# seung-lab/crackle

Hardware: AMD Instinct MI355X
Metric: voxels/s encode+decode, 1024x1024x512 uint32; bit-exact .ckl bytes (higher is better)
Workload: dtype u32

## Files before the change

### crackle_amd/csrc/ckl_encode.hip

```cpp
#include "ckl_encoder.hpp"
#include "ckl_runs.hpp"
#include "ckl_trail.hpp"

#include <algorithm>
#include <atomic>
#include <chrono>
#include <functional>
#include <memory>
#include <mutex>

namespace ckl {

using namespace dev;

template <typename LABEL>
__global__ void __launch_bounds__(kBlock) k_stats(const LABEL* __restrict__ labels, uint64_t voxels, unsigned long long* __restrict__ out ) {
	__shared__ unsigned long long s_max[kWaves], s_pairs[kWaves];
	unsigned long long mx = 0, pairs = 0;
	const uint64_t stride = static_cast<uint64_t>(gridDim.x) * kBlock;
	for (uint64_t i = static_cast<uint64_t>(blockIdx.x) * kBlock + threadIdx.x; i < voxels; i += stride) {
		const LABEL v = labels[i];
		if (static_cast<unsigned long long>(v) > mx) mx = v;
		if (i > 0) pairs += (labels[i - 1] == v);
	}
	for (int d = kWave / 2; d >= 1; d >>= 1) {
		const unsigned long long om = __shfl_xor(mx, d, kWave);
		const unsigned long long op = __shfl_xor(pairs, d, kWave);
		mx = om > mx ? om : mx;
		pairs += op;
	}
	const int lane = threadIdx.x & 63, wave = threadIdx.x >> 6;
	if (lane == 0) { s_max[wave] = mx; s_pairs[wave] = pairs; }
	__syncthreads();
	if (threadIdx.x == 0) {
		for (int w = 1; w < kWaves; w++) { mx = s_max[w] > mx ? s_max[w] : mx; pairs += s_pairs[w]; }
		atomicMax(out, mx);
		atomicAdd(out + 1, pairs);
	}
}

constexpr uint32_t kPlaneUnroll = 4;

template <typename LABEL>
__global__ void __launch_bounds__(kBlock) k_label_planes(
	const LABEL* __restrict__ labels, uint32_t sx, uint32_t sy, uint32_t chunks_per_row,
	uint32_t* __restrict__ planeV, uint32_t* __restrict__ planeH, uint32_t row_words, uint64_t plane_words,
	uint32_t* __restrict__ count_v, uint32_t* __restrict__ count_h
) {
	__shared__ uint32_t s_red[2 * kWaves];
	const uint32_t zi = blockIdx.y;
	const int lane = threadIdx.x & 63, wave = threadIdx.x >> 6;
	const uint32_t units = chunks_per_row * sy;
	const uint32_t unit0 = (blockIdx.x * kWaves + wave) * kPlaneUnroll;
	const LABEL* slice = labels + static_cast<uint64_t>(zi) * sy * sx;
	LABEL v[kPlaneUnroll], up[kPlaneUnroll], lf[kPlaneUnroll];
	uint32_t xs[kPlaneUnroll], ys[kPlaneUnroll];
#pragma unroll
	for (uint32_t k = 0; k < kPlaneUnroll; k++) {
		const uint32_t unit = unit0 + k;
		const uint32_t y = unit / chunks_per_row;
		const uint32_t x = (unit - y * chunks_per_row) * 64u + lane;
		xs[k] = x; ys[k] = y;
		const bool valid = unit < units && x < sx;
		const LABEL* row = slice + static_cast<uint64_t>(y) * sx;
		v[k] = valid ? row[x] : LABEL(0);
		up[k] = (valid && y > 0) ? row[static_cast<int64_t>(x) - static_cast<int64_t>(sx)] : v[k];
		lf[k] = (valid && lane == 0 && x > 0) ? row[x - 1] : v[k];
	}
	uint32_t nv = 0, nh = 0;
#pragma unroll
	for (uint32_t k = 0; k < kPlaneUnroll; k++) {
		const uint32_t unit = unit0 + k;
		const bool valid = unit < units && xs[k] < sx;
		LABEL left = __shfl_up(v[k], 1, kWave);
		if (lane == 0) left = lf[k];
		const bool dv = valid && xs[k] > 0 && v[k] != left;
		const bool dh = valid && v[k] != up[k];
		const unsigned long long mv = __ballot(dv), mh = __ballot(dh);
		if (lane == 0 && unit < units) {
			const uint32_t c = xs[k] >> 6;
			const uint64_t wbase = zi * plane_words + static_cast<uint64_t>(ys[k]) * row_words + c * 2u;
			planeV[wbase] = static_cast<uint32_t>(mv);
			planeH[wbase] = static_cast<uint32_t>(mh);
			if (c * 2u + 1u < row_words) {
				planeV[wbase + 1] = static_cast<uint32_t>(mv >> 32);
				planeH[wbase + 1] = static_cast<uint32_t>(mh >> 32);
			}
			nv += __popcll(mv);
			nh += __popcll(mh);
		}
	}
	if (lane == 0) { s_red[wave] = nv; s_red[kWaves + wave] = nh; }
	__syncthreads();
	if (threadIdx.x == 0) {
		uint32_t tv = 0, th = 0;
		for (int w = 0; w < kWaves; w++) { tv += s_red[w]; th += s_red[kWaves + w]; }
		if (tv) atomicAdd(count_v + zi, tv);
		if (th) atomicAdd(count_h + zi, th);
	}
}

constexpr uint32_t kBandRows = 32;

template <typename V, typename T>
__device__ __forceinline__ V nt_load_vec(const T* p) {
	typedef uint32_t u32x4_t __attribute__((ext_vector_type(4)));
	static_assert(sizeof(V) == 16, "one 16-byte vector");
	const u32x4_t raw = __builtin_nontemporal_load(reinterpret_cast<const u32x4_t*>(p));
	V v;
	__builtin_memcpy(&v, &raw, 16);
	return v;
}

template <typename T>
__device__ __forceinline__ T wave_shift_up1_label(T v) {
	if constexpr (sizeof(T) == 8) {
		const uint32_t lo = dev::wave_shift_up1(static_cast<uint32_t>(v), 0u), hi = dev::wave_shift_up1(static_cast<uint32_t>(static_cast<uint64_t>(v) >> 32), 0u);
		return static_cast<T>((static_cast<uint64_t>(hi) << 32) | lo);
	}
	else return static_cast<T>(dev::wave_shift_up1(static_cast<uint32_t>(v), 0u));
}
template <uint32_t G>
__device__ __forceinline__ uint32_t or_over_lane_group(uint32_t v) {
	static_assert(G == 2 || G == 4 || G == 8 || G == 16, "lane groups inside a row of 16");
	if constexpr (G >= 2) v |= dev::dpp_u32<0xB1, 0xF>(0u, v);
	if constexpr (G >= 4) v |= dev::dpp_u32<0x4E, 0xF>(0u, v);
	if constexpr (G >= 8) v |= dev::dpp_u32<0x141, 0xF>(0u, v);
	if constexpr (G >= 16) v |= dev::dpp_u32<0x140, 0xF>(0u, v);
	return v;
}

template <typename LABEL>
__global__ void __launch_bounds__(kBlock) k_label_planes_stream(
	const LABEL* __restrict__ labels, uint32_t sx, uint32_t sy, uint32_t strips, uint32_t bands,
	uint32_t* __restrict__ planeV, uint32_t* __restrict__ planeH, uint32_t row_words, uint64_t plane_words,
	uint32_t* __restrict__ partial, unsigned long long* __restrict__ partial_max, unsigned long long* __restrict__ total_pairs
) {
	if (blockIdx.x == 0 && blockIdx.y == 0 && threadIdx.x == 0) *total_pairs = 0;
	constexpr uint32_t P = 16 / sizeof(LABEL);
	constexpr uint32_t G = 32 / P;
	constexpr uint32_t WPR = 64 / G;
	struct alignas(16) Vec { LABEL v[P]; };
	__shared__ uint32_t s_red[3 * kWaves];
	__shared__ unsigned long long s_max[kWaves];
	__shared__ __attribute__((aligned(16))) uint32_t s_words[kWaves][2][kBandRows * WPR];
	const uint32_t zi = blockIdx.y;
	const uint32_t lane = threadIdx.x & 63u, wave = threadIdx.x >> 6;
	const uint32_t task = blockIdx.x * kWaves + wave;
	uint32_t nv = 0, nh = 0, pairs = 0;
	LABEL mxl = 0;
	if (task < strips * bands) {
		const uint32_t band = __builtin_amdgcn_readfirstlane(task / strips), strip = __builtin_amdgcn_readfirstlane(task - (task / strips) * strips);
		const uint32_t x0 = strip * (64u * P);
		const uint32_t x = x0 + lane * P;
		const uint32_t y0 = band * kBandRows, y1 = min(y0 + kBandRows, sy);
		const bool active = x < sx;
		const uint64_t slice_off = static_cast<uint64_t>(zi) * sy * sx;
		const LABEL* col = labels + slice_off + (active ? x : 0u);
		Vec prev;
#pragma unroll
		for (uint32_t i = 0; i < P; i++) prev.v[i] = 0;
		if (y0 > 0) prev = nt_load_vec<Vec>(col + static_cast<uint64_t>(y0 - 1) * sx);
		uint32_t* sv = s_words[wave][0];
		uint32_t* sh = s_words[wave][1];
		auto edge_of = [&](uint32_t y, bool& have) -> LABEL {
			const uint64_t lin = slice_off + static_cast<uint64_t>(y) * sx + x0;
			have = lin > 0;
			const uint64_t at = have ? lin - 1 : 0;
			if constexpr (sizeof(LABEL) >= 4) return labels[at];
			else {
				const uint64_t byte = at * sizeof(LABEL);
				const uint32_t w = reinterpret_cast<const uint32_t*>(reinterpret_cast<uintptr_t>(labels) & ~static_cast<uintptr_t>(3))[(byte + (reinterpret_cast<uintptr_t>(labels) & 3u)) >> 2];
				return static_cast<LABEL>(w >> (8u * static_cast<uint32_t>((byte + (reinterpret_cast<uintptr_t>(labels) & 3u)) & 3u)));
			}
		};
		constexpr uint32_t kRowsAhead = 4;
		Vec rows[kRowsAhead];
		LABEL edges[kRowsAhead];
		bool have_edges[kRowsAhead];
		auto request = [&](uint32_t r, uint32_t y) {
			const uint32_t yl = y < y1 ? y : y1 - 1u;
			rows[r] = nt_load_vec<Vec>(col + static_cast<uint64_t>(yl) * sx);
			edges[r] = edge_of(yl, have_edges[r]);
		};
#pragma unroll
		for (uint32_t r = 0; r < kRowsAhead; r++) request(r, y0 + r);
#pragma unroll
		for (uint32_t it = 0; it < kBandRows / kRowsAhead; it++) {
			const uint32_t yb = y0 + it * kRowsAhead;
#pragma unroll
			for (uint32_t r = 0; r < kRowsAhead; r++) {
				const uint32_t y = yb + r;
				const Vec cur = rows[r];
				const LABEL edge = edges[r];
				const bool have_edge = have_edges[r];
				request(r, y + kRowsAhead);
				if (y >= y1) continue;
				LABEL left = wave_shift_up1_label(cur.v[P - 1]);
				bool have_left = true;
				if (lane == 0) { left = edge; have_left = have_edge; }
				uint32_t bv = 0, bh = 0;
				if (active) {
#pragma unroll
					for (uint32_t i = 0; i < P; i++) {
						const LABEL l = i ? cur.v[i - 1] : left;
						bv |= (cur.v[i] != l ? 1u : 0u) << i;
						bh |= (cur.v[i] != prev.v[i] ? 1u : 0u) << i;
						mxl = cur.v[i] > mxl ? cur.v[i] : mxl;
					}
					pairs += P - __popc(bv) - ((have_left || (bv & 1u)) ? 0u : 1u);
					if (x == 0) bv &= ~1u;
					if (y == 0) bh = 0u;
				}
				nv += __popc(bv); nh += __popc(bh);
				bv <<= (lane % G) * P; bh <<= (lane % G) * P;
				bv = or_over_lane_group<G>(bv); bh = or_over_lane_group<G>(bh);
				if ((lane % G) == 0) { sv[(y - y0) * WPR + lane / G] = bv; sh[(y - y0) * WPR + lane / G] = bh; }
				prev = cur;
			}
		}
		const uint32_t word0 = x0 >> 5;
		uint32_t* pv = planeV + zi * plane_words;
		uint32_t* ph = planeH + zi * plane_words;
		constexpr uint32_t kVecWords = WPR >= 4 ? 4u : WPR;
		constexpr uint32_t kLanesPerRow = WPR / kVecWords;
		for (uint32_t r0 = 0; r0 < y1 - y0; r0 += 64u / kLanesPerRow) {
			const uint32_t r = r0 + lane / kLanesPerRow, w = (lane % kLanesPerRow) * kVecWords;
			if (r >= y1 - y0) continue;
			const uint64_t at = static_cast<uint64_t>(y0 + r) * row_words + word0 + w;
			if (word0 + w + kVecWords <= row_words && ((at & (kVecWords - 1u)) == 0u) && kVecWords == 4u) {
				*reinterpret_cast<uint4*>(pv + at) = *reinterpret_cast<const uint4*>(sv + r * WPR + w);
				*reinterpret_cast<uint4*>(ph + at) = *reinterpret_cast<const uint4*>(sh + r * WPR + w);
			}
			else {
				for (uint32_t q = 0; q < kVecWords; q++) if (word0 + w + q < row_words) { pv[at + q] = sv[r * WPR + w + q]; ph[at + q] = sh[r * WPR + w + q]; }
			}
		}
	}
	nv = wave_sum(nv); nh = wave_sum(nh); pairs = wave_sum(pairs);
	unsigned long long mx = static_cast<unsigned long long>(mxl);
	for (int d = kWave / 2; d >= 1; d >>= 1) { const unsigned long long o = __shfl_xor(mx, d, kWave); mx = o > mx ? o : mx; }
	if (lane == 0) { s_red[wave] = nv; s_red[kWaves + wave] = nh; s_red[2 * kWaves + wave] = pairs; s_max[wave] = mx; }
	__syncthreads();
	if (threadIdx.x == 0) {
		uint32_t tv = 0, th = 0, tp = 0;
		unsigned long long tm = 0;
		for (int w = 0; w < kWaves; w++) { tv += s_red[w]; th += s_red[kWaves + w]; tp += s_red[2 * kWaves + w]; tm = s_max[w] > tm ? s_max[w] : tm; }
		const uint64_t o = static_cast<uint64_t>(zi) * gridDim.x + blockIdx.x;
		partial[o * 4 + 0] = tv; partial[o * 4 + 1] = th; partial[o * 4 + 2] = tp; partial[o * 4 + 3] = 0;
		partial_max[o] = tm;
	}
}

__global__ void __launch_bounds__(kBlock) k_planes_from_cracks(
	const uint32_t* __restrict__ crackV, const uint32_t* __restrict__ crackH, uint32_t sx, uint32_t sy,
	uint32_t row_words, uint64_t plane_words, uint32_t permissible,
	uint32_t* __restrict__ planeV, uint32_t* __restrict__ planeH, uint32_t* __restrict__ counts, uint32_t nslices
) {
	__shared__ uint32_t s_red[kWaves];
	const uint32_t zi = blockIdx.y;
	const uint64_t i = static_cast<uint64_t>(blockIdx.x) * kBlock + threadIdx.x;
	uint32_t nv = 0, nh = 0;
	if (i < plane_words) {
		const uint32_t y = static_cast<uint32_t>(i / row_words);
		const uint32_t w = static_cast<uint32_t>(i - static_cast<uint64_t>(y) * row_words);
		const uint32_t left = sx - w * 32u;
		const uint32_t in_row = left >= 32u ? 0xFFFFFFFFu : ((1u << left) - 1u);
		const uint32_t mv = in_row & (w == 0 ? 0xFFFFFFFEu : 0xFFFFFFFFu);
		const uint32_t mh = y >= 1 ? in_row : 0u;
		const uint64_t at = zi * plane_words + i;
		const uint32_t inv = permissible ? 0xFFFFFFFFu : 0u;
		const uint32_t v = (crackV[at] ^ inv) & mv, h = (crackH[at] ^ inv) & mh;
		planeV[at] = v; planeH[at] = h;
		nv = __popc(v); nh = __popc(h);
	}
	nv = block_sum(nv, s_red); nh = block_sum(nh, s_red);
	if (threadIdx.x == 0) {
		if (nv) atomicAdd(counts + zi, nv);
		if (nh) atomicAdd(counts + nslices + zi, nh);
	}
}

__global__ void __launch_bounds__(kBlock) k_planes_reduce(
	const uint32_t* __restrict__ partial, const unsigned long long* __restrict__ partial_max, uint32_t nblk,
	unsigned long long* __restrict__ out ,
	unsigned long long* __restrict__ total_pairs
) {
	__shared__ uint32_t s_red[kWaves];
	__shared__ unsigned long long s_max[kWaves];
	const uint32_t zi = blockIdx.x;
	uint32_t tv = 0, th = 0, tp = 0;
	unsigned long long tm = 0;
	for (uint32_t b = threadIdx.x; b < nblk; b += kBlock) {
		const uint64_t o = static_cast<uint64_t>(zi) * nblk + b;
		tv += partial[o * 4 + 0]; th += partial[o * 4 + 1]; tp += partial[o * 4 + 2];
		const unsigned long long m = partial_max[o];
		tm = m > tm ? m : tm;
	}
	tv = block_sum(tv, s_red); th = block_sum(th, s_red); tp = block_sum(tp, s_red);
	for (int d = kWave / 2; d >= 1; d >>= 1) { const unsigned long long o = __shfl_xor(tm, d, kWave); tm = o > tm ? o : tm; }
	if ((threadIdx.x & 63) == 0) s_max[threadIdx.x >> 6] = tm;
	__syncthreads();
	if (threadIdx.x == 0) {
		for (int w = 0; w < kWaves; w++) tm = s_max[w] > tm ? s_max[w] : tm;
		out[4ull * zi + 0] = tv; out[4ull * zi + 1] = th; out[4ull * zi + 2] = tp; out[4ull * zi + 3] = tm;
		atomicAdd(total_pairs, static_cast<unsigned long long>(tp));
	}
}

enum : uint8_t { CODE_UP = 0, CODE_RIGHT = 1, CODE_DOWN = 2, CODE_LEFT = 3, CODE_NONE = 0xFE, CODE_TOMB = 0xFF };

struct FinishArgs {
	int sx, sy, xw, yw;
	uint32_t z0;
	uint32_t markov;
	const uint64_t* cbase;
	const uint64_t* kbase;
	const uint32_t* n_chains;
	const uint32_t* n_raw;
	const uint32_t* n_valid;
	const uint8_t* cp;
	const uint32_t* chain_node;
	const uint32_t* chain_off;
	const uint32_t* chain_clen;
	uint32_t* chain_order;
	uint32_t* chain_dst;
	uint32_t* chain_vstart;
	uint8_t* fcode;
	uint8_t* dcode;
	const uint64_t* pbase;
	uint8_t* payload;
	const uint64_t* bbase;
	uint8_t* boc;
	uint32_t* payload_len;
	uint32_t* boc_len;
};

__device__ __forceinline__ void put_le_dev(uint8_t* p, uint32_t v, int w) {
	for (int i = 0; i < w; i++) p[i] = static_cast<uint8_t>((v >> (8 * i)) & 0xFF);
}

constexpr int kFinishBlock = 1024;
constexpr int kFinishWaves = kFinishBlock / kWave;

constexpr uint32_t kFinishChains = 2048;

__global__ void __launch_bounds__(kFinishBlock) k_finish(FinishArgs a) {
	__shared__ uint32_t s_scan[kFinishWaves];
	__shared__ uint32_t s_node[kFinishChains], s_clen[kFinishChains], s_off[kFinishChains], s_ord[kFinishChains], s_dst[kFinishChains], s_vst[kFinishChains];
	const uint32_t zi = blockIdx.x + a.z0;
	const int tid = threadIdx.x;
	const uint32_t nch = a.n_chains[zi], nraw = a.n_raw[zi], nvalid = a.n_valid[zi];
	const uint8_t* cp = a.cp + a.cbase[zi];
	uint8_t* fcode = a.fcode + a.cbase[zi];
	const bool staged = nch <= kFinishChains;
	const uint32_t* ch_node = a.chain_node + a.kbase[zi];
	const uint32_t* ch_off = a.chain_off + a.kbase[zi];
	const uint32_t* ch_clen = a.chain_clen + a.kbase[zi];
	uint32_t* order = a.chain_order + a.kbase[zi];
	uint32_t* dst = a.chain_dst + a.kbase[zi];
	uint32_t* vstart = a.chain_vstart + a.kbase[zi];
	if (staged) {
		for (uint32_t c = tid; c < nch; c += kFinishBlock) { s_node[c] = ch_node[c]; s_clen[c] = ch_clen[c]; s_off[c] = ch_off[c]; }
		__syncthreads();
		ch_node = s_node; ch_off = s_off; ch_clen = s_clen; order = s_ord; dst = s_dst; vstart = s_vst;
	}
	const uint32_t sxe = a.sx + 1;

	if (tid == 0) {
		uint32_t v = 0;
		for (uint32_t c = 0; c < nch; c++) { vstart[c] = v; v += ch_clen[c]; }
		for (uint32_t c = 0; c < nch; c++) {
			const uint32_t key = ch_node[c];
			uint32_t p = c;
			while (p > 0 && ch_node[order[p - 1]] > key) { order[p] = order[p - 1]; p--; }
			order[p] = c;
		}
		uint32_t d = 0;
		for (uint32_t i = 0; i < nch; i++) { dst[order[i]] = d; d += ch_clen[order[i]]; }

		uint8_t* b = a.boc + a.bbase[zi];
		uint32_t num_y = 0, index_size = a.yw;
		for (uint32_t i = 0; i < nch;) {
			const uint32_t y = ch_node[order[i]] / sxe;
			uint32_t j = i;
			while (j < nch && ch_node[order[j]] / sxe == y) j++;
			index_size += a.yw + (j - i + 1) * a.xw;
			num_y++;
			i = j;
		}
		uint32_t idx = 0;
		put_le_dev(b + idx, index_size, 4); idx += 4;
		put_le_dev(b + idx, num_y, a.yw); idx += a.yw;
		uint32_t last_y = 0;
		for (uint32_t i = 0; i < nch;) {
			const uint32_t y = ch_node[order[i]] / sxe;
			uint32_t j = i;
			while (j < nch && ch_node[order[j]] / sxe == y) j++;
			put_le_dev(b + idx, y - last_y, a.yw); idx += a.yw;
			last_y = y;
			put_le_dev(b + idx, j - i, a.xw); idx += a.xw;
			uint32_t last_x = 0;
			for (uint32_t k = i; k < j; k++) {
				const uint32_t x = ch_node[order[k]] - sxe * y;
				put_le_dev(b + idx, x - last_x, a.xw); idx += a.xw;
				last_x = x;
			}
			i = j;
		}
		a.boc_len[zi] = idx;
	}
	__syncthreads();
	__threadfence_block();

	constexpr uint32_t kPer = 16;
	uint32_t carry = 0;
	for (uint32_t tile = 0; tile < nraw; tile += kFinishBlock * kPer) {
		const uint32_t i0 = tile + tid * kPer;
		uint32_t cnt = 0;
		uint8_t c[kPer];
		static_assert(kPer == 16, "one 16-byte load per thread");
		if (i0 + kPer <= nraw) {
			const uint4 v = *reinterpret_cast<const uint4*>(cp + i0);
			const uint32_t w4[4] = { v.x, v.y, v.z, v.w };
#pragma unroll
			for (uint32_t k = 0; k < kPer; k++) c[k] = static_cast<uint8_t>(w4[k >> 2] >> (8u * (k & 3u)));
		}
		else {
#pragma unroll
			for (uint32_t k = 0; k < kPer; k++) { const uint32_t i = i0 + k; c[k] = i < nraw ? cp[i] : CODE_TOMB; }
		}
#pragma unroll
		for (uint32_t k = 0; k < kPer; k++) cnt += (c[k] != CODE_TOMB);
		uint32_t v[1] = { cnt }, tot[1];
		block_excl_add<1, kFinishWaves>(v, tot, s_scan);
		uint32_t g = carry + v[0];
		if (cnt) {
			uint32_t lo = 0, hi = nch;
			while (lo + 1 < hi) {
				const uint32_t mid = (lo + hi) >> 1;
				if (ch_off[mid] <= i0) lo = mid; else hi = mid;
			}
			uint32_t chain = lo;
			uint32_t next_off = (chain + 1 < nch) ? ch_off[chain + 1] : 0xFFFFFFFFu;
			if (i0 + kPer <= next_off) {
				struct __attribute__((packed)) U128 { uint4 v; };
				struct __attribute__((packed)) U64 { unsigned long long v; };
				struct __attribute__((packed)) U32 { uint32_t v; };
				struct __attribute__((packed)) U16 { uint16_t v; };
				uint8_t* d = fcode + dst[chain] + (g - vstart[chain]);
				unsigned long long w0 = 0, w1 = 0;
				uint32_t m = 0;
#pragma unroll
				for (uint32_t k = 0; k < kPer; k++) {
					if (c[k] != CODE_TOMB) {
						if (m < 8u) w0 |= static_cast<unsigned long long>(c[k]) << (8u * m);
						else w1 |= static_cast<unsigned long long>(c[k]) << (8u * (m - 8u));
						m++;
					}
				}
				if (m == 16u) reinterpret_cast<U128*>(d)->v = make_uint4(static_cast<uint32_t>(w0), static_cast<uint32_t>(w0 >> 32), static_cast<uint32_t>(w1), static_cast<uint32_t>(w1 >> 32));
				else {
					if (m & 8u) { reinterpret_cast<U64*>(d)->v = w0; d += 8; w0 = w1; }
					if (m & 4u) { reinterpret_cast<U32*>(d)->v = static_cast<uint32_t>(w0); d += 4; w0 >>= 32; }
					if (m & 2u) { reinterpret_cast<U16*>(d)->v = static_cast<uint16_t>(w0); d += 2; w0 >>= 16; }
					if (m & 1u) d[0] = static_cast<uint8_t>(w0);
				}
			}
			else {
#pragma unroll
				for (uint32_t k = 0; k < kPer; k++) {
					const uint32_t i = i0 + k;
					while (i >= next_off) { chain++; next_off = (chain + 1 < nch) ? ch_off[chain + 1] : 0xFFFFFFFFu; }
					if (c[k] != CODE_TOMB) {
						fcode[dst[chain] + (g - vstart[chain])] = c[k];
						g++;
					}
				}
			}
		}
		carry += tot[0];
	}
	__syncthreads();
	__threadfence_block();

	if (a.markov) {
		uint8_t* dcode = a.dcode + a.cbase[zi];
		for (uint32_t g = tid; g < nvalid; g += kFinishBlock) {
			const uint32_t prev = g ? fcode[g - 1] : 0u;
			dcode[g] = static_cast<uint8_t>((fcode[g] - prev) & 3u);
		}
		if (tid == 0) a.payload_len[zi] = 0;
	}
	else {
		uint8_t* out = a.payload + a.pbase[zi];
		const uint32_t nbytes = (nvalid + 3) / 4;
		const uint32_t nwords = (nvalid + 15) / 16;
		for (uint32_t w = tid; w < nwords; w += kFinishBlock) {
			const uint32_t g0 = w * 16u;
			uint8_t c[16];
			if (g0 + 16u <= nvalid) {
				const uint4 v = *reinterpret_cast<const uint4*>(fcode + g0);
				const uint32_t w4[4] = { v.x, v.y, v.z, v.w };
#pragma unroll
				for (uint32_t j = 0; j < 16; j++) c[j] = static_cast<uint8_t>(w4[j >> 2] >> (8u * (j & 3u)));
			}
			else {
#pragma unroll
				for (uint32_t j = 0; j < 16; j++) c[j] = g0 + j < nvalid ? fcode[g0 + j] : 0;
			}
			uint32_t prev = g0 ? fcode[g0 - 1] : 0u;
			uint32_t enc = 0;
#pragma unroll
			for (uint32_t j = 0; j < 16; j++) {
				if (g0 + j < nvalid) enc |= ((c[j] - prev) & 3u) << (2 * j);
				prev = c[j];
			}
			if (4u * w + 4u <= nbytes) reinterpret_cast<uint32_t*>(out)[w] = enc;
			else for (uint32_t k = 4u * w; k < nbytes; k++) out[k] = static_cast<uint8_t>(enc >> (8u * (k - 4u * w)));
		}
		if (tid == 0) a.payload_len[zi] = nbytes;
	}
}

__device__ __forceinline__ uint32_t markov_ctx(const uint8_t* d, uint32_t g, int order) {
	uint32_t ctx = 0;
	for (int j = 1; j <= order; j++) {
		const uint32_t v = (g >= static_cast<uint32_t>(j)) ? d[g - j] : 0u;
		ctx |= v << (2 * (order - j));
	}
	return ctx;
}

__global__ void __launch_bounds__(kBlock) k_markov_hist(
	const uint8_t* __restrict__ dcode, const uint64_t* __restrict__ cbase, const uint32_t* __restrict__ n_valid,
	int order, uint32_t* __restrict__ hist, uint32_t lds_entries
) {
	extern __shared__ uint32_t s_hist[];
	const uint32_t zi = blockIdx.x;
	const uint8_t* d = dcode + cbase[zi];
	const uint32_t n = n_valid[zi];
	const uint32_t entries = 4u << (2 * order);
	const bool local = entries <= lds_entries;
	if (local) {
		for (uint32_t i = threadIdx.x; i < entries; i += kBlock) s_hist[i] = 0;
		__syncthreads();
	}
	uint32_t* target = local ? s_hist : hist;
	constexpr uint32_t kPer = 32;
	for (uint32_t g0 = threadIdx.x * kPer; g0 < n; g0 += kBlock * kPer) {
		uint32_t key = 0xFFFFFFFFu, cnt = 0;
		const uint32_t g1 = g0 + kPer < n ? g0 + kPer : n;
		for (uint32_t g = g0; g < g1; g++) {
			const uint32_t k = markov_ctx(d, g, order) * 4u + d[g];
			if (k == key) cnt++;
			else {
				if (cnt) atomicAdd(target + key, cnt);
				key = k; cnt = 1;
			}
		}
		if (cnt) atomicAdd(target + key, cnt);
	}
	if (local) {
		__syncthreads();
		for (uint32_t i = threadIdx.x; i < entries; i += kBlock) { const uint32_t v = s_hist[i]; if (v) atomicAdd(hist + i, v); }
	}
}

__global__ void __launch_bounds__(kBlock) k_markov_pack(
	const uint8_t* __restrict__ dcode, const uint64_t* __restrict__ cbase, const uint32_t* __restrict__ n_valid,
	int order, const uint8_t* __restrict__ model ,
	const uint64_t* __restrict__ pbase, uint8_t* __restrict__ payload, uint32_t* __restrict__ payload_len
) {
	__shared__ uint32_t s_scan[kWaves];
	const uint32_t zi = blockIdx.x;
	const uint8_t* d = dcode + cbase[zi];
	const uint32_t n = n_valid[zi];
	uint32_t* words = reinterpret_cast<uint32_t*>(payload + pbase[zi]);
	constexpr uint32_t kPer = 8;
	uint32_t carry = 0;
	for (uint32_t tile = 0; tile < n; tile += kBlock * kPer) {
		const uint32_t g0 = tile + threadIdx.x * kPer;
		uint32_t bits[kPer], lens[kPer], tot_len = 0;
#pragma unroll
		for (uint32_t k = 0; k < kPer; k++) {
			const uint32_t g = g0 + k;
			bits[k] = 0; lens[k] = 0;
			if (g < n) {
				if (g == 0) { bits[k] = d[0]; lens[k] = 2; }
				else {
					const uint32_t r = model[markov_ctx(d, g, order) * 4u + d[g]];
					bits[k] = (r == 0) ? 0u : (r == 1) ? 1u : (r == 2) ? 3u : 7u;
					lens[k] = (r == 0) ? 1u : (r == 1) ? 2u : 3u;
				}
			}
			tot_len += lens[k];
		}
		uint32_t v[1] = { tot_len }, tot[1];
		block_excl_add<1>(v, tot, s_scan);
		uint32_t off = carry + v[0];
#pragma unroll
		for (uint32_t k = 0; k < kPer; k++) {
			if (lens[k] && bits[k]) {
				const uint32_t w = off >> 5, sh = off & 31;
				atomicOr(words + w, bits[k] << sh);
				if (sh + lens[k] > 32) atomicOr(words + w + 1, bits[k] >> (32 - sh));
			}
			off += lens[k];
		}
		carry += tot[0];
	}
	if (threadIdx.x == 0) payload_len[zi] = (carry + 7) / 8;
}

template <typename LABEL>
__global__ void __launch_bounds__(kBlock) k_mapping_comps(
	const LABEL* __restrict__ labels, RunArrays r, uint64_t sxy,
	const uint64_t* __restrict__ comp_off, uint64_t* __restrict__ mapping
) {
	const uint32_t zi = blockIdx.y;
	const uint32_t c = blockIdx.x * kBlock + threadIdx.x;
	if (c >= r.ncomp[zi]) return;
	mapping[comp_off[zi] + c] = static_cast<uint64_t>(labels[zi * sxy + r.comp_pix[r.rbase[zi] + c]]);
}

__global__ void __launch_bounds__(kBlock) k_paint_components(
	const uint32_t* __restrict__ planeV, uint32_t row_words, uint64_t plane_words, uint32_t sx, uint64_t sxy,
	const uint32_t* __restrict__ word_base, const uint64_t* __restrict__ rbase, const uint32_t* __restrict__ run_cc,
	const uint64_t* __restrict__ comp_off, uint32_t id_base, uint32_t* __restrict__ out
) {
	const uint32_t zi = blockIdx.y;
	const uint32_t px = blockIdx.x * kBlock + threadIdx.x;
	if (px >= sxy) return;
	const uint32_t y = px / sx, x = px - y * sx;
	const uint32_t w = x >> 5, bit = x & 31u;
	const uint64_t wi = zi * plane_words + static_cast<uint64_t>(y) * row_words + w;
	uint32_t b = planeV[wi];
	if (w == 0) b |= 1u;
	const uint32_t run = word_base[wi] - 1u + __popc(b & (0xFFFFFFFFu >> (31u - bit)));
	out[zi * sxy + px] = run_cc[rbase[zi] + run] + static_cast<uint32_t>(comp_off[zi]) + id_base;
}

__global__ void __launch_bounds__(kBlock) k_paint_components4(
	const uint32_t* __restrict__ planeV, uint32_t row_words, uint64_t plane_words, uint32_t sx, uint64_t sxy,
	const uint32_t* __restrict__ word_base, const uint64_t* __restrict__ rbase, const uint32_t* __restrict__ run_cc,
	const uint64_t* __restrict__ comp_off, uint32_t id_base, uint32_t* __restrict__ out
) {
	const uint32_t zi = blockIdx.y;
	const uint32_t px = (blockIdx.x * kBlock + threadIdx.x) * 4u;
	if (px >= sxy) return;
	const uint32_t y = px / sx, x = px - y * sx;
	const uint32_t w = x >> 5, bit = x & 31u;
	const uint64_t wi = zi * plane_words + static_cast<uint64_t>(y) * row_words + w;
	uint32_t b = planeV[wi];
	if (w == 0) b |= 1u;
	const uint32_t* cc = run_cc + rbase[zi];
	const uint32_t add = static_cast<uint32_t>(comp_off[zi]) + id_base;
	uint32_t run = word_base[wi] - 1u + __popc(b & (0xFFFFFFFFu >> (31u - bit)));
	uint4 o;
	o.x = cc[run] + add;
	run += (b >> (bit + 1u)) & 1u; o.y = cc[run] + add;
	run += (b >> (bit + 2u)) & 1u; o.z = cc[run] + add;
	run += (b >> (bit + 3u)) & 1u; o.w = cc[run] + add;
	*reinterpret_cast<uint4*>(out + zi * sxy + px) = o;
}

inline void launch_paint_components(hipStream_t s, const uint32_t* planeV, uint32_t row_words, uint64_t plane_words, int64_t sx, int64_t sy, int64_t sz,
	const uint32_t* word_base, const uint64_t* rbase, const uint32_t* run_cc, const uint64_t* comp_off, uint32_t id_base, uint32_t* out) {
	const uint64_t sxy = static_cast<uint64_t>(sx) * sy;
	const bool four = sx % 4 == 0 && (reinterpret_cast<uintptr_t>(out) & 15u) == 0;
	const uint64_t threads = four ? sxy / 4 : sxy;
	const dim3 grid(static_cast<uint32_t>((threads + kBlock - 1) / kBlock), static_cast<uint32_t>(sz));
	if (four) hipLaunchKernelGGL(k_paint_components4, grid, dim3(kBlock), 0, s, planeV, row_words, plane_words, static_cast<uint32_t>(sx), sxy, word_base, rbase, run_cc, comp_off, id_base, out);
	else hipLaunchKernelGGL(k_paint_components, grid, dim3(kBlock), 0, s, planeV, row_words, plane_words, static_cast<uint32_t>(sx), sxy, word_base, rbase, run_cc, comp_off, id_base, out);
}

__global__ void __launch_bounds__(kBlock) k_bitonic_step(uint64_t* __restrict__ a, uint32_t j, uint32_t k, uint32_t n) {
	const uint32_t i = blockIdx.x * kBlock + threadIdx.x;
	if (i >= n) return;
	const uint32_t l = i ^ j;
	if (l > i) {
		const uint64_t x = a[i], y = a[l];
		const bool up = (i & k) == 0;
		if ((x > y) == up) { a[i] = y; a[l] = x; }
	}
}
__global__ void __launch_bounds__(kBlock) k_bitonic_step2(uint64_t* __restrict__ a, uint32_t j, uint32_t k, uint32_t n) {
	const uint32_t t = blockIdx.x * kBlock + threadIdx.x;
	if (t >= n / 4u) return;
	const uint32_t h = j >> 1;
	const uint32_t lb = static_cast<uint32_t>(__ffs(h)) - 1u;
	const uint32_t i = (t & (h - 1u)) | ((t >> lb) << (lb + 2u));
	uint64_t v0 = a[i], v1 = a[i | h], v2 = a[i | j], v3 = a[i | j | h];
	const bool up = (i & k) == 0;
	auto cx = [&](uint64_t& x, uint64_t& y) { if ((x > y) == up) { const uint64_t z = x; x = y; y = z; } };
	cx(v0, v2); cx(v1, v3);
	cx(v0, v1); cx(v2, v3);
	a[i] = v0; a[i | h] = v1; a[i | j] = v2; a[i | j | h] = v3;
}

__global__ void __launch_bounds__(kBlock) k_bitonic_first(uint64_t* __restrict__ a, uint32_t n) {
	__shared__ uint64_t s[2048];
	const uint32_t base = blockIdx.x * 2048u;
	for (uint32_t t = threadIdx.x; t < 2048u; t += kBlock) s[t] = base + t < n ? a[base + t] : ~0ull;
	__syncthreads();
	for (uint32_t k = 2; k <= 2048u; k <<= 1) {
		for (uint32_t j = k >> 1; j > 0; j >>= 1) {
			for (uint32_t t = threadIdx.x; t < 2048u; t += kBlock) {
				const uint32_t l = t ^ j;
				if (l > t) {
					const uint64_t x = s[t], y = s[l];
					const bool up = ((base + t) & k) == 0;
					if ((x > y) == up) { s[t] = y; s[l] = x; }
				}
			}
			__syncthreads();
		}
	}
	for (uint32_t t = threadIdx.x; t < 2048u; t += kBlock) if (base + t < n) a[base + t] = s[t];
}
__global__ void __launch_bounds__(kBlock) k_bitonic_local(uint64_t* __restrict__ a, uint32_t j_start, uint32_t k, uint32_t n) {
	__shared__ uint64_t s[2048];
	const uint32_t base = blockIdx.x * 2048u;
	for (uint32_t t = threadIdx.x; t < 2048u; t += kBlock) s[t] = base + t < n ? a[base + t] : ~0ull;
	__syncthreads();
	for (uint32_t j = j_start; j > 0; j >>= 1) {
		for (uint32_t t = threadIdx.x; t < 2048u; t += kBlock) {
			const uint32_t l = t ^ j;
			if (l > t) {
				const uint64_t x = s[t], y = s[l];
				const bool up = ((base + t) & k) == 0;
				if ((x > y) == up) { s[t] = y; s[l] = x; }
			}
		}
		__syncthreads();
	}
	for (uint32_t t = threadIdx.x; t < 2048u; t += kBlock) if (base + t < n) a[base + t] = s[t];
}
__global__ void __launch_bounds__(kBlock) k_pad_copy_u64(const uint64_t* __restrict__ src, uint64_t n, uint64_t* __restrict__ dst, uint64_t n_pad) {
	const uint64_t i = static_cast<uint64_t>(blockIdx.x) * kBlock + threadIdx.x;
	if (i < n_pad) dst[i] = i < n ? src[i] : ~0ull;
}
constexpr uint32_t kUniqPer = 8, kUniqItems = kBlock * kUniqPer;
__device__ __forceinline__ uint32_t unique_heads(const uint64_t* __restrict__ sorted, uint32_t n, uint32_t i0, uint64_t (&v)[kUniqPer]) {
	uint32_t flag = 0;
#pragma unroll
	for (uint32_t q = 0; q < kUniqPer; q++) {
		const uint32_t i = i0 + q;
		v[q] = i < n ? sorted[i] : 0;
		const uint64_t prev = q ? v[q - 1] : ((i > 0 && i < n) ? sorted[i - 1] : 0);
		flag |= ((i < n && (i == 0 || v[q] != prev)) ? 1u : 0u) << q;
	}
	return flag;
}
__global__ void __launch_bounds__(kBlock) k_unique_count(const uint64_t* __restrict__ sorted, uint32_t n, uint32_t* __restrict__ blk_count) {
	__shared__ uint32_t s_red[kWaves];
	uint64_t v[kUniqPer];
	const uint32_t flag = unique_heads(sorted, n, blockIdx.x * kUniqItems + threadIdx.x * kUniqPer, v);
	const uint32_t tot = block_sum(static_cast<uint32_t>(__popc(flag)), s_red);
	if (threadIdx.x == 0) blk_count[blockIdx.x] = tot;
}
__global__ void __launch_bounds__(kBlock) k_unique_scan(uint32_t* __restrict__ blk_count, uint32_t nblk, uint32_t* __restrict__ n_uniq) {
	__shared__ uint32_t s_scan[kWaves];
	uint32_t carry = 0;
	for (uint32_t b0 = 0; b0 < nblk; b0 += kBlock) {
		const uint32_t b = b0 + threadIdx.x;
		uint32_t c[1] = { b < nblk ? blk_count[b] : 0u }, tot[1];
		block_excl_add<1>(c, tot, s_scan);
		if (b < nblk) blk_count[b] = carry + c[0];
		carry += tot[0];
	}
	if (threadIdx.x == 0) *n_uniq = carry;
}
__global__ void __launch_bounds__(kBlock) k_unique_scatter(const uint64_t* __restrict__ sorted, uint32_t n, const uint32_t* __restrict__ blk_base, uint64_t* __restrict__ uniq) {
	__shared__ uint32_t s_scan[kWaves];
	uint64_t v[kUniqPer];
	const uint32_t flag = unique_heads(sorted, n, blockIdx.x * kUniqItems + threadIdx.x * kUniqPer, v);
	uint32_t c[1] = { static_cast<uint32_t>(__popc(flag)) }, tot[1];
	block_excl_add<1>(c, tot, s_scan);
	uint32_t o = blk_base[blockIdx.x] + c[0];
#pragma unroll
	for (uint32_t q = 0; q < kUniqPer; q++) if ((flag >> q) & 1u) uniq[o++] = v[q];
}

constexpr uint64_t kLabelHashEmpty = ~0ull;
__device__ __forceinline__ uint32_t label_hash(uint64_t v) {
	v ^= v >> 33; v *= 0xff51afd7ed558ccdull; v ^= v >> 33;
	return static_cast<uint32_t>(v);
}
__global__ void __launch_bounds__(kBlock) k_label_hash_insert(const uint64_t* __restrict__ mapping, uint32_t n, unsigned long long* __restrict__ table, uint32_t mask, uint32_t* __restrict__ has_max) {
	const uint32_t i = blockIdx.x * kBlock + threadIdx.x;
	if (i >= n) return;
	const unsigned long long v = mapping[i];
	if (v == kLabelHashEmpty) { *has_max = 1u; return; }
	uint32_t h = label_hash(v) & mask;
	for (uint32_t probe = 0; probe <= mask; probe++) {
		const unsigned long long seen = table[h];
		if (seen == v) return;
		if (seen == kLabelHashEmpty) {
			const unsigned long long old = atomicCAS(table + h, kLabelHashEmpty, v);
			if (old == kLabelHashEmpty || old == v) return;
		}
		h = (h + 1u) & mask;
	}
}
__device__ __forceinline__ uint32_t hash_occupied(const unsigned long long* __restrict__ table, uint32_t slots, uint32_t i0, uint64_t (&v)[kUniqPer]) {
	uint32_t flag = 0;
#pragma unroll
	for (uint32_t q = 0; q < kUniqPer; q++) {
		v[q] = i0 + q < slots ? table[i0 + q] : kLabelHashEmpty;
		flag |= (v[q] != kLabelHashEmpty ? 1u : 0u) << q;
	}
	return flag;
}
__global__ void __launch_bounds__(kBlock) k_label_hash_count(const unsigned long long* __restrict__ table, uint32_t slots, uint32_t* __restrict__ blk_count) {
	__shared__ uint32_t s_red[kWaves];
	uint64_t v[kUniqPer];
	const uint32_t flag = hash_occupied(table, slots, blockIdx.x * kUniqItems + threadIdx.x * kUniqPer, v);
	const uint32_t tot = block_sum(static_cast<uint32_t>(__popc(flag)), s_red);
	if (threadIdx.x == 0) blk_count[blockIdx.x] = tot;
}
__global__ void __launch_bounds__(kBlock) k_label_hash_scatter(
	const unsigned long long* __restrict__ table, uint32_t slots, const uint32_t* __restrict__ blk_base, const uint32_t* __restrict__ n_found,
	const uint32_t* __restrict__ has_max, uint64_t* __restrict__ out
) {
	__shared__ uint32_t s_scan[kWaves];
	uint64_t v[kUniqPer];
	const uint32_t flag = hash_occupied(table, slots, blockIdx.x * kUniqItems + threadIdx.x * kUniqPer, v);
	uint32_t c[1] = { static_cast<uint32_t>(__popc(flag)) }, tot[1];
	block_excl_add<1>(c, tot, s_scan);
	uint32_t o = blk_base[blockIdx.x] + c[0];
#pragma unroll
	for (uint32_t q = 0; q < kUniqPer; q++) if ((flag >> q) & 1u) out[o++] = v[q];
	if (blockIdx.x == 0 && threadIdx.x == 0 && *has_max) out[*n_found] = kLabelHashEmpty;
}

__global__ void __launch_bounds__(kBlock) k_flat_section(
	const uint64_t* __restrict__ uniq, const uint32_t* __restrict__ n_uniq, int stored_width,
	const uint32_t* __restrict__ ncomp, uint32_t nslices, int component_width,
	const uint64_t* __restrict__ mapping, uint32_t n, uint8_t* __restrict__ out
) {
	const uint32_t nu = *n_uniq;
	const int key_width = nu <= 0xFFu ? 1 : (nu <= 0xFFFFu ? 2 : 4);
	const uint32_t i = blockIdx.x * kBlock + threadIdx.x;
	if (i == 0) for (int b = 0; b < 8; b++) out[b] = static_cast<uint8_t>((static_cast<uint64_t>(nu) >> (8 * b)) & 0xFF);
	uint8_t* o_uniq = out + 8;
	uint8_t* o_cc = o_uniq + static_cast<uint64_t>(nu) * stored_width;
	uint8_t* o_keys = o_cc + static_cast<uint64_t>(nslices) * component_width;
	if (i < nu) {
		const uint64_t v = uniq[i];
		for (int b = 0; b < stored_width; b++) o_uniq[static_cast<uint64_t>(i) * stored_width + b] = static_cast<uint8_t>((v >> (8 * b)) & 0xFF);
	}
	if (i < nslices) {
		const uint32_t v = ncomp[i];
		for (int b = 0; b < component_width; b++) o_cc[static_cast<uint64_t>(i) * component_width + b] = b < 4 ? static_cast<uint8_t>((v >> (8 * b)) & 0xFF) : 0;
	}
	if (i < n) {
		const uint64_t v = mapping[i];
		uint32_t lo = 0, hi = nu;
		while (lo + 1 < hi) {
			const uint32_t mid = (lo + hi) >> 1;
			if (uniq[mid] <= v) lo = mid; else hi = mid;
		}
		for (int b = 0; b < key_width; b++) o_keys[static_cast<uint64_t>(i) * key_width + b] = static_cast<uint8_t>((lo >> (8 * b)) & 0xFF);
	}
}

__global__ void __launch_bounds__(kBlock) k_code_offsets(
	const uint32_t* __restrict__ boc_len, const uint32_t* __restrict__ payload_len, const uint32_t* __restrict__ slice_err,
	uint32_t nslices, uint64_t* __restrict__ out_off, uint32_t* __restrict__ report
) {
	__shared__ unsigned long long s_part[kBlock];
	__shared__ uint32_t s_err;
	if (threadIdx.x == 0) s_err = 0;
	const uint32_t per = (nslices + kBlock - 1) / kBlock;
	const uint32_t z0 = threadIdx.x * per, z1 = min(z0 + per, nslices);
	unsigned long long sum = 0;
	uint32_t err = 0;
	for (uint32_t z = z0; z < z1; z++) { sum += static_cast<unsigned long long>(boc_len[z]) + payload_len[z]; err |= slice_err[z]; }
	s_part[threadIdx.x] = sum;
	__syncthreads();
	if (err) atomicOr(&s_err, err);
	if (threadIdx.x == 0) {
		unsigned long long run = 0;
		for (uint32_t i = 0; i < kBlock; i++) { const unsigned long long v = s_part[i]; s_part[i] = run; run += v; }
		report[nslices] = static_cast<uint32_t>(run); report[nslices + 1] = static_cast<uint32_t>(run >> 32);
	}
	__syncthreads();
	unsigned long long off = s_part[threadIdx.x];
	for (uint32_t z = z0; z < z1; z++) {
		const uint32_t len = boc_len[z] + payload_len[z];
		out_off[z] = off;
		report[z] = len;
		off += len;
	}
	if (threadIdx.x == 0) report[nslices + 2] = s_err;
}

__global__ void __launch_bounds__(kBlock) k_gather_codes(
	const uint8_t* __restrict__ boc, const uint64_t* __restrict__ bbase, const uint32_t* __restrict__ boc_len,
	const uint8_t* __restrict__ payload, const uint64_t* __restrict__ pbase, const uint32_t* __restrict__ payload_len,
	const uint64_t* __restrict__ out_off, uint8_t* __restrict__ out
) {
	const uint32_t zi = blockIdx.x;
	uint8_t* o = out + out_off[zi];
	const uint32_t nb = boc_len[zi], np = payload_len[zi];
	const uint8_t* b = boc + bbase[zi];
	const uint8_t* p = payload + pbase[zi];
	for (uint32_t i = threadIdx.x; i < nb; i += kBlock) o[i] = b[i];
	for (uint32_t i = threadIdx.x; i < np; i += kBlock) o[nb + i] = p[i];
}

struct CrcShifts { uint32_t x[8]; };
__global__ void __launch_bounds__(kBlock) k_crc32c_pieces(const uint8_t* __restrict__ data, uint64_t n, uint64_t pad, uint32_t P, CrcShifts sh, uint32_t* __restrict__ parts) {
	__shared__ uint32_t s_tab[256];
	__shared__ uint32_t s_st[kBlock];
	{
		uint32_t c = threadIdx.x;
		for (int k = 0; k < 8; k++) c = (c & 1u) ? (c >> 1) ^ dev::kCrcPoly : (c >> 1);
		s_tab[threadIdx.x] = c;
	}
	__syncthreads();
	const uint64_t f0 = (static_cast<uint64_t>(blockIdx.x) * kBlock + threadIdx.x) * P;
	uint32_t c = 0;
	for (uint32_t g = 0; g < P; g += 16) {
		const int64_t m0 = static_cast<int64_t>(f0 + g) - static_cast<int64_t>(pad);
		uint32_t w[4] = { 0, 0, 0, 0 };
		if (m0 >= 0 && static_cast<uint64_t>(m0) + 16u <= n) __builtin_memcpy(w, data + m0, 16);
		else if (m0 + 16 > 0) for (int b = 0; b < 16; b++) { const int64_t i = m0 + b; if (i >= 0 && static_cast<uint64_t>(i) < n) w[b >> 2] |= static_cast<uint32_t>(data[i]) << (8 * (b & 3)); }
#pragma unroll
		for (int b = 0; b < 16; b++) c = s_tab[(c ^ (w[b >> 2] >> (8 * (b & 3)))) & 0xFFu] ^ (c >> 8);
	}
	s_st[threadIdx.x] = c;
	__syncthreads();
	for (int k = 0; k < 8; k++) {
		const uint32_t stride = 1u << k;
		if ((threadIdx.x & (2u * stride - 1u)) == 0u) s_st[threadIdx.x] = gf_mul(s_st[threadIdx.x], sh.x[k]) ^ s_st[threadIdx.x + stride];
		__syncthreads();
	}
	if (threadIdx.x == 0) parts[blockIdx.x] = s_st[0];
}
__global__ void __launch_bounds__(kBlock) k_crc32c_fold(const uint32_t* __restrict__ parts, uint32_t G, CrcShifts sh, uint32_t init_term, uint32_t* __restrict__ out) {
	__shared__ uint32_t s_st[kBlock];
	s_st[threadIdx.x] = threadIdx.x < G ? parts[threadIdx.x] : 0u;
	__syncthreads();
	for (int k = 0; (1u << k) < G; k++) {
		const uint32_t stride = 1u << k;
		if ((threadIdx.x & (2u * stride - 1u)) == 0u && threadIdx.x + stride < G) s_st[threadIdx.x] = gf_mul(s_st[threadIdx.x], sh.x[k]) ^ s_st[threadIdx.x + stride];
		__syncthreads();
	}
	if (threadIdx.x == 0) out[0] = ~(s_st[0] ^ init_term);
}

__global__ void __launch_bounds__(kBlock) k_copy_bytes(const uint8_t* __restrict__ src, uint8_t* __restrict__ dst, uint64_t n) {
	const uint64_t head = min(n, static_cast<uint64_t>((4u - (reinterpret_cast<uintptr_t>(dst) & 3u)) & 3u));
	const uint64_t words = (n - head) / 4u;
	const uint64_t tid = static_cast<uint64_t>(blockIdx.x) * kBlock + threadIdx.x;
	const uint64_t stride = static_cast<uint64_t>(gridDim.x) * kBlock;
	if (tid < head) dst[tid] = src[tid];
	const uint64_t tail0 = head + words * 4u;
	if (tid < n - tail0) dst[tail0 + tid] = src[tail0 + tid];
	const uint8_t* s0 = src + head;
	const uint32_t sh = static_cast<uint32_t>(reinterpret_cast<uintptr_t>(s0) & 3u) * 8u;
	const uint32_t* sw = reinterpret_cast<const uint32_t*>(reinterpret_cast<uintptr_t>(s0) & ~static_cast<uintptr_t>(3));
	uint32_t* dw = reinterpret_cast<uint32_t*>(dst + head);
	if (sh == 0u) {
		for (uint64_t i = tid; i < words; i += stride) dw[i] = sw[i];
	}
	else {
		for (uint64_t i = tid; i < words; i += stride) dw[i] = __funnelshift_r(sw[i], sw[i + 1], sh);
	}
}

__global__ void __launch_bounds__(kBlock) k_trail_step_kinds(const uint32_t* __restrict__ events, const uint64_t* __restrict__ ibase, const uint32_t* __restrict__ n_events, uint32_t* __restrict__ counts) {
	__shared__ uint32_t s_c[5];
	const uint32_t zi = blockIdx.x;
	if (threadIdx.x < 5) s_c[threadIdx.x] = 0u;
	__syncthreads();
	const uint32_t n = n_events[zi] & ~(dev::kEvFormatAddr12 | dev::kEvWalkWide);
	const uint32_t* ev = events + ibase[zi];
	uint32_t c[4] = { 0, 0, 0, 0 };
	for (uint32_t i = threadIdx.x; i < n; i += kBlock) c[ev[i] >> 30]++;
	for (int k = 0; k < 4; k++) if (c[k]) atomicAdd(&s_c[k], c[k]);
	if (threadIdx.x == 0) {
		uint32_t run = 0, longest = 0;
		for (uint32_t i = 0; i < n; i++) { if ((ev[i] >> 30) == 1u) run = 0; else { run++; longest = run > longest ? run : longest; } }
		s_c[4] = longest;
	}
	__syncthreads();
	if (threadIdx.x < 5) counts[zi * 5u + threadIdx.x] = s_c[threadIdx.x];
}

}

using namespace ckl;

static void crc32c_device(const uint8_t* data, uint64_t n, uint32_t* parts, uint32_t* out, hipStream_t s) {
	uint32_t P = 128, G = 1;
	while (G < static_cast<uint32_t>(kBlock) && static_cast<uint64_t>(G) * kBlock * P < n) G <<= 1;
	if (static_cast<uint64_t>(G) * kBlock * P < n) P = static_cast<uint32_t>(((n + static_cast<uint64_t>(G) * kBlock - 1) / (static_cast<uint64_t>(G) * kBlock) + 15) / 16 * 16);
	const uint64_t frame = static_cast<uint64_t>(G) * kBlock * P;
	static std::mutex shifts_mutex;
	static uint32_t shifts_for = 0;
	static CrcShifts shifts_in, shifts_over;
	CrcShifts in_wg, over_wg;
	{
		std::lock_guard<std::mutex> lock(shifts_mutex);
		if (shifts_for != P) {
			for (int k = 0; k < 8; k++) {
				shifts_in.x[k] = gf_xpow(8ull * P << k);
				shifts_over.x[k] = gf_xpow(8ull * P * kBlock << k);
			}
			shifts_for = P;
		}
		in_wg = shifts_in; over_wg = shifts_over;
	}
	hipLaunchKernelGGL(k_crc32c_pieces, dim3(G), dim3(kBlock), 0, s, data, n, frame - n, P, in_wg, parts);
	hipLaunchKernelGGL(k_crc32c_fold, dim3(1), dim3(kBlock), 0, s, parts, G, over_wg, gf_mul(0xFFFFFFFFu, gf_xpow(8ull * n)), out);
}

static void copy_bytes_device(const uint8_t* src, uint8_t* dst, uint64_t n, hipStream_t s) {
	if (!n) return;
	const uint32_t blocks = static_cast<uint32_t>(std::min<uint64_t>((n / 4u + kBlock - 1) / kBlock + 1u, 8192u));
	hipLaunchKernelGGL(k_copy_bytes, dim3(blocks), dim3(kBlock), 0, s, src, dst, n);
}

namespace {

struct UploadPacker {
	struct Item { void* buf; size_t off, count; void (*bind)(void*, uint8_t*, size_t); };
	std::vector<Item> items;
	std::vector<uint8_t> image;
	template <typename T>
	void add(DevBuf<T>& dst, const std::vector<T>& src) {
		const size_t off = (image.size() + 255) & ~static_cast<size_t>(255);
		image.resize(off + std::max<size_t>(src.size(), 1) * sizeof(T));
		if (!src.empty()) memcpy(image.data() + off, src.data(), src.size() * sizeof(T));
		items.push_back({ &dst, off, src.size(), [](void* b, uint8_t* base, size_t n) { static_cast<DevBuf<T>*>(b)->borrow(reinterpret_cast<T*>(base), n); } });
	}
	void commit(DevBuf<uint8_t>& block, hipStream_t s, void** staging = nullptr) {
		if (image.empty()) return;
		for (const Item& it : items) it.bind(it.buf, nullptr, 0);
		block.ensure(image.size());
		if (staging) {
			if (*staging) host_out_free(*staging);
			*staging = host_out_alloc(std::max<size_t>(image.size(), 64u << 10));
			memcpy(*staging, image.data(), image.size());
			upload_small(block.p, *staging, image.size(), s, *staging);
		}
		else CKL_HIP(hipMemcpyAsync(block.p, image.data(), image.size(), hipMemcpyHostToDevice, s));
		for (const Item& it : items) it.bind(it.buf, block.p + it.off, it.count);
	}
};

template <typename LABEL>
VolumeStats volume_stats(ckl_encoder& e, const LABEL* labels, uint64_t voxels) {
	VolumeStats st;
	if (voxels == 0) return st;
	hipStream_t s = e.stream;
	e.d_stats.ensure(2);
	CKL_HIP(hipMemsetAsync(e.d_stats.p, 0, 2 * sizeof(unsigned long long), s));
	const uint32_t blocks = static_cast<uint32_t>(std::min<uint64_t>((voxels + kBlock - 1) / kBlock, 256ull * 8));
	hipLaunchKernelGGL(k_stats<LABEL>, dim3(blocks), dim3(kBlock), 0, s, labels, voxels, e.d_stats.p);
	auto r = download(e.d_stats.p, 2, s);
	st.max_label = r[0]; st.pairs = r[1];
	LABEL f, l;
	CKL_HIP(hipMemcpy(&f, labels, sizeof(LABEL), hipMemcpyDeviceToHost));
	CKL_HIP(hipMemcpy(&l, labels + (voxels - 1), sizeof(LABEL), hipMemcpyDeviceToHost));
	st.first = f; st.last = l;
	return st;
}

inline uint32_t* plane_v(const ckl_encoder& e) { return e.d_planes.p; }
inline uint32_t* plane_h(const ckl_encoder& e, uint32_t ns) { return e.d_planes.p + e.plane_words * ns; }

inline bool planes_cached(const ckl_encoder& e, const void* labels, int64_t sx, int64_t sy, int64_t sz) {
	return e.planes_for == labels && e.planes_dims[0] == sx && e.planes_dims[1] == sy && e.planes_dims[2] == sz;
}

inline uint64_t crack_edges(const ckl_encoder& e, int64_t sx, int64_t sy, size_t zi, bool permissible) {
	const uint64_t interior = static_cast<uint64_t>(sx > 0 ? sx - 1 : 0) * sy + static_cast<uint64_t>(sx) * (sy > 0 ? sy - 1 : 0);
	const uint64_t differ = static_cast<uint64_t>(e.count_v[zi]) + e.count_h[zi];
	return permissible ? interior - differ : differ;
}

void planes_collect(ckl_encoder& e, uint32_t ns, VolumeStats* st, const std::vector<unsigned long long>* fetched = nullptr) {
	std::vector<unsigned long long> mine;
	if (!fetched) { mine = download(e.d_plane_out.p, 4ull * ns, e.stream); fetched = &mine; }
	const std::vector<unsigned long long>& o = *fetched;
	e.count_v.resize(ns); e.count_h.resize(ns);
	VolumeStats v;
	for (uint32_t zi = 0; zi < ns; zi++) {
		e.count_v[zi] = static_cast<uint32_t>(o[4ull * zi]);
		e.count_h[zi] = static_cast<uint32_t>(o[4ull * zi + 1]);
		v.pairs += o[4ull * zi + 2];
		v.max_label = std::max<uint64_t>(v.max_label, o[4ull * zi + 3]);
	}
	e.planes_deferred = false;
	if (st) *st = v;
}

void trail_prezero(ckl_encoder& e, int64_t sx, int64_t sy, int64_t sz) {
	hipStream_t s = e.stream2;
	const uint32_t ns = static_cast<uint32_t>(sz);
	const uint64_t nverts = static_cast<uint64_t>(sx + 1) * (sy + 1);
	const uint32_t start_words = static_cast<uint32_t>((nverts + 31) / 32);
	e.d_slice_err.ensure(ns);
	e.t_counters.ensure(7 * static_cast<size_t>(ns));
	e.t_start_bits.ensure(static_cast<size_t>(start_words) * ns);
	CKL_HIP(hipMemsetAsync(e.d_slice_err.p, 0, ns * sizeof(uint32_t), s));
	CKL_HIP(hipMemsetAsync(e.t_counters.p, 0, 7 * static_cast<size_t>(ns) * sizeof(uint32_t), s));
	CKL_HIP(hipMemsetAsync(e.t_start_bits.p, 0, static_cast<size_t>(start_words) * ns * sizeof(uint32_t), s));
	CKL_HIP(hipEventRecord(e.ev_prezero, s));
	e.trail_zeroed = true;
}

template <typename LABEL>
void planes_pass(ckl_encoder& e, const LABEL* labels, int64_t sx, int64_t sy, int64_t sz, VolumeStats* st, bool defer = false) {
	hipStream_t s = e.stream;
	const uint32_t ns = static_cast<uint32_t>(sz);
	e.trail_zeroed = false;
	e.planes_deferred = false;
	e.row_words = static_cast<uint32_t>((sx + 31) / 32);
	e.plane_words = static_cast<uint64_t>(e.row_words) * sy;
	e.d_planes.ensure(2 * e.plane_words * ns);
	constexpr uint32_t P = 16 / sizeof(LABEL);
	const bool fast = !getenv("CKL_PLANES_GENERIC") && sx >= static_cast<int64_t>(P) && sx % P == 0 && (reinterpret_cast<uintptr_t>(labels) & 15u) == 0;
	if (fast) {
		const uint32_t strips = static_cast<uint32_t>((sx + 64 * P - 1) / (64 * P));
		const uint32_t bands = static_cast<uint32_t>((sy + kBandRows - 1) / kBandRows);
		const uint32_t nblk = (strips * bands + kWaves - 1) / kWaves;
		e.d_plane_partial.ensure(4ull * nblk * ns);
		e.d_plane_partial_max.ensure(static_cast<size_t>(nblk) * ns);
		e.d_plane_out.ensure(4ull * ns + 1);
		trail_prezero(e, sx, sy, sz);
		hipLaunchKernelGGL(k_label_planes_stream<LABEL>, dim3(nblk, ns), dim3(kBlock), 0, s,
			labels, static_cast<uint32_t>(sx), static_cast<uint32_t>(sy), strips, bands,
			plane_v(e), plane_h(e, ns), e.row_words, e.plane_words,
			e.d_plane_partial.p, e.d_plane_partial_max.p, e.d_plane_out.p + 4ull * ns);
		hipLaunchKernelGGL(k_planes_reduce, dim3(ns), dim3(kBlock), 0, s, e.d_plane_partial.p, e.d_plane_partial_max.p, nblk, e.d_plane_out.p, e.d_plane_out.p + 4ull * ns);
		e.planes_deferred = defer;
		if (!e.planes_deferred) planes_collect(e, ns, st);
		return;
	}
	if (st) *st = volume_stats<LABEL>(e, labels, static_cast<uint64_t>(sx) * sy * sz);
	e.d_count_vh.ensure(2 * static_cast<size_t>(ns));
	CKL_HIP(hipMemsetAsync(e.d_count_vh.p, 0, 2 * static_cast<size_t>(ns) * sizeof(uint32_t), s));
	const uint32_t chunks = static_cast<uint32_t>((sx + 63) / 64);
	const uint64_t units = static_cast<uint64_t>(chunks) * sy;
	hipLaunchKernelGGL(k_label_planes<LABEL>, dim3(static_cast<uint32_t>((units + kWaves * kPlaneUnroll - 1) / (kWaves * kPlaneUnroll)), ns), dim3(kBlock), 0, s,
		labels, static_cast<uint32_t>(sx), static_cast<uint32_t>(sy), chunks,
		plane_v(e), plane_h(e, ns), e.row_words, e.plane_words,
		e.d_count_vh.p, e.d_count_vh.p + ns);
	std::vector<uint32_t> c = download(e.d_count_vh.p, 2 * static_cast<size_t>(ns), s);
	e.count_v.assign(c.begin(), c.begin() + ns);
	e.count_h.assign(c.begin() + ns, c.end());
}

void planes_pass_any(ckl_encoder& e, const void* labels, int64_t sx, int64_t sy, int64_t sz, VolumeStats* st) {
	with_label_type(e.dtype_bytes, [&](auto t) { planes_pass(e, static_cast<const typename decltype(t)::type*>(labels), sx, sy, sz, st); });
}

enum class GraphFormat : uint32_t { IMPERMISSIBLE = 0, PERMISSIBLE = 1, ON_DEVICE = 2 };
inline GraphFormat graph_format(bool permissible) { return permissible ? GraphFormat::PERMISSIBLE : GraphFormat::IMPERMISSIBLE; }
void graph_pass(ckl_encoder& e, int64_t sx, int64_t sy, int64_t sz, GraphFormat format, VolumeStats* st = nullptr) {
	hipStream_t s = e.stream;
	const uint32_t ns = static_cast<uint32_t>(sz);
	e.tiles_x = static_cast<uint32_t>((sx + 1 + kTrailTileDim - 1) / kTrailTileDim);
	e.tiles_y = static_cast<uint32_t>((sy + 1 + 7) / 8);
	const uint32_t mtx = static_cast<uint32_t>((sx + 1 + 7) / 8), mty = static_cast<uint32_t>((sy + 1 + 7) / 8);
	e.mtx2 = (mtx + 1) / 2;
	e.adjm_stride = static_cast<uint64_t>(e.mtx2) * ((mty + 1) / 2) * 4 * 2;
	e.d_adjm.ensure(e.adjm_stride * ns);
	e.graph_blocks = (e.tiles_x * e.tiles_y + kBlock - 1) / kBlock;
	e.t_blk_special.ensure(static_cast<size_t>(e.graph_blocks) * ns);
	e.t_blk_corner.ensure(static_cast<size_t>(e.graph_blocks) * ns);
	e.d_count_vh.ensure(4 * static_cast<size_t>(ns));
	const bool on_device = format == GraphFormat::ON_DEVICE;
	if (on_device && !e.planes_deferred) throw Error(CKL_ERR_RUNTIME, "crackle_amd: internal: crack format left to the device without deferred counts");
	const unsigned long long half_voxels = static_cast<unsigned long long>(static_cast<int64_t>(static_cast<uint64_t>(sx) * sy * sz) / 2);
	hipLaunchKernelGGL(k_trail_graph, dim3(e.graph_blocks, ns), dim3(kBlock), 0, s,
		plane_v(e), plane_h(e, ns), e.row_words, e.plane_words,
		static_cast<uint32_t>(sx), static_cast<uint32_t>(sy), static_cast<uint32_t>(format),
		on_device ? e.d_plane_out.p + 4ull * ns : nullptr, half_voxels,
		reinterpret_cast<uint32_t*>(e.d_adjm.p), e.adjm_stride * 4,
		e.mtx2, e.tiles_x, e.tiles_y, e.t_blk_special.p, e.t_blk_corner.p);
	hipLaunchKernelGGL(k_trail_count_scan, dim3(ns), dim3(kBlock), 0, s, e.t_blk_special.p, e.t_blk_corner.p, e.graph_blocks,
		e.d_count_vh.p + 2 * static_cast<size_t>(ns), e.d_count_vh.p + 3 * static_cast<size_t>(ns));
	std::vector<unsigned long long> po;
	if (e.planes_deferred) {
		po.resize(4ull * ns);
		CKL_HIP(hipMemcpyAsync(po.data(), e.d_plane_out.p, po.size() * sizeof(unsigned long long), hipMemcpyDeviceToHost, s));
	}
	std::vector<uint32_t> c = download(e.d_count_vh.p + 2 * static_cast<size_t>(ns), 2 * static_cast<size_t>(ns), s);
	e.count_special.assign(c.begin(), c.begin() + ns);
	e.count_corner.assign(c.begin() + ns, c.end());
	VolumeStats v;
	if (!po.empty()) planes_collect(e, ns, &v, &po);
	if (st && !po.empty()) *st = v;
	e.graph_permissible = on_device ? static_cast<int64_t>(v.pairs) < static_cast<int64_t>(static_cast<uint64_t>(sx) * sy * sz) / 2 : format == GraphFormat::PERMISSIBLE;
}

enum class CrackGoal { HISTOGRAM, CODES };
struct CrackRequest {
	CrackGoal goal = CrackGoal::CODES;
	bool permissible = false;
	int markov_order = 0;
	const std::vector<uint8_t>* model = nullptr;
	bool reuse_trail = false;
	std::function<void()> overlap;
};
struct CrackResult {
	std::vector<uint32_t> code_len;
	uint64_t total = 0;
	bool any_chain = false;
	std::vector<uint32_t> hist;
	std::vector<uint8_t> model;
};

inline size_t trail_walk_lds(uint32_t max_special) { return (static_cast<size_t>(max_special) + 256) * 16 + 1024; }

FinishArgs finish_args(const ckl_encoder& e, int64_t sx, int64_t sy, int markov_order) {
	FinishArgs fa;
	fa.sx = static_cast<int>(sx); fa.sy = static_cast<int>(sy);
	fa.xw = byte_width(static_cast<uint64_t>(sx) + 1); fa.yw = byte_width(static_cast<uint64_t>(sy) + 1);
	fa.markov = markov_order ? 1u : 0u;
	fa.cbase = e.d_cbase.p; fa.kbase = e.d_kbase.p;
	fa.n_chains = e.d_n_chains.p; fa.n_raw = e.d_n_raw.p; fa.n_valid = e.d_n_valid.p;
	fa.cp = e.d_cp.p; fa.chain_node = e.d_chain_node.p; fa.chain_off = e.d_chain_off.p; fa.chain_clen = e.d_chain_clen.p;
	fa.chain_order = e.d_chain_order.p; fa.chain_dst = e.d_chain_dst.p; fa.chain_vstart = e.d_chain_vstart.p;
	fa.fcode = e.d_fcode.p; fa.dcode = e.d_dcode.p;
	fa.pbase = e.d_pbase.p; fa.payload = e.d_payload.p; fa.bbase = e.d_bbase.p; fa.boc = e.d_boc.p;
	fa.payload_len = e.d_payload_len.p; fa.boc_len = e.d_boc_len.p;
	fa.z0 = 0;
	return fa;
}

TrailArgs trail_args(const ckl_encoder& e, int64_t sx, int64_t sy, uint32_t ns) {
	const uint64_t nverts = static_cast<uint64_t>(sx + 1) * (sy + 1);
	TrailArgs ta;
	ta.adjm = e.d_adjm.p; ta.adjm_stride = e.adjm_stride; ta.mtx2 = e.mtx2; ta.tiles_x = e.tiles_x; ta.tiles_y = e.tiles_y;
	ta.planeV = plane_v(e); ta.planeH = plane_h(e, ns); ta.row_words = e.row_words; ta.plane_words = e.plane_words;
	ta.sx = static_cast<uint32_t>(sx); ta.sy = static_cast<uint32_t>(sy); ta.inv = e.graph_permissible ? 0xFFFFFFFFu : 0u;
	ta.sxe = static_cast<uint32_t>(sx + 1); ta.sye = static_cast<uint32_t>(sy + 1); ta.nverts = static_cast<uint32_t>(nverts);
	ta.max_steps = e.t_max_steps.p;
	ta.nbase = e.t_nbase.p; ta.ncap = e.t_ncap.p;
	ta.n_nodes = e.t_counters.p; ta.n_corners = e.t_counters.p + 2 * ns;
	ta.n_starts = e.t_counters.p + 3 * ns; ta.n_items = e.t_counters.p + 4 * ns;
	ta.node_vertex = e.t_node_vertex.p; ta.node_adj = e.t_node_adj.p; ta.vert2node = e.t_vert2node.p;
	ta.cobase = e.t_cobase.p; ta.cocap = e.t_cocap.p; ta.corner_vertex = e.t_corner_vertex.p;
	ta.dart_end = e.t_dart_end.p; ta.dart_len = e.t_dart_len.p; ta.dart_minv = e.t_dart_minv.p; ta.dart_minpos = e.t_dart_minpos.p;
	ta.dart_codes = e.t_dart_codes.p; ta.dart_inline = e.t_dart_inline.p;
	ta.parent = e.t_parent.p; ta.compmin = e.t_compmin.p;
	ta.start_bits = e.t_start_bits.p; ta.start_words = static_cast<uint32_t>((nverts + 31) / 32); ta.starts = e.t_starts.p;
	ta.ibase = e.t_ibase.p; ta.icap = e.t_icap.p; ta.items = e.t_items.p; ta.item_off = e.t_item_off.p;
	ta.sbase = e.d_sbase.p; ta.scap = e.d_scap.p; ta.stack_node = e.d_stack_node.p; ta.stack_item = e.d_stack_code.p;
	ta.kbase = e.d_kbase.p; ta.kcap = e.d_kcap.p;
	ta.chain_node = e.d_chain_node.p; ta.chain_item0 = e.t_chain_item0.p; ta.chain_off = e.d_chain_off.p; ta.chain_clen = e.d_chain_clen.p;
	ta.n_chains = e.d_n_chains.p; ta.n_raw = e.d_n_raw.p; ta.n_valid = e.d_n_valid.p;
	ta.cbase = e.d_cbase.p; ta.ccap = e.d_ccap.p; ta.cp = e.d_cp.p; ta.slice_err = e.d_slice_err.p;
	ta.events = e.t_events.p; ta.n_events = e.t_counters.p + 5 * ns; ta.seg_len_sum = e.t_counters.p + 6 * ns; ta.chain_ev0 = e.t_chain_ev0.p; ta.ev_lnd = e.t_ev_lnd.p; ta.ev_item = e.t_ev_item.p;
	ta.dbg = nullptr;
	{ const char* env = getenv("CKL_TRAIL_WALK"); ta.walk_plain = (env && !strcmp(env, "plain")) ? 1u : 0u; ta.walk_no_regs = (env && !strcmp(env, "lds")) ? 1u : 0u; }
	{ const char* env = getenv("CKL_TRAIL_WALK_STACK"); ta.walk_stack_cap = env ? static_cast<uint32_t>(std::max(1, atoi(env))) : 0xFFFFFFFFu; }
	ta.graph_blocks = e.graph_blocks; ta.blk_special = e.t_blk_special.p; ta.blk_corner = e.t_blk_corner.p;
	ta.z0 = 0;
	return ta;
}

void trail_diag(ckl_encoder& e, uint32_t ns, const unsigned long long* ta_dbg, uint32_t max_special, size_t trail_lds_used) {
	hipStream_t s = e.stream;
	std::vector<uint32_t> c = download(e.t_counters.p, 5 * static_cast<size_t>(ns), s);
	double m[5] = { 0 };
	for (int k = 0; k < 5; k++) for (uint32_t zi = 0; zi < ns; zi++) m[k] += static_cast<double>(c[static_cast<size_t>(k) * ns + zi]) / ns;
	double sp = 0, co = 0;
	for (uint32_t zi = 0; zi < ns; zi++) { sp += static_cast<double>(e.count_special[zi]) / ns; co += static_cast<double>(e.count_corner[zi]) / ns; }
	if (ta_dbg) {
		std::vector<unsigned long long> g = download(ta_dbg, 16, s);
		if (g[11]) fprintf(stderr, "[ckl trail diag, k_trail_walk] mean cycles per slice: table fill=%.0f fill + walk=%.0f\n", static_cast<double>(g[6]) / g[11], static_cast<double>(g[7]) / g[11]);
		if (g[11]) fprintf(stderr, "[ckl trail diag, k_trail_walk] slices=%llu iterations/slice=%.0f cycles/iteration=%.0f clock=%.2f GHz (cycles / 100 MHz ticks)\n",
			g[11], static_cast<double>(g[8]) / g[11], g[8] ? static_cast<double>(g[9]) / g[8] : 0.0, g[10] ? static_cast<double>(g[9]) / (g[10] * 10.0) : 0.0);
		fprintf(stderr, "[ckl trail diag, k_trail_components, mean cycles per slice] union=%.0f component minima=%.0f starts/splits=%.0f bitmap scan=%.0f\n",
			static_cast<double>(g[12]) / ns, static_cast<double>(g[13]) / ns, static_cast<double>(g[14]) / ns, static_cast<double>(g[15]) / ns);
		fprintf(stderr, "[ckl trail diag, k_trail_segments] waves=%llu iterations/wave mean=%.1f max=%llu cycles/wave mean=%.0f max=%llu cycles/iteration=%.0f active lanes/iteration=%.1f\n",
			g[4], g[4] ? static_cast<double>(g[0]) / g[4] : 0.0, g[1], g[4] ? static_cast<double>(g[2]) / g[4] : 0.0, g[3],
			g[0] ? static_cast<double>(g[2]) / g[0] : 0.0, g[0] ? static_cast<double>(g[5]) / g[0] : 0.0);
	}
	fprintf(stderr, "[ckl trail diag] max degree-1/3/4 vertices of a slice=%u, k_trail_walk LDS=%zu bytes\n", max_special, trail_lds_used);
	fprintf(stderr, "[ckl trail diag, mean per slice] degree-1/3/4 vertices=%.0f corners=%.0f nodes=%.0f starts=%.0f items=%.0f\n", sp, co, m[0], m[3], m[4]);
}

void check_walk_errors(ckl_encoder& e, uint32_t ns) {
	const std::vector<uint32_t> errs = download(e.d_slice_err.p, ns, e.stream);
	for (uint32_t zi = 0; zi < ns; zi++) if (errs[zi]) throw Error(CKL_ERR_RUNTIME, "crackle_amd: crack walk scratch overflow on z=" + std::to_string(zi));
}

CrackResult crack_pass(ckl_encoder& e, int64_t sx, int64_t sy, int64_t sz, const CrackRequest& rq) {
	hipStream_t s = e.stream;
	const uint32_t ns = static_cast<uint32_t>(sz);
	const uint64_t nverts = static_cast<uint64_t>(sx + 1) * (sy + 1);
	const int markov_order = rq.markov_order;
	const bool reuse_trail = rq.reuse_trail;
	if (rq.goal == CrackGoal::HISTOGRAM && (!markov_order || rq.model)) throw Error(CKL_ERR_RUNTIME, "crackle_amd: internal: a markov histogram needs an order and no model");
	CrackResult result;
	e.d_slice_err.ensure(ns);
	const bool prezeroed = e.trail_zeroed && !reuse_trail;
	e.trail_zeroed = false;
	if (prezeroed) CKL_HIP(hipStreamWaitEvent(s, e.ev_prezero, 0));
	if (!reuse_trail && !prezeroed) CKL_HIP(hipMemsetAsync(e.d_slice_err.p, 0, ns * sizeof(uint32_t), s));

	std::vector<uint64_t> cbase(ns), sbase(ns), kbase(ns);
	std::vector<uint32_t> ccap(ns), scap(ns), kcap(ns), max_steps(ns);
	std::vector<uint64_t> nbase(ns), cobase(ns), ibase(ns);
	std::vector<uint32_t> ncap(ns), cocap(ns), icap(ns);
	uint64_t ctot = 0, stot = 0, ktot = 0, ntot = 0, cotot = 0, itot = 0;
	uint32_t max_ncap = 0, max_cocap = 0, max_icap = 0, max_special = 0;
	bool any = false;
	for (uint32_t zi = 0; zi < ns; zi++) {
		const uint64_t E = crack_edges(e, sx, sy, zi, rq.permissible);
		any = any || E > 0;
		const uint64_t cc = ((7 * E + 16 + 15) / 16) * 16;
		if (cc > 0xFFFFFFF0ull) throw Error(CKL_ERR_RUNTIME, "crackle_amd: slice has too many crack edges");
		cbase[zi] = ctot; ccap[zi] = static_cast<uint32_t>(cc); ctot += cc;
		max_steps[zi] = static_cast<uint32_t>(E + 1);
		const uint64_t nc = ((static_cast<uint64_t>(e.count_special[zi]) + e.count_corner[zi] + 16) / 16) * 16;
		if (nc >= (1ull << 28)) throw Error(CKL_ERR_RUNTIME, "crackle_amd: slice has too many crack vertices");
		nbase[zi] = ntot; ncap[zi] = static_cast<uint32_t>(nc); ntot += nc;
		cobase[zi] = cotot; cocap[zi] = e.count_corner[zi]; cotot += e.count_corner[zi];
		const uint64_t ic = 7 * nc + 16;
		ibase[zi] = itot; icap[zi] = static_cast<uint32_t>(ic); itot += ic;
		sbase[zi] = stot; scap[zi] = static_cast<uint32_t>(2 * nc + 4); stot += 2 * nc + 4;
		kbase[zi] = ktot; kcap[zi] = static_cast<uint32_t>(nc); ktot += nc;
		max_ncap = std::max<uint32_t>(max_ncap, ncap[zi]);
		max_cocap = std::max<uint32_t>(max_cocap, cocap[zi]);
		max_icap = std::max<uint32_t>(max_icap, icap[zi]);
		max_special = std::max<uint32_t>(max_special, e.count_special[zi]);
	}
	result.any_chain = any;
	if (g_ht && g_ht->on) {
		uint32_t over = 0;
		for (uint32_t zi = 0; zi < ns; zi++) over += e.count_special[zi] > 3584u;
		fprintf(stderr, "[ckl trail nodes] max special %u, slices above 3584: %u of %u\n", max_special, over, ns);
	}
	HT_MARK("c:caps");

	UploadPacker tables;
	tables.add(e.d_cbase, cbase); tables.add(e.d_ccap, ccap);
	tables.add(e.d_sbase, sbase); tables.add(e.d_scap, scap);
	tables.add(e.d_kbase, kbase); tables.add(e.d_kcap, kcap);
	e.d_cp.ensure(ctot); e.d_fcode.ensure(ctot);
	if (markov_order) e.d_dcode.ensure(ctot);
	e.d_stack_node.ensure(stot); e.d_stack_code.ensure(stot);
	e.d_chain_node.ensure(ktot); e.d_chain_off.ensure(ktot); e.d_chain_clen.ensure(ktot);
	e.d_chain_order.ensure(ktot); e.d_chain_dst.ensure(ktot); e.d_chain_vstart.ensure(ktot);
	e.d_n_chains.ensure(ns); e.d_n_raw.ensure(ns); e.d_n_valid.ensure(ns);
	e.d_payload_len.ensure(ns); e.d_boc_len.ensure(ns);
	const int xw = byte_width(static_cast<uint64_t>(sx) + 1), yw = byte_width(static_cast<uint64_t>(sy) + 1);
	std::vector<uint64_t> pbase(ns), bbase(ns);
	uint64_t ptot = 0, btot = 0;
	for (uint32_t zi = 0; zi < ns; zi++) {
		const uint64_t ncodes = ccap[zi];
		const uint64_t pbytes = markov_order ? (3ull * ncodes + 2 + 7) / 8 : (ncodes + 3) / 4;
		pbase[zi] = ptot; ptot += ((pbytes + 8 + 3) / 4) * 4;
		const uint64_t bbytes = 4 + yw + static_cast<uint64_t>(kcap[zi]) * (yw + 2 * xw);
		bbase[zi] = btot; btot += bbytes;
	}
	tables.add(e.d_pbase, pbase); tables.add(e.d_bbase, bbase);
	tables.add(e.t_nbase, nbase); tables.add(e.t_ncap, ncap);
	tables.add(e.t_cobase, cobase); tables.add(e.t_cocap, cocap);
	tables.add(e.t_ibase, ibase); tables.add(e.t_icap, icap);
	tables.add(e.t_max_steps, max_steps);
	tables.commit(e.d_crack_tables, s, e.uploads_by_kernel ? &e.tables_staging : nullptr);
	HT_MARK("c:tables");
	e.d_payload.ensure(ptot + 8); e.d_boc.ensure(btot + 8);
	e.codes_capacity = ptot + btot;
	if (markov_order) CKL_HIP(hipMemsetAsync(e.d_payload.p, 0, ptot + 8, s));

	DevBuf<unsigned long long> d_tdbg;
	size_t trail_lds_used = 0;
	if (!reuse_trail) {
		e.t_counters.ensure(7 * static_cast<size_t>(ns));
		if (!prezeroed) CKL_HIP(hipMemsetAsync(e.t_counters.p, 0, 7 * static_cast<size_t>(ns) * sizeof(uint32_t), s));
		e.t_node_vertex.ensure(ntot); e.t_node_adj.ensure(ntot + 16); e.t_vert2node.ensure(nverts * ns);
		e.t_corner_vertex.ensure(cotot);
		e.t_dart_end.ensure(4 * ntot); e.t_dart_len.ensure(4 * ntot); e.t_dart_minv.ensure(4 * ntot); e.t_dart_minpos.ensure(4 * ntot);
		e.t_dart_codes.ensure(4 * ntot); e.t_dart_inline.ensure(4 * ntot);
		e.t_parent.ensure(ntot); e.t_compmin.ensure(ntot); e.t_starts.ensure(ntot);
		const uint32_t start_words = static_cast<uint32_t>((nverts + 31) / 32);
		e.t_start_bits.ensure(static_cast<size_t>(start_words) * ns);
		if (!prezeroed) CKL_HIP(hipMemsetAsync(e.t_start_bits.p, 0, static_cast<size_t>(start_words) * ns * sizeof(uint32_t), s));
		e.t_items.ensure(itot); e.t_item_off.ensure(itot); e.t_chain_item0.ensure(ktot);
		e.t_events.ensure(itot); e.t_chain_ev0.ensure(ktot); e.t_ev_lnd.ensure(itot); e.t_ev_item.ensure(itot);
		e.last_trail_slices = ns;

		TrailArgs ta = trail_args(e, sx, sy, ns);
		const FinishArgs fa = finish_args(e, sx, sy, markov_order);
		if (kTuning && getenv("CKL_TRAIL_DIAG")) { d_tdbg.ensure(16); CKL_HIP(hipMemsetAsync(d_tdbg.p, 0, 128, s)); ta.dbg = d_tdbg.p; }
		int max_lds = 0;
		CKL_HIP(hipDeviceGetAttribute(&max_lds, hipDeviceAttributeMaxSharedMemoryPerBlock, e.device));
		const size_t budget = static_cast<size_t>(max_lds > 1024 ? max_lds - 1024 : 0);
		const uint32_t dart_blocks = (4 * max_ncap + kWalkChunk * kWaves - 1) / (kWalkChunk * kWaves);
		size_t clds = (static_cast<size_t>(max_special) + 1024) * 12;
		if (const char* env = getenv("CKL_TRAIL_LDS")) clds = static_cast<size_t>(std::max(0, atoi(env)));
		clds = (std::min(budget, std::max<size_t>(clds, 1024)) / 16) * 16;
		CKL_HIP(hipFuncSetAttribute(reinterpret_cast<const void*>(&k_trail_components), hipFuncAttributeMaxDynamicSharedMemorySize, static_cast<int>(clds)));
		size_t lds = trail_walk_lds(max_special);
		if (const char* env = getenv("CKL_TRAIL_LDS")) lds = static_cast<size_t>(std::max(0, atoi(env)));
		lds = std::min(budget, std::max<size_t>(lds, 4096));
		lds = (lds / 16) * 16;
		CKL_HIP(hipFuncSetAttribute(reinterpret_cast<const void*>(&k_trail_walk), hipFuncAttributeMaxDynamicSharedMemorySize, static_cast<int>(lds)));
		trail_lds_used = lds;
		HT_MARK("c:setup");

		if (any) {
			hipLaunchKernelGGL(k_trail_nodes, dim3(e.graph_blocks, ns), dim3(kBlock), 0, s, ta);
			hipLaunchKernelGGL(k_trail_segments, dim3(dart_blocks, ns), dim3(kBlock), 0, s, ta);
			if (max_cocap) hipLaunchKernelGGL(k_trail_loops, dim3((max_cocap + kBlock - 1) / kBlock, ns), dim3(kBlock), 0, s, ta);
			hipLaunchKernelGGL(k_trail_components, dim3(ns), dim3(kCompBlock), clds, s, ta, static_cast<uint32_t>(clds));
		}
		CKL_HIP(hipEventRecord(e.evd0, s));
		hipLaunchKernelGGL(k_trail_walk, dim3(ns), dim3(kWave), lds, s, ta, static_cast<uint32_t>(lds));
		CKL_HIP(hipEventRecord(e.evd1, s));
		hipLaunchKernelGGL(k_trail_items, dim3(ns), dim3(kItemsBlock), 0, s, ta);
		hipLaunchKernelGGL(k_trail_offsets, dim3(ns), dim3(kBlock), 0, s, ta);
		hipLaunchKernelGGL(k_trail_expand, dim3((max_icap + kExpandChunk * kWaves - 1) / (kExpandChunk * kWaves), ns), dim3(kBlock), 0, s, ta);
		hipLaunchKernelGGL(k_finish, dim3(ns), dim3(kFinishBlock), 0, s, fa);
	}
	HT_MARK("c:enqueue");
	if (kTuning && getenv("CKL_TRAIL_DIAG")) trail_diag(e, ns, d_tdbg.p, max_special, trail_lds_used);

	auto enqueue_tail = [&]() {
		e.d_out_off.ensure(ns);
		e.d_code_report.ensure(static_cast<size_t>(ns) + 3);
		e.d_codes_out.ensure(e.codes_capacity + 8);
		hipLaunchKernelGGL(k_code_offsets, dim3(1), dim3(kBlock), 0, s, e.d_boc_len.p, e.d_payload_len.p, e.d_slice_err.p, ns, e.d_out_off.p, e.d_code_report.p);
		hipLaunchKernelGGL(k_gather_codes, dim3(ns), dim3(kBlock), 0, s, e.d_boc.p, e.d_bbase.p, e.d_boc_len.p,
			e.d_payload.p, e.d_pbase.p, e.d_payload_len.p, e.d_out_off.p, e.d_codes_out.p);
	};
	if (!markov_order) enqueue_tail();
	if (rq.overlap) rq.overlap();
	HT_MARK("c:overlap");

	if (markov_order) {
		if (rq.model) result.model = *rq.model;
		else {
			const size_t rows = static_cast<size_t>(1) << (2 * markov_order);
			e.d_hist.ensure(rows * 4);
			CKL_HIP(hipMemsetAsync(e.d_hist.p, 0, rows * 4 * sizeof(uint32_t), s));
			const uint32_t hist_lds = (rows * 4 <= 16384) ? static_cast<uint32_t>(rows * 4) : 0u;
			if (hist_lds * 4 > 48 * 1024) CKL_HIP(hipFuncSetAttribute(reinterpret_cast<const void*>(&k_markov_hist), hipFuncAttributeMaxDynamicSharedMemorySize, static_cast<int>(hist_lds * 4)));
			hipLaunchKernelGGL(k_markov_hist, dim3(ns), dim3(kBlock), hist_lds * sizeof(uint32_t), s, e.d_dcode.p, e.d_cbase.p, e.d_n_valid.p, markov_order, e.d_hist.p, hist_lds);
			result.hist = download(e.d_hist.p, rows * 4, s);
			if (rq.goal == CrackGoal::HISTOGRAM) { check_walk_errors(e, ns); return result; }
			result.model = markov_stats_to_model(result.hist.data(), rows);
		}
		upload(e.d_model, result.model, s);
		hipLaunchKernelGGL(k_markov_pack, dim3(ns), dim3(kBlock), 0, s, e.d_dcode.p, e.d_cbase.p, e.d_n_valid.p, markov_order,
			e.d_model.p, e.d_pbase.p, e.d_payload.p, e.d_payload_len.p);
		enqueue_tail();
	}
	HT_MARK("c:finish_enq");
	const std::vector<uint32_t> report = download(e.d_code_report.p, static_cast<size_t>(ns) + 3, s);
	HT_MARK("c:finish_wait");
	if (report[ns + 2]) check_walk_errors(e, ns);
	result.code_len.assign(report.begin(), report.begin() + ns);
	result.total = static_cast<uint64_t>(report[ns]) | (static_cast<uint64_t>(report[ns + 1]) << 32);
	return result;
}

struct FlatResult {
	std::vector<uint32_t> ncomp;
	std::vector<uint32_t> crcs;
	uint64_t total = 0;
};

void ensure_geom_table(ckl_encoder& e, uint64_t sxy) {
	if (e.g_table_pixels == sxy && e.d_G.p) return;
	hipStream_t s = e.stream2;
	const uint32_t npx = static_cast<uint32_t>(sxy);
	const uint32_t B = 1024, nblk = npx / B + 1;
	std::vector<uint32_t> g_base(B), blk_g(nblk), blk_x(nblk);
	const uint32_t X = gf_xpow(32);
	g_base[0] = 0;
	for (uint32_t i = 1; i < B; i++) g_base[i] = gf_mul(X, g_base[i - 1] ^ 0x80000000u);
	const uint32_t gB = gf_mul(X, g_base[B - 1] ^ 0x80000000u);
	const uint32_t XB = gf_xpow(32ull * B);
	blk_g[0] = 0; blk_x[0] = 0x80000000u;
	for (uint32_t k = 1; k < nblk; k++) {
		blk_g[k] = blk_g[k - 1] ^ gf_mul(blk_x[k - 1], gB);
		blk_x[k] = gf_mul(blk_x[k - 1], XB);
	}
	DevBuf<uint32_t> t_base, t_g, t_x;
	upload(t_base, g_base, s); upload(t_g, blk_g, s); upload(t_x, blk_x, s);
	e.d_G.ensure(static_cast<size_t>(npx) + 1);
	hipLaunchKernelGGL(k_build_geom_table, dim3(npx / kBlock + 1), dim3(kBlock), 0, s, t_base.p, t_g.p, t_x.p, npx, e.d_G.p);
	CKL_HIP(hipStreamSynchronize(s));
	e.g_table_pixels = sxy;
}

RunArrays flat_arrays(const ckl_encoder& e) {
	RunArrays ra;
	ra.word_base = e.d_word_base.p; ra.rbase = e.d_rbase.p; ra.rcap = e.d_rcap.p;
	ra.parent = e.d_parent.p; ra.run_start = e.d_run_start.p; ra.run_cc = e.d_run_cc.p;
	ra.nruns = e.d_nruns.p; ra.ncomp = e.d_ncomp.p; ra.slice_err = e.d_slice_err2.p;
	ra.comp_pix = e.d_comp_pix.p;
	return ra;
}

void flat_enqueue(ckl_encoder& e, int64_t sx, int64_t sy, int64_t sz) {
	hipStream_t s = e.stream2;
	const uint32_t ns = static_cast<uint32_t>(sz);
	const uint64_t sxy = static_cast<uint64_t>(sx) * sy;
	ensure_geom_table(e, sxy);

	std::vector<uint64_t>& rbase = e.h_rbase;
	std::vector<uint32_t>& rcap = e.h_rcap;
	rbase.assign(ns, 0); rcap.assign(ns, 0);
	uint64_t rtot = 0;
	uint32_t max_rcap = 0;
	for (uint32_t zi = 0; zi < ns; zi++) {
		const uint64_t runs = static_cast<uint64_t>(sy) + e.count_v[zi];
		rbase[zi] = rtot; rcap[zi] = static_cast<uint32_t>(runs); rtot += runs;
		max_rcap = std::max<uint32_t>(max_rcap, static_cast<uint32_t>(runs));
	}
	upload(e.d_rbase, rbase, s); upload(e.d_rcap, rcap, s);
	e.d_word_base.ensure(e.plane_words * ns);
	e.d_parent.ensure(rtot); e.d_run_start.ensure(rtot); e.d_run_cc.ensure(rtot); e.d_comp_pix.ensure(rtot);
	e.d_nruns.ensure(ns);
	e.d_flat_report.ensure(4 * static_cast<size_t>(ns));
	e.d_ncomp.borrow(e.d_flat_report.p, ns); e.d_crc_acc.borrow(e.d_flat_report.p + ns, ns);
	e.d_idbits.borrow(e.d_flat_report.p + 2 * static_cast<size_t>(ns), ns); e.d_slice_err2.borrow(e.d_flat_report.p + 3 * static_cast<size_t>(ns), ns);
	CKL_HIP(hipMemsetAsync(e.d_slice_err2.p, 0, ns * sizeof(uint32_t), s));

	RunGeom g;
	g.planeV = plane_v(e); g.planeH = plane_h(e, ns);
	g.row_words = e.row_words; g.plane_words = e.plane_words;
	g.flip = 1u;
	g.sx = static_cast<uint32_t>(sx); g.sy = static_cast<uint32_t>(sy);
	const RunArrays ra = flat_arrays(e);
	hipLaunchKernelGGL(k_run_index, dim3(ns), dim3(kIndexBlock), 0, s, g, ra);
	launch_run_union(s, ns, g, ra);
	ResolveScratch rs;
	rs.nblk = (max_rcap + kBlock - 1) / kBlock;
	e.d_run_local.ensure(rtot);
	e.d_blk_roots.ensure(static_cast<size_t>(rs.nblk) * ns);
	rs.run_local = e.d_run_local.p; rs.blk_roots = e.d_blk_roots.p;
	launch_run_resolve(s, ns, ra, rs, e.d_G.p, static_cast<uint32_t>(sxy), 0u, e.d_crc_acc.p, e.d_idbits.p);
	HT_MARK("f:enqueue");
}

template <typename LABEL>
void flat_collect(ckl_encoder& e, const LABEL* labels, int64_t sx, int64_t sy, int64_t sz, FlatResult& out) {
	hipStream_t s = e.stream2;
	const uint32_t ns = static_cast<uint32_t>(sz);
	const uint64_t sxy = static_cast<uint64_t>(sx) * sy;
	const std::vector<uint32_t> rep = download(e.d_flat_report.p, 4 * static_cast<size_t>(ns), s);
	const uint32_t *acc = rep.data() + ns, *idbits = rep.data() + 2 * static_cast<size_t>(ns), *errs = rep.data() + 3 * static_cast<size_t>(ns);
	out.ncomp.assign(rep.begin(), rep.begin() + ns);
	HT_MARK("f:wait");
	for (uint32_t zi = 0; zi < ns; zi++) if (errs[zi]) throw Error(CKL_ERR_RUNTIME, "crackle_amd: run table overflow on z=" + std::to_string(zi));
	const uint32_t init_term = gf_mul(0xFFFFFFFFu, gf_xpow(32ull * sxy));
	out.crcs.resize(ns);
	uint32_t fix_bits = 0xFFFFFFFFu, fix = 0;
	for (uint32_t zi = 0; zi < ns; zi++) {
		if (idbits[zi] != fix_bits) { fix_bits = idbits[zi]; fix = gf_xpow(32 - fix_bits); }
		out.crcs[zi] = ~(gf_mul(acc[zi], fix) ^ init_term);
	}

	std::vector<uint64_t> comp_off(ns);
	uint64_t total = 0;
	for (uint32_t zi = 0; zi < ns; zi++) { comp_off[zi] = total; total += out.ncomp[zi]; }
	upload(e.d_comp_off, comp_off, s);
	e.d_mapping.ensure(total + 1);
	const RunArrays ra = flat_arrays(e);
	uint32_t max_ncomp = 1;
	for (uint32_t zi = 0; zi < ns; zi++) max_ncomp = std::max(max_ncomp, out.ncomp[zi]);
	hipLaunchKernelGGL(k_mapping_comps<LABEL>, dim3((max_ncomp + kBlock - 1) / kBlock, ns), dim3(kBlock), 0, s,
		labels, ra, sxy, e.d_comp_off.p, e.d_mapping.p);
	CKL_HIP(hipStreamSynchronize(s));
	out.total = total;
}

uint64_t flat_section(ckl_encoder& e, uint64_t N, int stored_width, int component_width, uint32_t ns, const ckl_encode_overrides* ov = nullptr) {
	hipStream_t s = e.stream2;
	if (N > 0x7FFFFFFFull) throw Error(CKL_ERR_RUNTIME, "crackle_amd: too many components");
	e.d_n_uniq.ensure(2);
	e.d_uniq.ensure(N + 1);
	const uint64_t* sort_src = e.d_mapping.p;
	uint64_t n_sort = N;
	if (N > 8192 && N <= (1ull << 26) && !getenv("CKL_LABEL_SORT_ALL")) {
		uint32_t slots = 16384;
		while (slots < 2 * N) slots <<= 1;
		e.d_label_hash.ensure(slots);
		CKL_HIP(hipMemsetAsync(e.d_label_hash.p, 0xFF, static_cast<size_t>(slots) * sizeof(uint64_t), s));
		CKL_HIP(hipMemsetAsync(e.d_n_uniq.p, 0, 2 * sizeof(uint32_t), s));
		unsigned long long* table = reinterpret_cast<unsigned long long*>(e.d_label_hash.p);
		hipLaunchKernelGGL(k_label_hash_insert, dim3(static_cast<uint32_t>((N + kBlock - 1) / kBlock)), dim3(kBlock), 0, s, e.d_mapping.p, static_cast<uint32_t>(N), table, slots - 1u, e.d_n_uniq.p + 1);
		const uint32_t hb = (slots + kUniqItems - 1) / kUniqItems;
		e.d_uniq_blk.ensure(hb + 1);
		hipLaunchKernelGGL(k_label_hash_count, dim3(hb), dim3(kBlock), 0, s, table, slots, e.d_uniq_blk.p);
		hipLaunchKernelGGL(k_unique_scan, dim3(1), dim3(kBlock), 0, s, e.d_uniq_blk.p, hb, e.d_n_uniq.p);
		hipLaunchKernelGGL(k_label_hash_scatter, dim3(hb), dim3(kBlock), 0, s, table, slots, e.d_uniq_blk.p, e.d_n_uniq.p, e.d_n_uniq.p + 1, e.d_uniq.p);
		const std::vector<uint32_t> found = download(e.d_n_uniq.p, 2, s);
		n_sort = static_cast<uint64_t>(found[0]) + (found[1] ? 1u : 0u);
		if (n_sort == 0 || n_sort > N) throw Error(CKL_ERR_RUNTIME, "crackle_amd: label table pass failed");
		e.d_label_list.ensure(n_sort);
		CKL_HIP(hipMemcpyAsync(e.d_label_list.p, e.d_uniq.p, n_sort * sizeof(uint64_t), hipMemcpyDeviceToDevice, s));
		sort_src = e.d_label_list.p;
	}
	const bool merge_unsorted = ov && ov->merge_unique && sort_src == e.d_label_list.p;
	uint32_t n_pad = 2048;
	while (n_pad < n_sort) n_pad <<= 1;
	if (!merge_unsorted) {
	e.d_sorted.ensure(n_pad);
	const uint32_t blocks = (n_pad + kBlock - 1) / kBlock;
	hipLaunchKernelGGL(k_pad_copy_u64, dim3(blocks), dim3(kBlock), 0, s, sort_src, n_sort, e.d_sorted.p, static_cast<uint64_t>(n_pad));
	hipLaunchKernelGGL(k_bitonic_first, dim3(n_pad / 2048), dim3(kBlock), 0, s, e.d_sorted.p, n_pad);
	for (uint32_t k = 4096; k <= n_pad; k <<= 1) {
		uint32_t j = k >> 1;
		for (; j >= 4096 && !getenv("CKL_BITONIC_SINGLE_STEPS"); j >>= 2) hipLaunchKernelGGL(k_bitonic_step2, dim3((n_pad / 4 + kBlock - 1) / kBlock), dim3(kBlock), 0, s, e.d_sorted.p, j, k, n_pad);
		for (; j >= 2048; j >>= 1) hipLaunchKernelGGL(k_bitonic_step, dim3(blocks), dim3(kBlock), 0, s, e.d_sorted.p, j, k, n_pad);
		hipLaunchKernelGGL(k_bitonic_local, dim3(n_pad / 2048), dim3(kBlock), 0, s, e.d_sorted.p, j, k, n_pad);
	}
	{
		const uint32_t ub = static_cast<uint32_t>((n_sort + kUniqItems - 1) / kUniqItems);
		e.d_uniq_blk.ensure(ub + 1);
		hipLaunchKernelGGL(k_unique_count, dim3(ub), dim3(kBlock), 0, s, e.d_sorted.p, static_cast<uint32_t>(n_sort), e.d_uniq_blk.p);
		hipLaunchKernelGGL(k_unique_scan, dim3(1), dim3(kBlock), 0, s, e.d_uniq_blk.p, ub, e.d_n_uniq.p);
		hipLaunchKernelGGL(k_unique_scatter, dim3(ub), dim3(kBlock), 0, s, e.d_sorted.p, static_cast<uint32_t>(n_sort), e.d_uniq_blk.p, e.d_uniq.p);
	}
	}
	uint64_t uniq_bound = N;
	if (ov && ov->merge_unique) {
		HT_MARK("l:enqueue");
		const uint32_t n_local = merge_unsorted ? static_cast<uint32_t>(n_sort) : download(e.d_n_uniq.p, 1, s)[0];
		std::vector<uint64_t> local = download(merge_unsorted ? e.d_label_list.p : e.d_uniq.p, n_local, s);
		HT_MARK("l:local");
		const uint64_t* merged = nullptr;
		uint64_t n_merged = 0;
		if (ov->merge_unique(ov->merge_ctx, local.data(), n_local, &merged, &n_merged) != 0 || (!merged && n_merged))
			throw Error(CKL_ERR_RUNTIME, "crackle_amd: the merge_unique callback failed");
		HT_MARK("l:merge");
		if (n_merged < n_local || n_merged > 0xFFFFFFFFull) throw Error(CKL_ERR_ARG, "crackle_amd: merge_unique returned a list that cannot contain the slab's labels");
		e.d_uniq.ensure(n_merged + 1);
		if (n_merged) CKL_HIP(hipMemcpyAsync(e.d_uniq.p, merged, n_merged * sizeof(uint64_t), hipMemcpyHostToDevice, s));
		const uint32_t nm = static_cast<uint32_t>(n_merged);
		CKL_HIP(hipMemcpyAsync(e.d_n_uniq.p, &nm, sizeof(uint32_t), hipMemcpyHostToDevice, s));
		CKL_HIP(hipStreamSynchronize(s));
		e.d_labels_bin.ensure(8 + n_merged * static_cast<uint64_t>(stored_width) + static_cast<uint64_t>(ns) * component_width + N * 4 + 16);
		uniq_bound = std::max<uint64_t>(uniq_bound, n_merged);
	}
	e.d_labels_bin.ensure(8 + N * static_cast<uint64_t>(stored_width) + static_cast<uint64_t>(ns) * component_width + N * 4 + 16);
	const uint64_t work = std::max<uint64_t>(std::max<uint64_t>(uniq_bound, ns), 1);
	hipLaunchKernelGGL(k_flat_section, dim3(static_cast<uint32_t>((work + kBlock - 1) / kBlock)), dim3(kBlock), 0, s,
		e.d_uniq.p, e.d_n_uniq.p, stored_width, e.d_ncomp.p, ns, component_width, e.d_mapping.p, static_cast<uint32_t>(N), e.d_labels_bin.p);
	HT_MARK("l:enqueue");
	const uint32_t nu = download(e.d_n_uniq.p, 1, s)[0];
	HT_MARK("l:wait");
	return 8 + static_cast<uint64_t>(nu) * stored_width + static_cast<uint64_t>(ns) * component_width + N * static_cast<uint64_t>(byte_width(nu));
}

Header stream_header(int data_width, int64_t sx, int64_t sy, int64_t sz, const VolumeStats& st, bool allow_pins, bool fortran_order, uint64_t markov_model_order, const ckl_encode_overrides* ov) {
	Header head;
	head.crack_format = IMPERMISSIBLE;
	head.label_format = PINS_VARIABLE_WIDTH;
	if (static_cast<int64_t>(st.pairs) < static_cast<int64_t>(static_cast<uint64_t>(sx) * sy * sz) / 2) {
		head.crack_format = PERMISSIBLE;
		head.label_format = FLAT;
	}
	if (ov && ov->force_crack_format >= 0) {
		head.crack_format = ov->force_crack_format;
		head.label_format = ov->force_crack_format == PERMISSIBLE ? FLAT : PINS_VARIABLE_WIDTH;
	}
	if (sz == 1 || !allow_pins) head.label_format = FLAT;
	if (ov && ov->force_label_format >= 0) head.label_format = ov->force_label_format;
	head.is_signed = false;
	head.data_width = data_width;
	head.stored_data_width = ov && ov->force_stored_width ? ov->force_stored_width : byte_width(st.max_label);
	head.sx = static_cast<uint32_t>(sx); head.sy = static_cast<uint32_t>(sy); head.sz = static_cast<uint32_t>(sz);
	head.log2_grid_size = 31;
	head.fortran_order = fortran_order;
	head.markov_model_order = static_cast<int>(markov_model_order & 0xFF);
	head.is_sorted = true;
	return head;
}
inline std::vector<uint8_t> header_bytes(const Header& head) {
	std::vector<uint8_t> hb;
	head.write(hb);
	return hb;
}

template <typename LABEL>
void encode_typed(
	ckl_encoder& e, const LABEL* labels, int64_t sx, int64_t sy, int64_t sz,
	bool allow_pins, bool fortran_order, uint64_t markov_model_order,
	bool optimize_pins, bool auto_bgcolor, int64_t manual_bgcolor,
	const ckl_encode_overrides* ov, uint8_t** out, uint64_t* out_len
) {
	const uint64_t voxels = static_cast<uint64_t>(sx) * sy * sz;
	hipStream_t s = e.stream;
	CKL_HIP(hipEventRecord(e.ev0, s));

	HostTimer ht;
	g_ht = &ht;
	VolumeStats st;
	e.trail_zeroed = false;
	const bool have_planes = ov && voxels > 0 && planes_cached(e, labels, sx, sy, sz);
	e.planes_for = nullptr;
	const bool labels_first = getenv("CKL_NO_OVERLAP") || static_cast<uint64_t>(sx) * sy > (1536ull * 1536ull)
		|| (getenv("CKL_LABELS_AT_WALK") && atoi(getenv("CKL_LABELS_AT_WALK")) == 0);
	if (voxels > 0 && !have_planes) planes_pass<LABEL>(e, labels, sx, sy, sz, &st, !labels_first);
	else if (have_planes) st = e.planes_stats;
	ht.mark("planes");
	bool graph_done = false;
	if (e.planes_deferred) {
		e.trail_for = nullptr;
		graph_pass(e, sx, sy, sz, ov && ov->force_crack_format >= 0 ? graph_format(ov->force_crack_format == PERMISSIBLE) : GraphFormat::ON_DEVICE, &st);
		graph_done = true;
		ht.mark("graph");
	}
	Header head = stream_header(static_cast<int>(sizeof(LABEL)), sx, sy, sz, st, allow_pins, fortran_order, markov_model_order, ov);
	const int stored_width = head.stored_data_width;
	e.uploads_by_kernel = head.label_format == FLAT;
	if (voxels == 0) { hand_out(header_bytes(head), OutAlloc::MALLOC, out, out_len); return; }
	if (optimize_pins) throw Error(CKL_ERR_ARG, "crackle_amd: allow_pins=2 (find_optimal_pins) is out of scope");
	if (head.label_format != FLAT && head.label_format != PINS_VARIABLE_WIDTH) throw Error(CKL_ERR_ARG, "crackle_amd: unsupported label format");
	if (head.markov_model_order > 13) throw Error(CKL_ERR_ARG, "crackle_amd: markov_model_order > 13 is not supported on device");

	bool labels_at_walk = false;
	if (labels_first && !graph_done) flat_enqueue(e, sx, sy, sz);
	const bool trail_cached = !graph_done && have_planes && ov && ov->has_model && head.markov_model_order > 0 && e.trail_for == static_cast<const void*>(labels)
		&& e.trail_perm == (head.crack_format == PERMISSIBLE) && e.trail_order == head.markov_model_order;
	e.trail_for = nullptr;
	if (graph_done && e.graph_permissible != (head.crack_format == PERMISSIBLE)) throw Error(CKL_ERR_RUNTIME, "crackle_amd: internal: device and host disagree on the crack format");
	if (!trail_cached && !graph_done) graph_pass(e, sx, sy, sz, graph_format(head.crack_format == PERMISSIBLE));
	ht.mark("graph");
	if (!labels_first) {
		uint32_t max_special = 0;
		for (uint32_t v : e.count_special) max_special = std::max(max_special, v);
		int max_lds = 0;
		CKL_HIP(hipDeviceGetAttribute(&max_lds, hipDeviceAttributeMaxSharedMemoryPerBlock, e.device));
		labels_at_walk = max_special < 5000 && 2 * trail_walk_lds(max_special) + 40960 <= static_cast<size_t>(max_lds);
		if (!labels_at_walk) flat_enqueue(e, sx, sy, sz);
	}

	const bool permissible = head.crack_format == PERMISSIBLE;
	{
		bool any = false;
		for (int64_t z = 0; z < sz && !any; z++) any = crack_edges(e, sx, sy, z, permissible) > 0;
		if (!any && !(ov && ov->has_model)) head.markov_model_order = 0;
	}
	std::vector<uint8_t> forced_model;
	CrackRequest crq;
	crq.permissible = permissible;
	crq.markov_order = head.markov_model_order;
	crq.reuse_trail = trail_cached;
	if (ov && ov->has_model && head.markov_model_order > 0) {
		const size_t rows = static_cast<size_t>(1) << (2 * head.markov_model_order);
		forced_model.assign(ov->model, ov->model + rows * 4);
		crq.model = &forced_model;
	}

	FlatResult fr;
	std::vector<uint8_t> pins_binary;
	uint64_t label_bytes = 0;
	const uint64_t off_index = Header::kBytes;
	const uint64_t off_labels = off_index + 4ull * (sz + 1);
	uint64_t est_code_bytes = 0;
	{
		const int xw = byte_width(static_cast<uint64_t>(sx) + 1), yw = byte_width(static_cast<uint64_t>(sy) + 1);
		for (int64_t z = 0; z < sz; z++) {
			const uint64_t codes = crack_edges(e, sx, sy, z, permissible) + 4ull * (static_cast<uint64_t>(e.count_special[z]) + e.count_corner[z]) + 16;
			est_code_bytes += (head.markov_model_order ? (3 * codes + 7) / 8 : (codes + 3) / 4) + 8;
			est_code_bytes += 4 + yw + 64ull * (yw + 2 * xw);
		}
	}
	if (getenv("CKL_SMALL_ESTIMATE")) est_code_bytes = 0;
	const uint64_t model_bytes_est = head.markov_model_order ? (1ull << (2 * head.markov_model_order)) : 0;
	struct HostOut { void* p = nullptr; ~HostOut() { if (p) host_out_free(p); } } early;
	uint64_t early_cap = 0;
	uint32_t labels_crc = 0;
	const int component_width = byte_width(static_cast<uint64_t>(sx) * sy);
	hipStream_t s2 = e.stream2;
	bool labels_stay = false;
	auto label_side = [&]() {
		if (labels_at_walk) {
			CKL_HIP(hipStreamWaitEvent(s2, e.evd0, 0));
			flat_enqueue(e, sx, sy, sz);
		}
		flat_collect<LABEL>(e, labels, sx, sy, sz, fr);
		HT_MARK("flat");
		const uint64_t N = fr.total;
		if (head.label_format == PINS_VARIABLE_WIDTH) {
			if (N > 0xFFFFFFFFull) throw Error(CKL_ERR_RUNTIME, "crackle_amd: too many components");
			e.d_cc_volume.ensure(voxels);
			launch_paint_components(s2, plane_v(e), e.row_words, e.plane_words, sx, sy, sz, e.d_word_base.p, e.d_rbase.p, e.d_run_cc.p, e.d_comp_off.p, 0u, e.d_cc_volume.p);
			pins_binary = pins_section_plain<LABEL>(e, labels, e.d_cc_volume.p, e.d_mapping.p, sx, sy, sz, N, fr.ncomp, head.pin_index_width(), stored_width, auto_bgcolor, manual_bgcolor);
			label_bytes = pins_binary.size();
		}
		else {
			label_bytes = flat_section(e, N, stored_width, component_width, static_cast<uint32_t>(sz), ov);
			HT_MARK("label_table");
			labels_stay = e.async_host_copy && e.keep_device_stream && !e.defer_codes && label_bytes > 0;
			early_cap = off_labels + label_bytes + model_bytes_est + est_code_bytes + 4ull * (sz + 1) + 64;
			early.p = host_out_alloc(early_cap);
			HT_MARK("l:buffer");
			uint8_t* eo = static_cast<uint8_t*>(early.p);
			if (labels_stay) {
				e.d_labels_crc.ensure(1 + kBlock);
				if (!e.ev_labels_crc) CKL_HIP(hipEventCreateWithFlags(&e.ev_labels_crc, hipEventDisableTiming));
				crc32c_device(e.d_labels_bin.p, label_bytes, e.d_labels_crc.p + 1, e.d_labels_crc.p, s2);
				CKL_HIP(hipEventRecord(e.ev_labels_crc, s2));
			}
			else {
				if (label_bytes) CKL_HIP(hipMemcpyAsync(eo + off_labels, e.d_labels_bin.p, label_bytes, hipMemcpyDeviceToHost, s2));
				CKL_HIP(hipStreamSynchronize(s2));
				labels_crc = crc32c(eo + off_labels, label_bytes);
			}
			HT_MARK("labels_d2h");
		}
	};

	const bool no_overlap = getenv("CKL_NO_OVERLAP") != nullptr;
	if (!no_overlap) crq.overlap = label_side;
	const CrackResult cr = crack_pass(e, sx, sy, sz, crq);
	if (no_overlap) label_side();
	ht.mark("cracks");
	std::vector<uint8_t> stored_model;
	if (head.markov_model_order > 0) stored_model = markov_model_to_stored(cr.model);

	head.num_label_bytes = label_bytes;
	const uint64_t off_model = off_labels + label_bytes;
	const uint64_t off_codes = off_model + stored_model.size();
	const uint64_t off_tail = off_codes + cr.total;
	const uint64_t total = off_tail + 4ull * (sz + 1);
	uint8_t* o;
	if (early.p && total <= early_cap) { o = static_cast<uint8_t*>(early.p); early.p = nullptr; }
	else {
		o = static_cast<uint8_t*>(host_out_alloc(total));
		if (early.p && label_bytes) memcpy(o + off_labels, static_cast<uint8_t*>(early.p) + off_labels, label_bytes);
	}
	try {
		e.last_codes_total = cr.total;
		if (head.label_format == PINS_VARIABLE_WIDTH) {
			if (label_bytes) memcpy(o + off_labels, pins_binary.data(), label_bytes);
			labels_crc = crc32c(o + off_labels, label_bytes);
		}
		std::vector<uint8_t> hb;
		head.write(hb);
		memcpy(o, hb.data(), hb.size());
		auto put4 = [&](uint64_t at, uint32_t v) { for (int b = 0; b < 4; b++) o[at + b] = static_cast<uint8_t>((v >> (8 * b)) & 0xFF); };
		for (int64_t z = 0; z < sz; z++) put4(off_index + 4ull * z, cr.code_len[z]);
		put4(off_index + 4ull * sz, crc32c(o + off_index, 4ull * sz));
		if (!stored_model.empty()) memcpy(o + off_model, stored_model.data(), stored_model.size());
		for (int64_t z = 0; z < sz; z++) put4(off_tail + 4 + 4ull * z, fr.crcs[z]);
		put4(off_tail, labels_crc);
		e.device_stream_bytes = 0;
		if (e.keep_device_stream) {
			e.d_stream_out.ensure(total + 16);
			uint8_t* ds = e.d_stream_out.p;
			const void* up = head.label_format == FLAT ? o : nullptr;
			upload_small(ds, o, off_labels, s, up);
			if (label_bytes) {
				if (head.label_format == FLAT) copy_bytes_device(e.d_labels_bin.p, ds + off_labels, label_bytes, s);
				else CKL_HIP(hipMemcpyAsync(ds + off_labels, o + off_labels, label_bytes, hipMemcpyHostToDevice, s));
			}
			if (!stored_model.empty()) upload_small(ds + off_model, o + off_model, stored_model.size(), s, up);
			if (cr.total) copy_bytes_device(e.d_codes_out.p, ds + off_codes, cr.total, s);
			upload_small(ds + off_tail, o + off_tail, 4ull * (sz + 1), s, up);
			if (labels_stay) {
				CKL_HIP(hipStreamWaitEvent(s, e.ev_labels_crc, 0));
				CKL_HIP(hipMemcpyAsync(ds + off_tail, e.d_labels_crc.p, 4, hipMemcpyDeviceToDevice, s));
			}
			e.device_stream_bytes = total;
		}
		if (cr.total && !e.defer_codes) {
			if (e.async_host_copy && e.keep_device_stream) {
				if (!e.stream_copy) CKL_HIP(hipStreamCreateWithFlags(&e.stream_copy, hipStreamNonBlocking));
				if (!e.ev_codes) CKL_HIP(hipEventCreateWithFlags(&e.ev_codes, hipEventDisableTiming));
				CKL_HIP(hipEventRecord(e.ev_codes, s));
				CKL_HIP(hipStreamWaitEvent(e.stream_copy, e.ev_codes, 0));
				CKL_HIP(hipMemcpyAsync(o + off_codes, e.d_codes_out.p, cr.total, hipMemcpyDeviceToHost, e.stream_copy));
				if (labels_stay) {
					CKL_HIP(hipMemcpyAsync(o + off_labels, e.d_labels_bin.p, label_bytes, hipMemcpyDeviceToHost, e.stream_copy));
					CKL_HIP(hipMemcpyAsync(o + off_tail, e.d_labels_crc.p, 4, hipMemcpyDeviceToHost, e.stream_copy));
				}
				e.host_copy_pending = true;
			}
			else CKL_HIP(hipMemcpyAsync(o + off_codes, e.d_codes_out.p, cr.total, hipMemcpyDeviceToHost, s));
		}
		ht.mark("assembly");
		CKL_HIP(hipEventRecord(e.ev1, s));
		CKL_HIP(hipStreamSynchronize(s));
		ht.mark("codes_d2h");
		CKL_HIP(hipGetLastError());
		CKL_HIP(hipEventElapsedTime(&e.pipeline_ms, e.ev0, e.ev1));
		CKL_HIP(hipEventElapsedTime(&e.dominant_ms, e.evd0, e.evd1));
	}
	catch (...) {
		drain_host_copy(e, true);
		host_out_free(o);
		throw;
	}
	*out = o;
	*out_len = total;
}

void reencode_markov(const uint8_t* buf, uint64_t n, int markov_order, int device, uint8_t** out, uint64_t* out_len) {
	if (n < Header::kBytesV0) throw Error(CKL_ERR_FORMAT, "crackle: Input too small to be a valid stream. Bytes: " + std::to_string(n));
	Header head = Header::parse(buf, n);
	if (markov_order < 0 || markov_order > 13) throw Error(CKL_ERR_ARG, "crackle_amd: markov_model_order must be in [0, 13] on device");
	if (head.markov_model_order == markov_order) { hand_out(buf, n, OutAlloc::HOST_OUT, out, out_len); return; }
	const bool v0 = head.format_version == 0;
	const uint64_t sz = head.sz;
	const uint64_t tail_bytes = v0 ? 0 : 4 * (sz + 1);
	const uint64_t off_index = head.header_bytes();
	const uint64_t off_labels = off_index + head.grid_index_bytes();
	if (!head.layout_fits(n)) throw Error(CKL_ERR_RUNTIME, "crackle: get_crack_code_offsets: Unable to read past end of buffer.");
	const uint64_t old_codes = off_labels + head.num_label_bytes + head.markov_model_bytes();
	uint64_t old_tail = old_codes;
	for (uint64_t z = 0; z < sz; z++) old_tail += rd_le(buf + off_index + 4 * z, 4);
	if (old_tail > n || tail_bytes > n - old_tail) throw Error(CKL_ERR_RUNTIME, "crackle: get_crack_codes: Unable to read past end of buffer.");

	const bool prof = getenv("CKL_PROFILE") != nullptr;
	auto t_prev = std::chrono::steady_clock::now();
	auto lap = [&](const char* what) {
		if (!prof) return;
		const auto now = std::chrono::steady_clock::now();
		fprintf(stderr, "[ckl reencode host ms] %s=%.2f\n", what, std::chrono::duration<double, std::milli>(now - t_prev).count());
		t_prev = now;
	};
	struct DecoderGuard { ckl_decoder* d = nullptr; ~DecoderGuard() { if (d) ckl_decoder_destroy(d); } } dec;
	struct EncoderGuard { ckl_encoder* e = nullptr; ~EncoderGuard() { if (e) ckl_encoder_destroy(e); } } enc;
	if (ckl_decoder_create(buf, n, 0, -1, device, &dec.d) != CKL_OK) throw Error(CKL_ERR_RUNTIME, ckl_last_error());
	lap("decoder_create");
	CrackResult cr;
	std::vector<uint8_t> stored_model;
	head.markov_model_order = markov_order;
	if (head.voxels() > 0) {
		const uint32_t *cv = nullptr, *ch = nullptr;
		uint32_t row_words = 0;
		uint64_t plane_words = 0;
		if (ckl_decoder_crack_planes(dec.d, &cv, &ch, &row_words, &plane_words) != CKL_OK) throw Error(CKL_ERR_RUNTIME, ckl_last_error());
		lap("crack_planes");
		if (ckl_encoder_create(head.sx, head.sy, head.sz, 1, device, &enc.e) != CKL_OK) throw Error(CKL_ERR_RUNTIME, ckl_last_error());
		lap("encoder_create");
		ckl_encoder& e = *enc.e;
		hipStream_t s = e.stream;
		const uint32_t ns = head.sz;
		const bool permissible = head.crack_format == PERMISSIBLE;
		e.row_words = row_words;
		e.plane_words = plane_words;
		e.d_planes.ensure(2 * plane_words * ns);
		e.d_count_vh.ensure(4 * static_cast<size_t>(ns));
		CKL_HIP(hipMemsetAsync(e.d_count_vh.p, 0, 2 * static_cast<size_t>(ns) * sizeof(uint32_t), s));
		hipLaunchKernelGGL(k_planes_from_cracks, dim3(static_cast<uint32_t>((plane_words + kBlock - 1) / kBlock), ns), dim3(kBlock), 0, s,
			cv, ch, head.sx, head.sy, row_words, plane_words, permissible ? 1u : 0u,
			plane_v(e), plane_h(e, ns), e.d_count_vh.p, ns);
		std::vector<uint32_t> c = download(e.d_count_vh.p, 2 * static_cast<size_t>(ns), s);
		e.count_v.assign(c.begin(), c.begin() + ns);
		e.count_h.assign(c.begin() + ns, c.end());
		lap("planes");
		graph_pass(e, head.sx, head.sy, head.sz, graph_format(permissible));
		lap("graph");
		CrackRequest crq;
		crq.permissible = permissible;
		crq.markov_order = markov_order;
		cr = crack_pass(e, head.sx, head.sy, head.sz, crq);
		lap("cracks");
		if (markov_order > 0) stored_model = markov_model_to_stored(cr.model);
	}
	else cr.code_len.assign(sz, 0);

	const uint64_t off_model = off_labels + head.num_label_bytes;
	const uint64_t off_codes = off_model + stored_model.size();
	const uint64_t off_tail = off_codes + cr.total;
	const uint64_t total = off_tail + tail_bytes;
	uint8_t* o = static_cast<uint8_t*>(host_out_alloc(total));
	try {
		if (cr.total) CKL_HIP(hipMemcpyAsync(o + off_codes, enc.e->d_codes_out.p, cr.total, hipMemcpyDeviceToHost, enc.e->stream));
		std::vector<uint8_t> hb;
		head.write(hb);
		memcpy(o, hb.data(), hb.size());
		auto put4 = [&](uint64_t at, uint32_t v) { for (int b = 0; b < 4; b++) o[at + b] = static_cast<uint8_t>((v >> (8 * b)) & 0xFF); };
		for (uint64_t z = 0; z < sz; z++) put4(off_index + 4 * z, cr.code_len[z]);
		if (!v0) put4(off_index + 4 * sz, crc32c(o + off_index, 4 * sz));
		memcpy(o + off_labels, buf + off_labels, head.num_label_bytes);
		if (!stored_model.empty()) memcpy(o + off_model, stored_model.data(), stored_model.size());
		if (tail_bytes) memcpy(o + off_tail, buf + old_tail, tail_bytes);
		if (cr.total) CKL_HIP(hipStreamSynchronize(enc.e->stream));
		lap("assembly");
	}
	catch (...) { host_out_free(o); throw; }
	*out = o;
	*out_len = total;
}

void check_dims(int64_t sx, int64_t sy, int64_t sz, int dtype_bytes, int is_signed) {
	if (is_signed) throw Error(CKL_ERR_ARG, "Signed integer data types are not currently supported.");
	if (dtype_bytes != 1 && dtype_bytes != 2 && dtype_bytes != 4 && dtype_bytes != 8) throw Error(CKL_ERR_ARG, "crackle_amd: dtype width must be 1, 2, 4 or 8 bytes");
	if (sx < 0 || sy < 0 || sz < 0) throw Error(CKL_ERR_ARG, "crackle_amd: negative dimension");
	if (sx > 0x7FFFFFF0ll || sy > 0x7FFFFFF0ll || sz > 0x7FFFFFF0ll) throw Error(CKL_ERR_ARG, "crackle_amd: dimension too large");
	if (static_cast<uint64_t>(sx + 1) * static_cast<uint64_t>(sy + 1) >= (1ull << 30)) throw Error(CKL_ERR_ARG, "crackle_amd: slices of 2^30 or more crack vertices are not supported");
}

}

extern "C" {

int ckl_encoder_create(int64_t sx, int64_t sy, int64_t sz, int dtype_bytes, int device, ckl_encoder** out) {
	return guard([&] {
		if (!out) throw Error(CKL_ERR_ARG, "crackle_amd: null argument");
		check_dims(sx, sy, sz, dtype_bytes, 0);
		select_device(device);
		std::unique_ptr<ckl_encoder> e(new ckl_encoder());
		e->device = device;
		e->dtype_bytes = dtype_bytes;
		CKL_HIP(hipStreamCreateWithFlags(&e->stream, hipStreamNonBlocking));
		{
			int lo = 0, hi = 0;
			CKL_HIP(hipDeviceGetStreamPriorityRange(&lo, &hi));
			CKL_HIP(hipStreamCreateWithPriority(&e->stream2, hipStreamNonBlocking, hi));
		}
		CKL_HIP(hipEventCreate(&e->ev0));
		CKL_HIP(hipEventCreate(&e->ev1));
		CKL_HIP(hipEventCreate(&e->evd0));
		CKL_HIP(hipEventCreate(&e->evd1));
		CKL_HIP(hipEventCreateWithFlags(&e->ev_in, hipEventDisableTiming));
		CKL_HIP(hipEventCreateWithFlags(&e->ev_prezero, hipEventDisableTiming));
		*out = e.release();
	});
}

int ckl_encoder_run(
	ckl_encoder* e, const void* labels_device, int64_t sx, int64_t sy, int64_t sz,
	int allow_pins, int fortran_order, uint64_t markov_model_order,
	int optimize_pins, int auto_bgcolor, int64_t manual_bgcolor,
	const ckl_encode_overrides* overrides, uint8_t** out, uint64_t* out_len
) {
	return guard([&] {
		if (!e || !out || !out_len) throw Error(CKL_ERR_ARG, "crackle_amd: null argument");
		check_dims(sx, sy, sz, e->dtype_bytes, 0);
		if (markov_model_order > 15) throw Error(CKL_ERR_ARG, "crackle_amd: markov_model_order must be in [0, 15]");
		enter(e);
		drain_host_copy(*e);
		const auto t_run0 = std::chrono::steady_clock::now();
		with_label_type(e->dtype_bytes, [&](auto t) {
			encode_typed(*e, static_cast<const typename decltype(t)::type*>(labels_device), sx, sy, sz, allow_pins != 0, fortran_order != 0,
				markov_model_order, optimize_pins != 0, auto_bgcolor != 0, manual_bgcolor, overrides, out, out_len);
		});
		if (getenv("CKL_PROFILE")) {
			fprintf(stderr, "[ckl encoder_run ms] encode=%.2f\n", std::chrono::duration<double, std::milli>(std::chrono::steady_clock::now() - t_run0).count());
		}
	});
}

int ckl_reencode_markov(const uint8_t* buf, uint64_t n, int markov_model_order, int device, uint8_t** out, uint64_t* out_len) {
	return guard([&] {
		if (!buf || !out || !out_len) throw Error(CKL_ERR_ARG, "crackle_amd: null argument");
		select_device(device);
		reencode_markov(buf, n, markov_model_order, device, out, out_len);
	});
}

int ckl_encoder_defer_codes(ckl_encoder* e, int defer) {
	if (!e) { set_last_error("crackle_amd: null encoder"); return CKL_ERR_ARG; }
	e->defer_codes = defer != 0;
	return CKL_OK;
}

int ckl_encoder_async_host_copy(ckl_encoder* e, int on) {
	if (!e) { set_last_error("crackle_amd: null encoder"); return CKL_ERR_ARG; }
	e->async_host_copy = on != 0;
	return CKL_OK;
}

int ckl_encoder_host_wait(ckl_encoder* e) {
	return guard([&] {
		if (!e) throw Error(CKL_ERR_ARG, "crackle_amd: null encoder");
		if (e->host_copy_pending) select_device(e->device);
		drain_host_copy(*e);
	});
}

int ckl_encoder_keep_device_stream(ckl_encoder* e, int keep) {
	if (!e) { set_last_error("crackle_amd: null encoder"); return CKL_ERR_ARG; }
	e->keep_device_stream = keep != 0;
	return CKL_OK;
}

int ckl_encoder_device_stream(const ckl_encoder* e, const uint8_t** stream_device, uint64_t* n_bytes) {
	if (!e || !stream_device || !n_bytes) { set_last_error("crackle_amd: null argument"); return CKL_ERR_ARG; }
	if (!e->device_stream_bytes) { set_last_error("crackle_amd: no device-resident stream (ckl_encoder_keep_device_stream before the run)"); return CKL_ERR_ARG; }
	*stream_device = e->d_stream_out.p;
	*n_bytes = e->device_stream_bytes;
	return CKL_OK;
}

int ckl_encoder_codes_to_host(ckl_encoder* e, uint8_t* dst_host, uint64_t capacity, uint64_t* n_bytes) {
	return guard([&] {
		if (!e || !n_bytes) throw Error(CKL_ERR_ARG, "crackle_amd: null argument");
		*n_bytes = e->last_codes_total;
		if (e->last_codes_total == 0) return;
		if (!dst_host || capacity < e->last_codes_total) throw Error(CKL_ERR_ARG, "crackle_amd: code buffer too small: need " + std::to_string(e->last_codes_total) + " bytes");
		select_device(e->device);
		if (e->async_host_copy) {
			if (!e->stream_copy) CKL_HIP(hipStreamCreateWithFlags(&e->stream_copy, hipStreamNonBlocking));
			CKL_HIP(hipMemcpyAsync(dst_host, e->d_codes_out.p, e->last_codes_total, hipMemcpyDeviceToHost, e->stream_copy));
			e->host_copy_pending = true;
			return;
		}
		CKL_HIP(hipMemcpyAsync(dst_host, e->d_codes_out.p, e->last_codes_total, hipMemcpyDeviceToHost, e->stream));
		CKL_HIP(hipStreamSynchronize(e->stream));
	});
}

int ckl_encoder_stats(
	ckl_encoder* e, const void* labels_device, int64_t sx, int64_t sy, int64_t sz,
	uint64_t* max_label, uint64_t* pixel_pairs, uint64_t* first_voxel, uint64_t* last_voxel
) {
	return guard([&] {
		enter(e);
		check_dims(sx, sy, sz, e->dtype_bytes, 0);
		const uint64_t voxels = static_cast<uint64_t>(sx) * sy * sz;
		VolumeStats st;
		e->planes_for = nullptr;
		if (voxels > 0) {
			uint64_t f = 0, l = 0;
			const uint8_t* base = static_cast<const uint8_t*>(labels_device);
			struct Drain { hipStream_t s; ~Drain() { (void)hipStreamSynchronize(s); } } drain{ e->stream };
			CKL_HIP(hipMemcpyAsync(&f, base, e->dtype_bytes, hipMemcpyDeviceToHost, e->stream));
			CKL_HIP(hipMemcpyAsync(&l, base + (voxels - 1) * e->dtype_bytes, e->dtype_bytes, hipMemcpyDeviceToHost, e->stream));
			planes_pass_any(*e, labels_device, sx, sy, sz, &st);
			CKL_HIP(hipStreamSynchronize(e->stream));
			st.first = f; st.last = l;
			e->planes_for = labels_device;
			e->planes_stats = st;
			e->planes_dims[0] = sx; e->planes_dims[1] = sy; e->planes_dims[2] = sz;
		}
		if (max_label) *max_label = st.max_label;
		if (pixel_pairs) *pixel_pairs = st.pairs;
		if (first_voxel) *first_voxel = st.first;
		if (last_voxel) *last_voxel = st.last;
	});
}

int ckl_encoder_markov_stats(
	ckl_encoder* e, const void* labels_device, int64_t sx, int64_t sy, int64_t sz,
	int crack_format, uint64_t markov_model_order, uint32_t* hist
) {
	return guard([&] {
		if (!e || !hist) throw Error(CKL_ERR_ARG, "crackle_amd: null argument");
		check_dims(sx, sy, sz, e->dtype_bytes, 0);
		if (markov_model_order == 0 || markov_model_order > 13) throw Error(CKL_ERR_ARG, "crackle_amd: markov_model_order must be in [1, 13]");
		enter(e);
		const size_t rows = static_cast<size_t>(1) << (2 * markov_model_order);
		std::vector<uint32_t> h(rows * 4, 0);
		if (static_cast<uint64_t>(sx) * sy * sz > 0) {
			CrackRequest crq;
			crq.goal = CrackGoal::HISTOGRAM;
			crq.permissible = crack_format == PERMISSIBLE;
			crq.markov_order = static_cast<int>(markov_model_order);
			const bool cached = planes_cached(*e, labels_device, sx, sy, sz);
			if (!cached) planes_pass_any(*e, labels_device, sx, sy, sz, nullptr);
			e->trail_for = nullptr;
			graph_pass(*e, sx, sy, sz, graph_format(crq.permissible));
			h = crack_pass(*e, sx, sy, sz, crq).hist;
			if (cached) { e->trail_for = labels_device; e->trail_perm = crq.permissible; e->trail_order = crq.markov_order; }
		}
		memcpy(hist, h.data(), h.size() * sizeof(uint32_t));
	});
}

static uint32_t* encoder_components(ckl_encoder* e, const void* labels_device, int64_t sx, int64_t sy, int64_t sz, uint32_t id_base, uint32_t* cc_device, uint32_t* ncomp_host) {
	check_dims(sx, sy, sz, e->dtype_bytes, 0);
	enter(e);
	const uint64_t voxels = static_cast<uint64_t>(sx) * sy * sz;
	if (voxels == 0) return cc_device;
	FlatResult fr;
	if (!planes_cached(*e, labels_device, sx, sy, sz)) planes_pass_any(*e, labels_device, sx, sy, sz, nullptr);
	flat_enqueue(*e, sx, sy, sz);
	with_label_type(e->dtype_bytes, [&](auto t) { flat_collect(*e, static_cast<const typename decltype(t)::type*>(labels_device), sx, sy, sz, fr); });
	if (fr.total + id_base > 0xFFFFFFFFull) throw Error(CKL_ERR_RUNTIME, "crackle_amd: too many components");
	hipStream_t s2 = e->stream2;
	if (!cc_device) { e->d_cc_volume.ensure(voxels); cc_device = e->d_cc_volume.p; }
	launch_paint_components(s2, plane_v(*e), e->row_words, e->plane_words, sx, sy, sz, e->d_word_base.p, e->d_rbase.p, e->d_run_cc.p, e->d_comp_off.p, id_base, cc_device);
	for (int64_t z = 0; z < sz; z++) ncomp_host[z] = fr.ncomp[z];
	return cc_device;
}

int ckl_encoder_components(
	ckl_encoder* e, const void* labels_device, int64_t sx, int64_t sy, int64_t sz,
	uint32_t id_base, uint32_t* cc_host, uint32_t* ncomp_host
) {
	return guard([&] {
		if (!e || !cc_host || !ncomp_host) throw Error(CKL_ERR_ARG, "crackle_amd: null argument");
		const uint32_t* cc = encoder_components(e, labels_device, sx, sy, sz, id_base, nullptr, ncomp_host);
		const uint64_t voxels = static_cast<uint64_t>(sx) * sy * sz;
		if (voxels) CKL_HIP(hipMemcpyAsync(cc_host, cc, voxels * sizeof(uint32_t), hipMemcpyDeviceToHost, e->stream2));
		CKL_HIP(hipStreamSynchronize(e->stream2));
	});
}

int ckl_encoder_components_device(
	ckl_encoder* e, const void* labels_device, int64_t sx, int64_t sy, int64_t sz,
	uint32_t id_base, uint32_t* cc_device, uint32_t* ncomp_host
) {
	return guard([&] {
		if (!e || !cc_device || !ncomp_host) throw Error(CKL_ERR_ARG, "crackle_amd: null argument");
		encoder_components(e, labels_device, sx, sy, sz, id_base, cc_device, ncomp_host);
		CKL_HIP(hipStreamSynchronize(e->stream2));
	});
}

int ckl_encoder_last_timing(const ckl_encoder* e, float* pipeline_ms, float* dominant_kernel_ms) {
	if (!e) { set_last_error("crackle_amd: null encoder"); return CKL_ERR_ARG; }
	if (pipeline_ms) *pipeline_ms = e->pipeline_ms;
	if (dominant_kernel_ms) *dominant_kernel_ms = e->dominant_ms;
	return CKL_OK;
}

int ckl_encoder_walk_paths(ckl_encoder* e, uint32_t* fast_slices, uint32_t* compiled_slices) {
	return guard([&] {
		if (!e) throw Error(CKL_ERR_ARG, "crackle_amd: null encoder");
		uint32_t fast = 0, plain = 0;
		const size_t ns = e->last_trail_slices;
		if (ns && e->t_counters.p) {
			select_device(e->device);
			std::vector<uint32_t> nev(ns);
			CKL_HIP(hipMemcpy(nev.data(), e->t_counters.p + 5 * ns, ns * sizeof(uint32_t), hipMemcpyDeviceToHost));
			for (uint32_t v : nev) { if (v & (kEvFormatAddr12 | kEvWalkWide)) fast++; else if (v) plain++; }
		}
		if (fast_slices) *fast_slices = fast;
		if (compiled_slices) *compiled_slices = plain;
	});
}

int ckl_encoder_walk_step_kinds(ckl_encoder* e, uint32_t* counts, uint32_t max_slices, uint32_t* n_slices) {
	return guard([&] {
		if (!e || !counts || !n_slices) throw Error(CKL_ERR_ARG, "crackle_amd: null argument");
		const size_t ns = e->last_trail_slices;
		*n_slices = static_cast<uint32_t>(ns);
		if (!ns || !e->t_counters.p || !e->t_events.p) { *n_slices = 0; return; }
		if (ns > max_slices) throw Error(CKL_ERR_ARG, "crackle_amd: counts holds fewer slices than the last run had");
		select_device(e->device);
		DevBuf<uint32_t> d_counts;
		d_counts.ensure(ns * 5);
		hipLaunchKernelGGL(k_trail_step_kinds, dim3(static_cast<uint32_t>(ns)), dim3(kBlock), 0, e->stream, e->t_events.p, e->t_ibase.p, e->t_counters.p + 5 * ns, d_counts.p);
		CKL_HIP(hipMemcpyAsync(counts, d_counts.p, ns * 5 * sizeof(uint32_t), hipMemcpyDeviceToHost, e->stream));
		CKL_HIP(hipStreamSynchronize(e->stream));
	});
}

void ckl_encoder_destroy(ckl_encoder* e) { delete e; }

int ckl_compress(
	const void* labels, int labels_mem, int dtype_bytes, int is_signed,
	int64_t sx, int64_t sy, int64_t sz,
	int allow_pins, int fortran_order, uint64_t markov_model_order,
	int optimize_pins, int auto_bgcolor, int64_t manual_bgcolor,
	int device, uint8_t** out, uint64_t* out_len
) {
	ckl_encoder* e = nullptr;
	try {
		check_dims(sx, sy, sz, dtype_bytes, is_signed);
		if (!out || !out_len) throw Error(CKL_ERR_ARG, "crackle_amd: null argument");
		if (static_cast<uint64_t>(sx) * sy * sz == 0) {
			hand_out(header_bytes(stream_header(dtype_bytes, sx, sy, sz, VolumeStats(), allow_pins != 0, fortran_order != 0, markov_model_order, nullptr)), OutAlloc::MALLOC, out, out_len);
			return CKL_OK;
		}
	}
	catch (const Error& err) { set_last_error(err.what()); return err.status; }
	const int rc = ckl_encoder_create(sx, sy, sz, dtype_bytes, device, &e);
	if (rc != CKL_OK) return rc;
	const EncoderPtr owner(e);
	return guard([&]() -> int {
		const uint64_t bytes = static_cast<uint64_t>(sx) * sy * sz * dtype_bytes;
		const void* dev_labels = labels;
		DevBuf<uint8_t> tmp;
		if (labels_mem == CKL_MEM_HOST && bytes) {
			if (!labels) throw Error(CKL_ERR_ARG, "crackle_amd: null labels");
			tmp.ensure(bytes);
			CKL_HIP(hipMemcpy(tmp.p, labels, bytes, hipMemcpyHostToDevice));
			dev_labels = tmp.p;
		}
		return ckl_encoder_run(e, dev_labels, sx, sy, sz, allow_pins, fortran_order, markov_model_order,
			optimize_pins, auto_bgcolor, manual_bgcolor, nullptr, out, out_len);
	});
}

}
```

### crackle_amd/csrc/ckl_encoder.hpp

```cpp
#pragma once

#include "ckl_common.hpp"

#include <chrono>
#include <utility>

struct VolumeStats { uint64_t max_label = 0, pairs = 0, first = 0, last = 0; };

struct ckl_encoder {
	template <typename T> using DevBuf = ckl::DevBuf<T>;

	int device = 0;
	hipStream_t stream = nullptr;
	hipStream_t stream2 = nullptr;
	hipEvent_t ev0 = nullptr, ev1 = nullptr, ev_in = nullptr;
	hipEvent_t evd0 = nullptr, evd1 = nullptr;
	hipEvent_t ev_prezero = nullptr;
	float pipeline_ms = 0.f, dominant_ms = 0.f;
	int dtype_bytes = 0;

	DevBuf<unsigned long long> d_stats;
	DevBuf<uint4> d_adjm;
	DevBuf<uint32_t> d_slice_err;
	DevBuf<uint64_t> d_cbase, d_sbase, d_kbase, d_pbase, d_bbase, d_out_off, d_comp_off;
	DevBuf<uint32_t> d_ccap, d_scap, d_kcap;
	DevBuf<uint8_t> d_crack_tables;
	DevBuf<uint8_t> d_cp, d_fcode, d_dcode, d_payload, d_boc, d_codes_out, d_model;
	DevBuf<uint32_t> d_code_report;
	uint64_t codes_capacity = 0;
	bool defer_codes = false;
	bool keep_device_stream = false;
	bool async_host_copy = false;
	bool host_copy_pending = false;
	hipStream_t stream_copy = nullptr;
	hipStream_t stream_tab = nullptr;
	hipEvent_t ev_codes = nullptr;
	void* tables_staging = nullptr;
	bool uploads_by_kernel = false;
	hipEvent_t ev_labels_crc = nullptr;
	DevBuf<uint32_t> d_labels_crc;
	DevBuf<uint8_t> d_stream_out;
	uint64_t device_stream_bytes = 0;
	uint64_t last_codes_total = 0;
	DevBuf<uint32_t> d_stack_node, d_stack_code;
	DevBuf<uint32_t> d_chain_node, d_chain_off, d_chain_clen, d_chain_order, d_chain_dst, d_chain_vstart;
	DevBuf<uint32_t> d_n_chains, d_n_raw, d_n_valid, d_payload_len, d_boc_len;
	DevBuf<uint32_t> d_hist;
	DevBuf<uint32_t> d_planes, d_count_vh;
	uint32_t row_words = 0;
	uint64_t plane_words = 0;
	std::vector<uint32_t> count_v, count_h;
	DevBuf<uint64_t> d_rbase;
	DevBuf<uint32_t> d_rcap, d_word_base, d_parent, d_run_start, d_run_cc, d_comp_pix, d_nruns, d_ncomp, d_idbits, d_blk_roots;
	DevBuf<uint16_t> d_run_local;
	DevBuf<uint32_t> d_G, d_crc_acc;
	DevBuf<uint32_t> d_flat_report;
	uint64_t g_table_pixels = 0;
	DevBuf<uint64_t> d_mapping, d_sorted, d_uniq, d_label_hash, d_label_list;
	DevBuf<uint32_t> d_cc_volume;
	DevBuf<uint32_t> d_pin_kept, d_pin_u32;
	DevBuf<uint8_t> d_pin_tables;
	DevBuf<uint64_t> d_pin_u64;
	DevBuf<uint32_t> d_slice_err2, d_n_uniq, d_uniq_blk;
	DevBuf<uint8_t> d_labels_bin;
	const void* planes_for = nullptr;
	const void* trail_for = nullptr;
	bool trail_perm = false;
	int trail_order = 0;
	VolumeStats planes_stats;
	int64_t planes_dims[3] = { 0, 0, 0 };
	std::vector<uint64_t> h_rbase;
	std::vector<uint32_t> h_rcap;
	std::vector<uint32_t> count_special, count_corner;
	DevBuf<uint32_t> d_plane_partial, t_blk_special, t_blk_corner;
	DevBuf<unsigned long long> d_plane_partial_max, d_plane_out;
	uint32_t graph_blocks = 0;
	uint32_t tiles_x = 0, tiles_y = 0, mtx2 = 0;
	uint64_t adjm_stride = 0;
	bool graph_permissible = false;
	bool planes_deferred = false;
	bool trail_zeroed = false;
	DevBuf<uint64_t> t_nbase, t_cobase, t_ibase;
	DevBuf<uint32_t> t_ncap, t_cocap, t_icap, t_max_steps;
	size_t last_trail_slices = 0;
	DevBuf<uint32_t> t_counters;
	DevBuf<uint32_t> t_node_vertex, t_vert2node, t_corner_vertex;
	DevBuf<uint8_t> t_node_adj;
	DevBuf<uint32_t> t_dart_end, t_dart_len, t_dart_minv, t_dart_minpos, t_parent, t_start_bits, t_starts;
	DevBuf<uint4> t_dart_codes;
	DevBuf<uint8_t> t_dart_inline;
	DevBuf<unsigned long long> t_compmin;
	DevBuf<uint32_t> t_items, t_item_off, t_chain_item0, t_events, t_chain_ev0, t_ev_lnd, t_ev_item;

	~ckl_encoder() {
		if (ev0) (void)hipEventDestroy(ev0);
		if (ev1) (void)hipEventDestroy(ev1);
		if (evd0) (void)hipEventDestroy(evd0);
		if (evd1) (void)hipEventDestroy(evd1);
		if (ev_in) (void)hipEventDestroy(ev_in);
		if (ev_prezero) (void)hipEventDestroy(ev_prezero);
		if (stream) (void)hipStreamDestroy(stream);
		if (stream2) (void)hipStreamDestroy(stream2);
		if (stream_copy) { (void)hipStreamSynchronize(stream_copy); (void)hipStreamDestroy(stream_copy); }
		if (stream_tab) { (void)hipStreamSynchronize(stream_tab); (void)hipStreamDestroy(stream_tab); }
		if (ev_codes) (void)hipEventDestroy(ev_codes);
		if (tables_staging) ckl::host_out_free(tables_staging);
		if (ev_labels_crc) (void)hipEventDestroy(ev_labels_crc);
	}
};

namespace ckl {

template <typename T>
inline std::vector<T> download(const T* p, size_t n, hipStream_t s) {
	std::vector<T> h(n);
	if (n) CKL_HIP(hipMemcpyAsync(h.data(), p, n * sizeof(T), hipMemcpyDeviceToHost, s));
	CKL_HIP(hipStreamSynchronize(s));
	return h;
}

struct HostTimer {
	bool on;
	std::chrono::steady_clock::time_point t0;
	std::vector<std::pair<const char*, double>> marks;
	HostTimer() : on(getenv("CKL_PROFILE") != nullptr), t0(std::chrono::steady_clock::now()) {}
	void mark(const char* name) {
		if (!on) return;
		auto t1 = std::chrono::steady_clock::now();
		marks.emplace_back(name, std::chrono::duration<double, std::milli>(t1 - t0).count());
		t0 = t1;
	}
	~HostTimer();
};
inline thread_local HostTimer* g_ht = nullptr;
#define HT_MARK(name) do { if (g_ht) g_ht->mark(name); } while (0)
inline HostTimer::~HostTimer() {
		g_ht = nullptr;
		if (!on) return;
		fprintf(stderr, "[ckl encode host ms]");
		for (auto& m : marks) fprintf(stderr, " %s=%.2f", m.first, m.second);
		fprintf(stderr, "\n");
}

inline void enter(ckl_encoder* e) {
	if (!e) throw Error(CKL_ERR_ARG, "crackle_amd: null encoder");
	select_device(e->device);
	wait_for_default_stream(e->stream, e->ev_in);
	wait_for_default_stream(e->stream2, e->ev_in);
}

inline void drain_host_copy(ckl_encoder& e, bool quiet = false) {
	if (!e.host_copy_pending) return;
	if (quiet) (void)hipStreamSynchronize(e.stream_copy);
	else CKL_HIP(hipStreamSynchronize(e.stream_copy));
	e.host_copy_pending = false;
}

enum class OutAlloc { MALLOC, HOST_OUT };
inline void hand_out(const uint8_t* bytes, size_t n, OutAlloc how, uint8_t** out, uint64_t* out_len) {
	uint8_t* p = static_cast<uint8_t*>(how == OutAlloc::MALLOC ? malloc(n ? n : 1) : host_out_alloc(n ? n : 1));
	if (!p) throw Error(CKL_ERR_RUNTIME, "crackle_amd: out of host memory");
	if (n) memcpy(p, bytes, n);
	*out = p;
	*out_len = n;
}
inline void hand_out(const std::vector<uint8_t>& bin, OutAlloc how, uint8_t** out, uint64_t* out_len) { hand_out(bin.data(), bin.size(), how, out, out_len); }

template <typename LABEL>
std::vector<uint8_t> pins_section_plain(
	ckl_encoder& e, const LABEL* labels, const uint32_t* cc, const uint64_t* comp_label, int64_t sx, int64_t sy, int64_t sz, uint64_t N,
	const std::vector<uint32_t>& nc, int index_width, int stored_width, bool auto_bgcolor, int64_t manual_bgcolor);

}
```

### crackle_amd/csrc/ckl_strips.hpp

```cpp
#pragma once

#include "ckl_runs.hpp"
#include <type_traits>

namespace ckl {
namespace dev {

constexpr uint32_t kStripWords = 1024;
constexpr uint32_t kStripCap = 2560;
constexpr uint32_t kStripRunsPerThread = kStripCap / kBlock;
constexpr uint32_t kStripBitmapWords = kStripCap / 32;
constexpr uint32_t kStripEdgeCap = kStripWords + kStripCap / 2;
constexpr uint32_t kStripOverflow = 0xFFFFFFFFu;
constexpr int kResolveBlock = 1024;
constexpr uint32_t kResolveCap = 0xFFFFu;
constexpr uint32_t kMaxStrips = 1024;

struct StripArrays {
	uint16_t* run_lid;
	uint32_t* sc_w;
	uint32_t* sc_cc;
	void* sc_label;
	uint32_t* strip_nruns;
	uint32_t* strip_nsc;
	uint16_t* row_run;
	uint16_t* seam_first;
	uint16_t* seam_last;
	uint32_t* slice_err;
	uint32_t* overflow;
	uint32_t nstrips, strip_rows;
	uint32_t cap;
	uint32_t zbase;
};

__device__ __forceinline__ void strip_of_block(uint32_t& zi_local, uint32_t& k) {
	const uint32_t total = gridDim.x * gridDim.y, i = blockIdx.y * gridDim.x + blockIdx.x;
	const uint32_t body = total & ~7u;
	const uint32_t c = i < body ? (i & 7u) * (body >> 3) + (i >> 3) : i;
	zi_local = c / gridDim.x;
	k = c - zi_local * gridDim.x;
}

__device__ __forceinline__ uint32_t strip_lid(const uint16_t* slot_lids, uint32_t nsc, uint32_t j) {
	return nsc <= 256u ? reinterpret_cast<const uint8_t*>(slot_lids)[j] : slot_lids[j];
}

struct RecordLists {
	uint4* rec;
	uint32_t* count;
	uint32_t cap;
	uint32_t nstrips, strip_rows;
	uint32_t strip_shift;
	uint32_t strip_magic;
	__device__ __forceinline__ uint32_t strip_of(uint32_t y) const { return strip_shift != 0xFFFFFFFFu ? y >> strip_shift : __umulhi(y, strip_magic); }
};

__device__ __forceinline__ void raster_record(
	const uint4 rec, uint32_t y0, uint32_t rows, uint32_t sx, uint32_t sy, uint32_t rw, uint32_t* sV, uint32_t* sH, uint32_t& bad
) {
	uint32_t p = rec.x;
	const uint32_t jump = rec.z & 0xAAAAAAAAu;
#pragma unroll
	for (uint32_t k = 0; k < 16; k++) {
		if ((jump >> (2u * k + 1u)) & 1u) p += rec.w;
		if (((rec.z >> (2u * k)) & 1u) == 0u) continue;
		const uint32_t kind = (rec.y >> (2u * k)) & 3u;
		const uint32_t horiz = kind & 1u;
		const uint32_t unit = horiz ? 1u : 0x10000u;
		const uint32_t neg = ((kind ^ (kind >> 1)) & 1u) ^ 1u;
		const uint32_t q = neg ? p - unit : p + unit;
		const uint32_t c = p < q ? p : q;
		const uint32_t col = c & 0xFFFFu, row = c >> 16;
		const uint32_t qx = q & 0xFFFFu, qy = q >> 16;
		if (qx > sx || qy > sy) bad |= 1u;
		else {
			const bool ok = horiz ? (row - 1u < sy - 1u && col < sx) : (col - 1u < sx - 1u && row < sy);
			const uint32_t rel = row - y0;
			if (ok && rel < rows) atomicOr((horiz ? sH : sV) + rel * rw + (col >> 5), 1u << (col & 31u));
		}
		p = q;
	}
}

__device__ __forceinline__ void raster_half_record(
	const uint4 rec, uint32_t h, uint32_t y0, uint32_t y1, uint32_t rlo_h, uint32_t sx, uint32_t sy, uint32_t rw, uint32_t* lds_v, uint32_t* lds_h, uint32_t& bad
) {
	constexpr uint32_t kLo = 0x55555555u;
	uint32_t p = rec.x;
	uint32_t kinds = rec.y, flags = rec.z;
	if (h) {
		const uint32_t ms = flags & kLo & 0xFFFFu, pv = kinds;
		const uint32_t mR = ms & ~(pv >> 1) & pv, mL = ms & (pv >> 1) & pv, mD = ms & (pv >> 1) & ~pv, mU = ms & ~(pv >> 1) & ~pv;
		p += __popc(mR) - __popc(mL) + ((__popc(mD) - __popc(mU)) << 16);
		if (flags & 0xAAAAu) p += rec.w;
		kinds >>= 16; flags >>= 16;
	}
#pragma unroll
	for (uint32_t k = 0; k < 8; k++) {
		const uint32_t j = (flags >> (2u * k + 1u)) & 1u;
		p += rec.w & (0u - j);
		const uint32_t e = (flags >> (2u * k)) & 1u;
		const uint32_t kind = (kinds >> (2u * k)) & 3u;
		const uint32_t horiz = kind & 1u;
		const uint32_t neg = ((kind ^ (kind >> 1)) & 1u) ^ 1u;
		const uint32_t unit = horiz ? 1u : 0x10000u;
		const uint32_t d = ((unit ^ (0u - neg)) + neg) & (0u - e);
		const uint32_t q = p + d;
		const uint32_t c = p < q ? p : q;
		const uint32_t col = c & 0xFFFFu, row = c >> 16;
		bad |= ((q & 0xFFFFu) > sx || (q >> 16) > sy) ? 1u : 0u;
		const uint32_t rlo = horiz ? rlo_h : y0, clo = horiz ? 0u : 1u;
		const bool ok = e != 0u && (row - rlo) <= (y1 - 1u - rlo) && row >= rlo && (col - clo) <= (sx - 1u - clo) && col >= clo;
		uint32_t* base = horiz ? lds_h : lds_v;
		const uint32_t at = ok ? (row - y0) * rw + (col >> 5) : 0u;
		atomicOr(base + at, ok ? (1u << (col & 31u)) : 0u);
		p = q;
	}
}

constexpr uint32_t kStripCclWords = (kStripCap + kStripEdgeCap + kStripWords / 2 + 2 * kStripBitmapWords + kWaves + 2 + 7) & ~7u;
template <bool DIAG, bool RECORDS>
__device__ __forceinline__ void strip_ccl_body(
	const RunGeom& g, const StripArrays& sa, const RecordLists& rl, const uint32_t* __restrict__ G, uint32_t n_pixels, unsigned long long* __restrict__ diag,
	uint32_t zi, uint32_t k, uint32_t* lds
) {
	uint32_t* s_parent = lds;
	uint32_t* s_mem = s_parent + kStripCap;
	uint16_t* s_wb = reinterpret_cast<uint16_t*>(s_mem + kStripEdgeCap);
	uint32_t* s_b = s_mem;
	uint16_t* s_pool = reinterpret_cast<uint16_t*>(s_mem + kStripWords);
	uint32_t* s_bm = s_mem + kStripEdgeCap + kStripWords / 2;
	uint32_t* s_bmbase = s_bm + kStripBitmapWords;
	uint32_t* s_scan = s_bmbase + kStripBitmapWords;
	uint32_t* s_misc = s_scan + kWaves;
	static_assert((kStripCap * 4) % 16 == 0 && (kStripEdgeCap * 4) % 16 == 0, "tables stay 16-byte aligned");
	unsigned long long d_t = DIAG ? __builtin_amdgcn_s_memtime() : 0ull;
	auto stamp = [&](int slot) {
		if (DIAG && threadIdx.x == 0) {
			const unsigned long long now = __builtin_amdgcn_s_memtime();
			atomicAdd(diag + slot, now - d_t);
			d_t = now;
		}
	};
	const uint32_t rw = g.row_words;
	const uint32_t t = threadIdx.x;
	const uint32_t si = zi * sa.nstrips + k;
	const uint32_t y0 = k * sa.strip_rows;
	const uint32_t y1 = min(y0 + sa.strip_rows, g.sy);
	const uint32_t nw = (y1 - y0) * rw;
	const uint64_t slot = static_cast<uint64_t>(si) * sa.cap;
	uint32_t b[4], up[4], upl[4], cnt = 0;
	if (RECORDS) {
		static_assert(kStripCap >= kStripWords, "plane H piece is built in the union-find table");
		uint32_t* sV = s_mem;
		uint32_t* sH = s_parent;
		const uint32_t n_rec = min(rl.count[si], rl.cap);
		const uint4* list = rl.rec + static_cast<uint64_t>(si) * rl.cap;
		uint4 first = list[(t >> 1) < rl.cap ? (t >> 1) : 0u];
#pragma unroll
		for (uint32_t j = 0; j < 4; j++) { sV[t * 4u + j] = 0u; sH[t * 4u + j] = 0u; }
		__syncthreads();
		uint32_t bad = 0;
		{
			const uint32_t half = t & 1u, rlo_h = y0 ? y0 : 1u;
			if ((t >> 1) < n_rec) raster_half_record(first, half, y0, y1, rlo_h, g.sx, g.sy, rw, sV, sH, bad);
			for (uint32_t r = (t >> 1) + kBlock / 2u; r < n_rec; r += kBlock / 2u) raster_half_record(list[r], half, y0, y1, rlo_h, g.sx, g.sy, rw, sV, sH, bad);
		}
		if (bad) atomicOr(sa.slice_err + zi, ERR_RANGE);
		__syncthreads();
		stamp(5);
		const uint4 v4 = *reinterpret_cast<const uint4*>(sV + t * 4u);
		const uint4 h4 = *reinterpret_cast<const uint4*>(sH + t * 4u);
		b[0] = v4.x; b[1] = v4.y; b[2] = v4.z; b[3] = v4.w;
		up[0] = h4.x; up[1] = h4.y; up[2] = h4.z; up[3] = h4.w;
		upl[0] = sH[t ? t * 4u - 1u : 0u];
		if (t * 4u < nw) {
			uint32_t* pv = const_cast<uint32_t*>(g.planeV) + zi * g.plane_words + static_cast<uint64_t>(y0) * rw;
			uint32_t* ph = const_cast<uint32_t*>(g.planeH) + zi * g.plane_words + static_cast<uint64_t>(y0) * rw;
			if (t * 4u + 4u <= nw) {
				*reinterpret_cast<uint4*>(pv + t * 4u) = v4;
				*reinterpret_cast<uint4*>(ph + t * 4u) = h4;
			}
			else {
				for (uint32_t j = 0; t * 4u + j < nw; j++) { pv[t * 4u + j] = b[j]; ph[t * 4u + j] = up[j]; }
			}
		}
		__syncthreads();
	}
	else {
		const uint32_t* pv = g.planeV + zi * g.plane_words + static_cast<uint64_t>(y0) * rw;
		const uint32_t* ph = g.planeH + zi * g.plane_words + static_cast<uint64_t>(y0) * rw;
#pragma unroll
		for (uint32_t j = 0; j < 4; j++) {
			const uint32_t wl = t * 4u + j;
			const uint32_t at = wl < nw ? wl : 0u;
			b[j] = pv[at];
			up[j] = ph[at];
		}
		upl[0] = ph[(t * 4u < nw && t) ? t * 4u - 1u : 0u];
	}
	uint32_t w[4];
	{
		const uint32_t yy = (t * 4u) / rw;
		uint32_t ww = t * 4u - yy * rw;
#pragma unroll
		for (uint32_t j = 0; j < 4; j++) { w[j] = ww; if (++ww == rw) ww = 0; }
	}
	upl[0] = (w[0] && t * 4u >= rw && t * 4u < nw) ? g.ups_of(upl[0], w[0] - 1u) : 0u;
#pragma unroll
	for (uint32_t j = 0; j < 4; j++) {
		const uint32_t wl = t * 4u + j;
		b[j] = wl < nw ? g.breaks_of(b[j], w[j]) : 0u;
		up[j] = (wl >= rw && wl < nw) ? g.ups_of(up[j], w[j]) : 0u;
		cnt += __popc(b[j]);
	}
#pragma unroll
	for (uint32_t j = 1; j < 4; j++) upl[j] = w[j] ? up[j - 1] : 0u;
	uint32_t v[1] = { cnt }, tot[1];
	block_excl_add<1>(v, tot, s_scan);
	const uint32_t nloc = tot[0];
	if (nloc > sa.cap) {
		if (t == 0) { sa.strip_nruns[si] = kStripOverflow; sa.strip_nsc[si] = 0u; atomicOr(sa.overflow, 1u); }
		return;
	}
	stamp(0);
	{
		uint32_t local = v[0];
		uint32_t px = ((t * 4u) / rw) * g.sx;
#pragma unroll
		for (uint32_t j = 0; j < 4; j++) {
			const uint32_t wl = t * 4u + j;
			if (j && w[j] == 0) px += g.sx;
			if (wl < nw) {
				s_b[wl] = b[j];
				s_wb[wl] = static_cast<uint16_t>(local);
				for (uint32_t m = b[j]; m; m &= m - 1u) s_pool[local++] = static_cast<uint16_t>(px + w[j] * 32u + (__ffs(m) - 1u));
			}
		}
	}
	for (uint32_t j = t; j < nloc; j += kBlock) s_parent[j] = j;
	if (t < kStripBitmapWords) s_bm[t] = 0u;
	__syncthreads();
	stamp(1);
	uint32_t gv[kStripRunsPerThread];
	{
		const uint32_t p0 = y0 * g.sx;
#pragma unroll
		for (uint32_t i = 0; i < kStripRunsPerThread; i++) {
			const uint32_t j = t + i * kBlock;
			gv[i] = G[n_pixels - (p0 + s_pool[j < nloc ? j : 0u])];
		}
	}
	{
		uint32_t yy = (t * 4u) / rw;
#pragma unroll
		for (uint32_t j = 0; j < 4; j++) {
			const uint32_t wl = t * 4u + j;
			if (j && w[j] == 0) yy++;
			if (wl >= nw) break;
			const uint16_t wbv = s_wb[wl];
			if (w[j] == 0) sa.row_run[static_cast<uint64_t>(zi) * g.sy + y0 + yy] = wbv;
			if (wl < rw) sa.seam_first[static_cast<uint64_t>(si) * rw + wl] = wbv;
			if (wl + rw >= nw) sa.seam_last[static_cast<uint64_t>(si) * rw + (wl + rw - nw)] = wbv;
		}
	}
	{
		uint32_t c[4], b_up[4], base_up[4], base_here[4], n_e = 0;
#pragma unroll
		for (uint32_t j = 0; j < 4; j++) {
			const uint32_t wl = t * 4u + j;
			const uint32_t above = up[j] ? wl - rw : 0u;
			b_up[j] = s_b[above]; base_up[j] = s_wb[above]; base_here[j] = s_wb[wl < nw ? wl : 0u];
			c[j] = up[j] & (~((up[j] << 1) | (upl[j] >> 31)) | b[j] | b_up[j]);
			n_e += __popc(c[j]);
		}
		uint32_t ve[1] = { n_e }, te[1];
		block_excl_add<1>(ve, te, s_scan);
		const uint32_t n_edges = te[0];
		if (n_edges <= kStripEdgeCap) {
			uint32_t at = ve[0];
#pragma unroll
			for (uint32_t j = 0; j < 4; j++) {
				for (uint32_t cc = c[j]; cc; cc &= cc - 1u) {
					const uint32_t m = mask_le(__ffs(cc) - 1u);
					s_mem[at++] = (base_here[j] + __popc(b[j] & m) - 1u) | ((base_up[j] + __popc(b_up[j] & m) - 1u) << 16);
				}
			}
			__syncthreads();
			for (uint32_t e = t; e < n_edges; e += kBlock) { const uint32_t pr = s_mem[e]; sm_unite(s_parent, pr & 0xFFFFu, pr >> 16); }
		}
		else {
#pragma unroll
			for (uint32_t j = 0; j < 4; j++) {
				for (uint32_t cc = c[j]; cc; cc &= cc - 1u) {
					const uint32_t m = mask_le(__ffs(cc) - 1u);
					sm_unite(s_parent, base_here[j] + __popc(b[j] & m) - 1u, base_up[j] + __popc(b_up[j] & m) - 1u);
				}
			}
		}
	}
	__syncthreads();
	stamp(2);
	uint32_t root[kStripRunsPerThread];
#pragma unroll
	for (uint32_t i = 0; i < kStripRunsPerThread; i++) {
		const uint32_t j = t + i * kBlock;
		root[i] = j < nloc ? sm_find(s_parent, j) : 0u;
		if (j < nloc && root[i] == j) atomicOr(s_bm + (j >> 5), 1u << (j & 31u));
	}
	__syncthreads();
	if (t < kWave) {
		static_assert(kStripBitmapWords <= 2 * kWave, "two bitmap words per lane");
		const uint32_t c0 = t < kStripBitmapWords ? __popc(s_bm[t]) : 0u;
		const uint32_t c1 = t + kWave < kStripBitmapWords ? __popc(s_bm[t + kWave]) : 0u;
		const uint32_t i0 = wave_incl_add(c0);
		const uint32_t tot0 = __shfl(i0, kWave - 1, kWave);
		const uint32_t i1 = wave_incl_add(c1);
		if (t < kStripBitmapWords) s_bmbase[t] = i0 - c0;
		if (t + kWave < kStripBitmapWords) s_bmbase[t + kWave] = tot0 + i1 - c1;
		if (t == kWave - 1) s_misc[1] = tot0 + i1;
	}
	__syncthreads();
	const uint32_t nsc = s_misc[1];
	uint16_t* lid_out = sa.run_lid + slot;
	const bool narrow = nsc <= 256u;
#pragma unroll
	for (uint32_t i = 0; i < kStripRunsPerThread; i++) {
		const uint32_t j = t + i * kBlock;
		if (j >= nloc) break;
		const uint32_t r = root[i];
		const uint32_t lid = s_bmbase[r >> 5] + __popc(s_bm[r >> 5] & ((1u << (r & 31u)) - 1u));
		s_pool[j] = static_cast<uint16_t>(lid);
		if (narrow) reinterpret_cast<uint8_t*>(lid_out)[j] = static_cast<uint8_t>(lid);
		else lid_out[j] = static_cast<uint16_t>(lid);
	}
	for (uint32_t j = t; j < nsc; j += kBlock) s_parent[j] = 0u;
	__syncthreads();
	stamp(3);
#pragma unroll
	for (uint32_t i = 0; i < kStripRunsPerThread; i++) {
		const uint32_t j = t + i * kBlock;
		if (j >= nloc) break;
		atomicXor(s_parent + s_pool[j], gv[i]);
		if (j) atomicXor(s_parent + s_pool[j - 1], gv[i]);
	}
	if (t == 0 && nloc) atomicXor(s_parent + s_pool[nloc - 1], G[n_pixels - y1 * g.sx]);
	__syncthreads();
	uint32_t* w_out = sa.sc_w + slot;
	for (uint32_t j = t; j < nsc; j += kBlock) w_out[j] = s_parent[j];
	if (t == 0) { sa.strip_nruns[si] = nloc; sa.strip_nsc[si] = nsc; }
	stamp(4);
}

template <bool DIAG, bool RECORDS>
static __global__ void __launch_bounds__(kBlock, 7) k_strip_ccl(RunGeom g, StripArrays sa, RecordLists rl, const uint32_t* __restrict__ G, uint32_t n_pixels, unsigned long long* __restrict__ diag) {
	__shared__ __attribute__((aligned(16))) uint32_t s_lds[kStripCclWords];
	strip_ccl_body<DIAG, RECORDS>(g, sa, rl, G, n_pixels, diag, blockIdx.y + sa.zbase, blockIdx.x, s_lds);
}

struct ResolveArgs {
	uint32_t idbits, crc_fix, check_crc;
	const uint32_t* crc_expect;
	const uint32_t* ncomp_expect;
	const uint64_t* comp_off;
	const uint64_t* label_map;
	const uint8_t* keys;
	const uint8_t* uniq;
	uint32_t key_width, stored_width, is_signed;
	uint64_t num_unique;
	uint32_t has_label;
	uint64_t label;
	uint32_t cap;
	uint32_t* host_flags;
	uint32_t host_flags_n;
};

template <int W>
__device__ __forceinline__ uint64_t ld_le(const uint8_t* p) {
	if constexpr (W == 1) return *p;
	else if constexpr (W == 2) { uint16_t v; __builtin_memcpy(&v, p, 2); return v; }
	else if constexpr (W == 4) { uint32_t v; __builtin_memcpy(&v, p, 4); return v; }
	else { uint64_t v; __builtin_memcpy(&v, p, 8); return v; }
}
template <typename F>
__device__ __forceinline__ void with_width(uint32_t w, F&& f) {
	switch (w) {
		case 1: f(std::integral_constant<int, 1>{}); break;
		case 2: f(std::integral_constant<int, 2>{}); break;
		case 4: f(std::integral_constant<int, 4>{}); break;
		default: f(std::integral_constant<int, 8>{}); break;
	}
}

template <typename OUT, bool LABELS, bool DIAG>
__device__ __forceinline__ bool slice_resolve_body(
	const RunGeom& g, const StripArrays& sa, const ResolveArgs& ra, uint32_t* __restrict__ ncomp_out, unsigned long long* __restrict__ diag,
	uint32_t zi, uint32_t* s_tab, uint32_t* s_scbase, uint32_t* s_scan, uint32_t* s_flag_p
) {
	uint32_t& s_flag = *s_flag_p;
	static_assert(kResolveCap <= 0xFFFFu, "index and rank share a table entry");
	constexpr int NW = kResolveBlock / kWave;
	unsigned long long d_t = DIAG ? __builtin_amdgcn_s_memtime() : 0ull;
	auto stamp = [&](int slot) {
		if (DIAG && threadIdx.x == 0) {
			const unsigned long long now = __builtin_amdgcn_s_memtime();
			atomicAdd(diag + slot, now - d_t);
			d_t = now;
		}
	};
	const uint32_t t = threadIdx.x;
	const uint32_t ns = sa.nstrips;
	const uint32_t rw = g.row_words;
	const uint32_t si0 = zi * ns;
	const uint32_t items = (ns - 1u) * rw;
	constexpr uint32_t kSeamPer = 2;
	uint32_t q_up[kSeamPer], q_prev[kSeamPer], q_bh[kSeamPer], q_bu[kSeamPer], q_wh[kSeamPer], q_wu[kSeamPer];
	auto seam_load = [&](uint32_t it0) {
#pragma unroll
		for (uint32_t u = 0; u < kSeamPer; u++) {
			const uint32_t it_raw = it0 + u * kResolveBlock + t;
			const uint32_t it = it_raw < items ? it_raw : 0u;
			const uint32_t seam = it / rw, w = it - seam * rw;
			const uint32_t k = seam + 1u, y = k * sa.strip_rows;
			const uint64_t at = zi * g.plane_words + static_cast<uint64_t>(y) * rw + w;
			const uint32_t h = g.planeH[at], hp = g.planeH[w ? at - 1u : at];
			const uint32_t vh = g.planeV[at], vu = g.planeV[at - rw];
			q_wh[u] = sa.seam_first[static_cast<uint64_t>(si0 + k) * rw + w];
			q_wu[u] = sa.seam_last[static_cast<uint64_t>(si0 + k - 1u) * rw + w];
			q_up[u] = it_raw < items ? g.ups_of(h, w) : 0u;
			q_prev[u] = w ? (g.ups_of(hp, w - 1u) >> 31) : 0u;
			q_bh[u] = g.breaks_of(vh, w); q_bu[u] = g.breaks_of(vu, w);
		}
	};
	if (items) seam_load(0);
	uint32_t my_nsc = 0;
	if (t == 0) s_flag = 0;
	__syncthreads();
	if (t < ns) {
		const uint32_t nr = sa.strip_nruns[si0 + t];
		if (nr == kStripOverflow) s_flag = 1;
		my_nsc = sa.strip_nsc[si0 + t];
	}
	uint32_t v[1] = { my_nsc }, tot[1];
	block_excl_add<1, NW>(v, tot, s_scan);
	if (t < ns) s_scbase[t] = v[0];
	if (t == 0) s_scbase[ns] = tot[0];
	const uint32_t total = tot[0];
	__syncthreads();
	if (s_flag || total > ra.cap) {
		if (t == 0) {
			atomicOr(sa.overflow, s_flag ? 1u : 2u);
			if (ra.host_flags) { ra.host_flags[ra.host_flags_n + (s_flag ? 0u : 1u)] = 1u; ra.host_flags[zi] = sa.slice_err[zi]; }
		}
		return false;
	}
	for (uint32_t i = t; i < total; i += kResolveBlock) s_tab[i] = i;
	__syncthreads();
	stamp(0);
	for (uint32_t it0 = 0; it0 < items; it0 += kSeamPer * kResolveBlock) {
		if (it0) seam_load(it0);
#pragma unroll
		for (uint32_t u = 0; u < kSeamPer; u++) {
			if (!q_up[u]) continue;
			const uint32_t it = it0 + u * kResolveBlock + t;
			const uint32_t k = it / rw + 1u;
			const uint16_t* lid_h = sa.run_lid + static_cast<uint64_t>(si0 + k) * sa.cap;
			const uint16_t* lid_u = sa.run_lid + static_cast<uint64_t>(si0 + k - 1u) * sa.cap;
			const uint32_t nsc_h = s_scbase[k + 1u] - s_scbase[k], nsc_u = s_scbase[k] - s_scbase[k - 1u];
			for (uint32_t c = q_up[u] & (~((q_up[u] << 1) | q_prev[u]) | q_bh[u] | q_bu[u]); c; c &= c - 1u) {
				const uint32_t m = mask_le(__ffs(c) - 1u);
				const uint32_t jh = q_wh[u] + __popc(q_bh[u] & m) - 1u, ju = q_wu[u] + __popc(q_bu[u] & m) - 1u;
				if (jh >= sa.cap || ju >= sa.cap) continue;
				const uint32_t lh = strip_lid(lid_h, nsc_h, jh), lu = strip_lid(lid_u, nsc_u, ju);
				if (lh < nsc_h && lu < nsc_u) sm_unite(s_tab, s_scbase[k] + lh, s_scbase[k - 1u] + lu);
			}
		}
	}
	__syncthreads();
	stamp(1);
	const uint32_t per = (total + kResolveBlock - 1) / kResolveBlock;
	const uint32_t i0 = min(total, t * per), i1 = min(total, i0 + per);
	for (uint32_t i = i0; i < i1; i++) sm_store(s_tab, i, sm_find(s_tab, i));
	__syncthreads();
	uint32_t nroot = 0;
	for (uint32_t i = i0; i < i1; i++) nroot += s_tab[i] == i ? 1u : 0u;
	constexpr uint32_t kPer = 4;
	uint32_t strip0 = 0;
	if (i0 < i1) {
		uint32_t lo = 0, hi = ns;
		while (lo + 1 < hi) { const uint32_t mid = (lo + hi) >> 1; if (s_scbase[mid] <= i0) lo = mid; else hi = mid; }
		strip0 = lo;
	}
	uint32_t v2[1] = { nroot }, tot2[1];
	block_excl_add<1, NW>(v2, tot2, s_scan);
	{
		uint32_t rk = v2[0];
		for (uint32_t i = i0; i < i1; i++) if (s_tab[i] == i) s_tab[i] = i | (rk++ << 16);
	}
	__syncthreads();
	stamp(2);
	const uint32_t ncomp = tot2[0];
	const uint32_t nexp = ra.ncomp_expect[zi];
	const uint64_t coff = ra.comp_off[zi];
	uint32_t part = 0;
	uint32_t sidx = strip0;
	for (uint32_t r0 = i0; r0 < i1; r0 += kPer) {
		uint32_t cc[kPer], wgt[kPer];
		uint64_t gi[kPer], key[kPer];
#pragma unroll
		for (uint32_t q = 0; q < kPer; q++) {
			const uint32_t i = r0 + q;
			const bool on = i < i1;
			const uint32_t ii = on ? i : i0;
			if (on) while (sidx + 1 < ns && s_scbase[sidx + 1] <= ii) sidx++;
			const uint32_t sq = on ? sidx : strip0;
			gi[q] = static_cast<uint64_t>(si0 + sq) * sa.cap + (ii - s_scbase[sq]);
			cc[q] = s_tab[s_tab[ii] & 0xFFFFu] >> 16;
			wgt[q] = sa.sc_w[gi[q]];
			key[q] = 0;
		}
		uint64_t lab[kPer];
		if (LABELS) {
			with_width(ra.key_width, [&](auto W) {
#pragma unroll
				for (uint32_t q = 0; q < kPer; q++) key[q] = ld_le<decltype(W)::value>(ra.keys + (coff + (cc[q] < nexp ? cc[q] : 0u)) * static_cast<uint64_t>(decltype(W)::value));
			});
#pragma unroll
			for (uint32_t q = 0; q < kPer; q++) lab[q] = 0;
			if (ra.num_unique) {
				with_width(ra.stored_width, [&](auto W) {
#pragma unroll
					for (uint32_t q = 0; q < kPer; q++) lab[q] = ld_le<decltype(W)::value>(ra.uniq + (key[q] < ra.num_unique ? key[q] : 0ull) * static_cast<uint64_t>(decltype(W)::value));
				});
			}
		}
#pragma unroll
		for (uint32_t q = 0; q < kPer; q++) {
			if (r0 + q >= i1) continue;
			if (LABELS) {
				uint64_t val = 0;
				if (cc[q] < nexp && key[q] < ra.num_unique) {
					val = lab[q];
					if (ra.is_signed && ra.stored_width < 8u && (val >> (8u * ra.stored_width - 1u))) val |= ~0ull << (8u * ra.stored_width);
				}
				if (ra.has_label) val = (val == ra.label);
				static_cast<OUT*>(sa.sc_label)[gi[q]] = static_cast<OUT>(val);
			}
			else sa.sc_cc[gi[q]] = cc[q];
			uint32_t wg = wgt[q];
			for (int j = static_cast<int>(ra.idbits) - 1; j >= 0; j--) {
				part ^= ((cc[q] >> j) & 1u) ? wg : 0u;
				wg = (wg >> 1) ^ ((wg & 1u) ? kCrcPoly : 0u);
			}
		}
	}
	part = wave_xor(part);
	if ((t & (kWave - 1)) == 0) s_scan[t >> 6] = part;
	__syncthreads();
	if (t == 0) {
		uint32_t x = 0;
		for (int wv = 0; wv < NW; wv++) x ^= s_scan[wv];
		uint32_t e = 0;
		if (ncomp != nexp) e |= ERR_NCOMP;
		else if (ra.check_crc && gf_mul(x, ra.crc_fix) != ra.crc_expect[zi]) e |= ERR_CRC;
		if (e) atomicOr(sa.slice_err + zi, e);
		ncomp_out[zi] = ncomp;
		if (ra.host_flags) ra.host_flags[zi] = sa.slice_err[zi] | e;
	}
	stamp(3);
	return true;
}

template <typename OUT, bool LABELS, bool DIAG>
static __global__ void __launch_bounds__(kResolveBlock, 8) k_slice_resolve(RunGeom g, StripArrays sa, ResolveArgs ra, uint32_t* __restrict__ ncomp_out, unsigned long long* __restrict__ diag) {
	extern __shared__ __attribute__((aligned(16))) uint32_t s_tab[];
	__shared__ uint32_t s_scbase[kMaxStrips + 1];
	__shared__ uint32_t s_scan[kResolveBlock / kWave];
	__shared__ uint32_t s_flag;
	slice_resolve_body<OUT, LABELS, DIAG>(g, sa, ra, ncomp_out, diag, blockIdx.x + sa.zbase, s_tab, s_scbase, s_scan, &s_flag);
}

template <typename OUT>
static __global__ void __launch_bounds__(kBlock) k_strip_labels(StripArrays sa, ResolveArgs ra) {
	const uint32_t zi = blockIdx.y + sa.zbase;
	const uint32_t si = zi * sa.nstrips + blockIdx.x;
	if (sa.strip_nruns[si] == kStripOverflow) return;
	const uint32_t n = min(sa.strip_nsc[si], sa.cap);
	const uint32_t nexp = ra.ncomp_expect[zi];
	const uint64_t coff = ra.comp_off[zi];
	const uint64_t slot = static_cast<uint64_t>(si) * sa.cap;
	for (uint32_t j = threadIdx.x; j < n; j += kBlock) {
		const uint32_t c = sa.sc_cc[slot + j];
		uint64_t val = c < nexp ? ra.label_map[coff + c] : 0ull;
		if (ra.has_label) val = (val == ra.label);
		static_cast<OUT*>(sa.sc_label)[slot + j] = static_cast<OUT>(val);
	}
}

__device__ __forceinline__ uint32_t strip_component_of_pixel(const RunGeom& g, const StripArrays& sa, uint32_t zi, uint32_t x, uint32_t y) {
	const uint32_t k = y / sa.strip_rows;
	const uint32_t si = zi * sa.nstrips + k;
	const uint32_t nr = sa.strip_nruns[si];
	if (nr == kStripOverflow) return 0xFFFFFFFFu;
	uint32_t run = sa.row_run[static_cast<uint64_t>(zi) * g.sy + y];
	const uint32_t wx = x >> 5;
	for (uint32_t w = 0; w < wx; w++) run += __popc(g.breaks(zi, y, w));
	run += __popc(g.breaks(zi, y, wx) & mask_le(x & 31u)) - 1u;
	if (run >= nr || run >= sa.cap) return 0xFFFFFFFFu;
	const uint64_t slot = static_cast<uint64_t>(si) * sa.cap;
	const uint32_t lid = strip_lid(sa.run_lid + slot, sa.strip_nsc[si], run);
	return lid < sa.cap ? sa.sc_cc[slot + lid] : 0xFFFFFFFFu;
}

}
}
```

Before: 157.5 billion.

## Label flat slices with LDS strip CCL plus slice resolve in the encoder

Adds an encoder path that labels each z-slice's connected components through per-strip union-find in LDS (reusing the decoder's strip CCL, parameterized by capacity), followed by a per-slice resolve kernel. That kernel also gathers each component's label value into slots and computes the CRC partial. This replaces the global run-index/union/resolve chain and the separate mapping kernel when strip capacity allows and labels run beside the walk. Overflow falls back to a retry with a larger resolve capacity, then to the old run path. The risks are extra host logic, fallback cost on dense slices, and a fixed 16-bit id width in the CRC.

Result: faster. 161.7 billion, median of 6 (+2.7%).

```diff
diff --git a/crackle_amd/csrc/ckl_encode.hip b/crackle_amd/csrc/ckl_encode.hip
--- a/crackle_amd/csrc/ckl_encode.hip
+++ b/crackle_amd/csrc/ckl_encode.hip
@@ -1,5 +1,6 @@
 #include "ckl_encoder.hpp"
 #include "ckl_runs.hpp"
+#include "ckl_strips.hpp"
 #include "ckl_trail.hpp"
 
 #include <algorithm>
@@ -624,6 +625,22 @@
 	mapping[comp_off[zi] + c] = static_cast<uint64_t>(labels[zi * sxy + r.comp_pix[r.rbase[zi] + c]]);
 }
 
+constexpr uint32_t kEncStripCap = 2048;
+constexpr size_t kFlatResolveLds = 40960;
+static_assert(2 * strip_ccl_words(kEncStripCap) * sizeof(uint32_t) <= kFlatResolveLds, "two strip workgroups beside two walks");
+__global__ void __launch_bounds__(kBlock, 7) k_strip_ccl_enc(RunGeom g, StripArrays sa, const uint32_t* __restrict__ G, uint32_t n_pixels) {
+	__shared__ __attribute__((aligned(16))) uint32_t s_lds[strip_ccl_words(kEncStripCap)];
+	strip_ccl_body<false, false, true, kEncStripCap>(g, sa, RecordLists{}, G, n_pixels, nullptr, blockIdx.y, blockIdx.x, s_lds);
+}
+
+__global__ void __launch_bounds__(kBlock) k_gather_slots(
+	const uint64_t* __restrict__ slots, uint32_t slot_cap, const uint32_t* __restrict__ ncomp, const uint64_t* __restrict__ comp_off, uint64_t* __restrict__ mapping
+) {
+	const uint32_t zi = blockIdx.y;
+	const uint32_t c = blockIdx.x * kBlock + threadIdx.x;
+	if (c < ncomp[zi]) mapping[comp_off[zi] + c] = slots[static_cast<uint64_t>(zi) * slot_cap + c];
+}
+
 __global__ void __launch_bounds__(kBlock) k_paint_components(
 	const uint32_t* __restrict__ planeV, uint32_t row_words, uint64_t plane_words, uint32_t sx, uint64_t sxy,
 	const uint32_t* __restrict__ word_base, const uint64_t* __restrict__ rbase, const uint32_t* __restrict__ run_cc,
@@ -1507,11 +1524,27 @@
 	return ra;
 }
 
-void flat_enqueue(ckl_encoder& e, int64_t sx, int64_t sy, int64_t sz) {
+void flat_report_layout(ckl_encoder& e, uint32_t ns, hipStream_t s) {
+	e.d_flat_report.ensure(4 * static_cast<size_t>(ns) + 1);
+	e.d_ncomp.borrow(e.d_flat_report.p, ns); e.d_crc_acc.borrow(e.d_flat_report.p + ns, ns);
+	e.d_idbits.borrow(e.d_flat_report.p + 2 * static_cast<size_t>(ns), ns); e.d_slice_err2.borrow(e.d_flat_report.p + 3 * static_cast<size_t>(ns), ns);
+	CKL_HIP(hipMemsetAsync(e.d_slice_err2.p, 0, (static_cast<size_t>(ns) + 1) * sizeof(uint32_t), s));
+}
+
+RunGeom flat_geom(const ckl_encoder& e, int64_t sx, int64_t sy, uint32_t ns) {
+	RunGeom g;
+	g.planeV = plane_v(e); g.planeH = plane_h(e, ns);
+	g.row_words = e.row_words; g.plane_words = e.plane_words;
+	g.flip = 1u;
+	g.sx = static_cast<uint32_t>(sx); g.sy = static_cast<uint32_t>(sy);
+	return g;
+}
+
+void flat_enqueue_runs(ckl_encoder& e, int64_t sx, int64_t sy, int64_t sz) {
 	hipStream_t s = e.stream2;
 	const uint32_t ns = static_cast<uint32_t>(sz);
 	const uint64_t sxy = static_cast<uint64_t>(sx) * sy;
-	ensure_geom_table(e, sxy);
+	e.flat_strips = false;
 
 	std::vector<uint64_t>& rbase = e.h_rbase;
 	std::vector<uint32_t>& rcap = e.h_rcap;
@@ -1527,16 +1560,9 @@
 	e.d_word_base.ensure(e.plane_words * ns);
 	e.d_parent.ensure(rtot); e.d_run_start.ensure(rtot); e.d_run_cc.ensure(rtot); e.d_comp_pix.ensure(rtot);
 	e.d_nruns.ensure(ns);
-	e.d_flat_report.ensure(4 * static_cast<size_t>(ns));
-	e.d_ncomp.borrow(e.d_flat_report.p, ns); e.d_crc_acc.borrow(e.d_flat_report.p + ns, ns);
-	e.d_idbits.borrow(e.d_flat_report.p + 2 * static_cast<size_t>(ns), ns); e.d_slice_err2.borrow(e.d_flat_report.p + 3 * static_cast<size_t>(ns), ns);
-	CKL_HIP(hipMemsetAsync(e.d_slice_err2.p, 0, ns * sizeof(uint32_t), s));
-
-	RunGeom g;
-	g.planeV = plane_v(e); g.planeH = plane_h(e, ns);
-	g.row_words = e.row_words; g.plane_words = e.plane_words;
-	g.flip = 1u;
-	g.sx = static_cast<uint32_t>(sx); g.sy = static_cast<uint32_t>(sy);
+	flat_report_layout(e, ns, s);
+
+	const RunGeom g = flat_geom(e, sx, sy, ns);
 	const RunArrays ra = flat_arrays(e);
 	hipLaunchKernelGGL(k_run_index, dim3(ns), dim3(kIndexBlock), 0, s, g, ra);
 	launch_run_union(s, ns, g, ra);
@@ -1546,7 +1572,86 @@
 	e.d_blk_roots.ensure(static_cast<size_t>(rs.nblk) * ns);
 	rs.run_local = e.d_run_local.p; rs.blk_roots = e.d_blk_roots.p;
 	launch_run_resolve(s, ns, ra, rs, e.d_G.p, static_cast<uint32_t>(sxy), 0u, e.d_crc_acc.p, e.d_idbits.p);
-	HT_MARK("f:enqueue");
+	HT_MARK("f:enqueue_runs");
+}
+
+uint32_t flat_resolve_cap(size_t lds_bytes) {
+	uint32_t cap = static_cast<uint32_t>(std::min<size_t>(kResolveCap, (lds_bytes - (kMaxStrips + 64u) * 4u) / 4u));
+	if (const char* env = getenv("CKL_ENC_RESOLVE_CAP")) cap = std::min<uint32_t>(cap, static_cast<uint32_t>(std::max(1, atoi(env))));
+	return cap;
+}
+uint32_t flat_resolve_cap_max(ckl_encoder& e) {
+	if (!e.max_lds) CKL_HIP(hipDeviceGetAttribute(&e.max_lds, hipDeviceAttributeMaxSharedMemoryPerBlock, e.device));
+	return flat_resolve_cap(static_cast<size_t>(e.max_lds) - 8192u);
+}
+
+bool flat_strip_plan(ckl_encoder& e, int64_t sx, int64_t sy, uint32_t ns) {
+	if (getenv("CKL_ENC_LABEL_RUNS")) return false;
+	const uint64_t sxy = static_cast<uint64_t>(sx) * sy;
+	if (e.row_words == 0 || e.row_words > kStripWords || sxy >= 0xFFFF0000ull) return false;
+	uint64_t runs_max = 0, comps_min = 0;
+	const uint64_t pairs_up = static_cast<uint64_t>(sx) * (sy - 1);
+	for (uint32_t zi = 0; zi < ns; zi++) {
+		const uint64_t runs = static_cast<uint64_t>(sy) + e.count_v[zi];
+		const uint64_t equal_up = pairs_up - std::min<uint64_t>(pairs_up, e.count_h[zi]);
+		runs_max = std::max<uint64_t>(runs_max, runs);
+		comps_min = std::max<uint64_t>(comps_min, runs > equal_up ? runs - equal_up : 0ull);
+	}
+	const double runs_per_row = static_cast<double>(runs_max) / static_cast<double>(sy);
+	const uint32_t fit = static_cast<uint32_t>(0.7 * kEncStripCap / runs_per_row);
+	if (fit < 1u) return false;
+	const uint32_t rows = std::max<uint32_t>(1u, std::min<uint32_t>(kStripWords / e.row_words, fit));
+	const uint32_t nstrips = (static_cast<uint32_t>(sy) + rows - 1) / rows;
+	if (nstrips > kMaxStrips || comps_min > flat_resolve_cap_max(e)) return false;
+	e.flat_strip_rows = rows; e.flat_nstrips = nstrips;
+	e.flat_strip_cap = static_cast<uint32_t>(std::min<uint64_t>(kEncStripCap, static_cast<uint64_t>(rows) * sx));
+	if (const char* env = getenv("CKL_ENC_STRIP_CAP")) e.flat_strip_cap = std::min<uint32_t>(e.flat_strip_cap, static_cast<uint32_t>(std::max(1, atoi(env))));
+	return true;
+}
+
+StripArrays flat_strip_arrays(const ckl_encoder& e) {
+	StripArrays sa = {};
+	sa.run_lid = e.s_run_lid.p; sa.sc_w = e.s_sc_w.p; sa.sc_cc = e.s_sc_first.p;
+	sa.strip_nruns = e.s_strip_nruns.p; sa.strip_nsc = e.s_strip_nsc.p;
+	sa.seam_first = e.s_seam_first.p; sa.seam_last = e.s_seam_last.p;
+	sa.slice_err = e.d_slice_err2.p; sa.overflow = e.d_flat_report.p + 4 * e.d_ncomp.n;
+	sa.nstrips = e.flat_nstrips; sa.strip_rows = e.flat_strip_rows; sa.cap = e.flat_strip_cap; sa.zbase = 0;
+	return sa;
+}
+
+void flat_launch_resolve(ckl_encoder& e, const void* labels, int64_t sx, int64_t sy, uint32_t ns, uint32_t cap) {
+	hipStream_t s = e.stream2;
+	e.flat_resolve_cap = cap;
+	e.d_label_slots.ensure(static_cast<size_t>(ns) * cap);
+	ResolveArgs ra = {};
+	ra.cap = cap;
+	EncResolve en;
+	en.labels = labels; en.sxy = static_cast<uint64_t>(sx) * sy; en.slots = e.d_label_slots.p; en.crc_acc = e.d_crc_acc.p; en.idbits = e.d_idbits.p;
+	const RunGeom g = flat_geom(e, sx, sy, ns);
+	const StripArrays sa = flat_strip_arrays(e);
+	const size_t tab_bytes = static_cast<size_t>(cap) * sizeof(uint32_t);
+	with_label_type(e.dtype_bytes, [&](auto t) {
+		typedef typename decltype(t)::type LABEL;
+		if (tab_bytes > 48u * 1024u) CKL_HIP(hipFuncSetAttribute(reinterpret_cast<const void*>(&k_slice_resolve_enc<LABEL>), hipFuncAttributeMaxDynamicSharedMemorySize, static_cast<int>(tab_bytes)));
+		hipLaunchKernelGGL(k_slice_resolve_enc<LABEL>, dim3(ns), dim3(kResolveBlock), tab_bytes, s, g, sa, ra, en, e.d_ncomp.p);
+	});
+}
+
+void flat_enqueue(ckl_encoder& e, const void* labels, int64_t sx, int64_t sy, int64_t sz, bool need_runs, bool beside_walk) {
+	hipStream_t s = e.stream2;
+	const uint32_t ns = static_cast<uint32_t>(sz);
+	const uint64_t sxy = static_cast<uint64_t>(sx) * sy;
+	ensure_geom_table(e, sxy);
+	if (need_runs || !beside_walk || !flat_strip_plan(e, sx, sy, ns)) { flat_enqueue_runs(e, sx, sy, sz); return; }
+	e.flat_strips = true;
+	const size_t nst = static_cast<size_t>(e.flat_nstrips) * ns;
+	e.s_strip_nruns.ensure(nst); e.s_strip_nsc.ensure(nst);
+	e.s_seam_first.ensure(nst * e.row_words); e.s_seam_last.ensure(nst * e.row_words);
+	e.s_run_lid.ensure(nst * e.flat_strip_cap); e.s_sc_w.ensure(nst * e.flat_strip_cap); e.s_sc_first.ensure(nst * e.flat_strip_cap);
+	flat_report_layout(e, ns, s);
+	hipLaunchKernelGGL(k_strip_ccl_enc, dim3(e.flat_nstrips, ns), dim3(kBlock), 0, s, flat_geom(e, sx, sy, ns), flat_strip_arrays(e), e.d_G.p, static_cast<uint32_t>(sxy));
+	flat_launch_resolve(e, labels, sx, sy, ns, flat_resolve_cap(kFlatResolveLds));
+	HT_MARK("f:enqueue_strips");
 }
 
 template <typename LABEL>
@@ -1554,10 +1659,21 @@
 	hipStream_t s = e.stream2;
 	const uint32_t ns = static_cast<uint32_t>(sz);
 	const uint64_t sxy = static_cast<uint64_t>(sx) * sy;
-	const std::vector<uint32_t> rep = download(e.d_flat_report.p, 4 * static_cast<size_t>(ns), s);
+	const size_t rep_n = 4 * static_cast<size_t>(ns) + 1;
+	std::vector<uint32_t> rep = download(e.d_flat_report.p, rep_n, s);
+	if (e.flat_strips && rep[rep_n - 1] == 2u && e.flat_resolve_cap < flat_resolve_cap_max(e)) {
+		CKL_HIP(hipMemsetAsync(e.d_flat_report.p + rep_n - 1, 0, sizeof(uint32_t), s));
+		flat_launch_resolve(e, labels, sx, sy, ns, flat_resolve_cap_max(e));
+		HT_MARK("f:resolve_retry");
+		rep = download(e.d_flat_report.p, rep_n, s);
+	}
+	if (e.flat_strips && rep[rep_n - 1]) {
+		flat_enqueue_runs(e, sx, sy, sz);
+		rep = download(e.d_flat_report.p, rep_n, s);
+	}
 	const uint32_t *acc = rep.data() + ns, *idbits = rep.data() + 2 * static_cast<size_t>(ns), *errs = rep.data() + 3 * static_cast<size_t>(ns);
 	out.ncomp.assign(rep.begin(), rep.begin() + ns);
-	HT_MARK("f:wait");
+	HT_MARK(e.flat_strips ? "f:wait_strips" : "f:wait_runs");
 	for (uint32_t zi = 0; zi < ns; zi++) if (errs[zi]) throw Error(CKL_ERR_RUNTIME, "crackle_amd: run table overflow on z=" + std::to_string(zi));
 	const uint32_t init_term = gf_mul(0xFFFFFFFFu, gf_xpow(32ull * sxy));
 	out.crcs.resize(ns);
@@ -1567,17 +1683,17 @@
 		out.crcs[zi] = ~(gf_mul(acc[zi], fix) ^ init_term);
 	}
 
-	std::vector<uint64_t> comp_off(ns);
+	std::vector<uint64_t>& comp_off = e.h_comp_off;
+	comp_off.assign(ns, 0);
 	uint64_t total = 0;
 	for (uint32_t zi = 0; zi < ns; zi++) { comp_off[zi] = total; total += out.ncomp[zi]; }
 	upload(e.d_comp_off, comp_off, s);
 	e.d_mapping.ensure(total + 1);
-	const RunArrays ra = flat_arrays(e);
 	uint32_t max_ncomp = 1;
 	for (uint32_t zi = 0; zi < ns; zi++) max_ncomp = std::max(max_ncomp, out.ncomp[zi]);
-	hipLaunchKernelGGL(k_mapping_comps<LABEL>, dim3((max_ncomp + kBlock - 1) / kBlock, ns), dim3(kBlock), 0, s,
-		labels, ra, sxy, e.d_comp_off.p, e.d_mapping.p);
-	CKL_HIP(hipStreamSynchronize(s));
+	const dim3 grid((max_ncomp + kBlock - 1) / kBlock, ns);
+	if (e.flat_strips) hipLaunchKernelGGL(k_gather_slots, grid, dim3(kBlock), 0, s, e.d_label_slots.p, e.flat_resolve_cap, e.d_ncomp.p, e.d_comp_off.p, e.d_mapping.p);
+	else hipLaunchKernelGGL(k_mapping_comps<LABEL>, grid, dim3(kBlock), 0, s, labels, flat_arrays(e), sxy, e.d_comp_off.p, e.d_mapping.p);
 	out.total = total;
 }
 
@@ -1728,7 +1844,8 @@
 	if (head.markov_model_order > 13) throw Error(CKL_ERR_ARG, "crackle_amd: markov_model_order > 13 is not supported on device");
 
 	bool labels_at_walk = false;
-	if (labels_first && !graph_done) flat_enqueue(e, sx, sy, sz);
+	const bool need_runs = head.label_format != FLAT;
+	if (labels_first && !graph_done) flat_enqueue(e, labels, sx, sy, sz, need_runs, false);
 	const bool trail_cached = !graph_done && have_planes && ov && ov->has_model && head.markov_model_order > 0 && e.trail_for == static_cast<const void*>(labels)
 		&& e.trail_perm == (head.crack_format == PERMISSIBLE) && e.trail_order == head.markov_model_order;
 	e.trail_for = nullptr;
@@ -1740,8 +1857,8 @@
 		for (uint32_t v : e.count_special) max_special = std::max(max_special, v);
 		int max_lds = 0;
 		CKL_HIP(hipDeviceGetAttribute(&max_lds, hipDeviceAttributeMaxSharedMemoryPerBlock, e.device));
-		labels_at_walk = max_special < 5000 && 2 * trail_walk_lds(max_special) + 40960 <= static_cast<size_t>(max_lds);
-		if (!labels_at_walk) flat_enqueue(e, sx, sy, sz);
+		labels_at_walk = max_special < 5000 && 2 * trail_walk_lds(max_special) + kFlatResolveLds <= static_cast<size_t>(max_lds);
+		if (!labels_at_walk) flat_enqueue(e, labels, sx, sy, sz, need_runs, false);
 	}
 
 	const bool permissible = head.crack_format == PERMISSIBLE;
@@ -1786,7 +1903,7 @@
 	auto label_side = [&]() {
 		if (labels_at_walk) {
 			CKL_HIP(hipStreamWaitEvent(s2, e.evd0, 0));
-			flat_enqueue(e, sx, sy, sz);
+			flat_enqueue(e, labels, sx, sy, sz, need_runs, true);
 		}
 		flat_collect<LABEL>(e, labels, sx, sy, sz, fr);
 		HT_MARK("flat");
@@ -2179,7 +2296,7 @@
 	if (voxels == 0) return cc_device;
 	FlatResult fr;
 	if (!planes_cached(*e, labels_device, sx, sy, sz)) planes_pass_any(*e, labels_device, sx, sy, sz, nullptr);
-	flat_enqueue(*e, sx, sy, sz);
+	flat_enqueue(*e, labels_device, sx, sy, sz, true, false);
 	with_label_type(e->dtype_bytes, [&](auto t) { flat_collect(*e, static_cast<const typename decltype(t)::type*>(labels_device), sx, sy, sz, fr); });
 	if (fr.total + id_base > 0xFFFFFFFFull) throw Error(CKL_ERR_RUNTIME, "crackle_amd: too many components");
 	hipStream_t s2 = e->stream2;
diff --git a/crackle_amd/csrc/ckl_encoder.hpp b/crackle_amd/csrc/ckl_encoder.hpp
--- a/crackle_amd/csrc/ckl_encoder.hpp
+++ b/crackle_amd/csrc/ckl_encoder.hpp
@@ -71,6 +71,13 @@
 	int64_t planes_dims[3] = { 0, 0, 0 };
 	std::vector<uint64_t> h_rbase;
 	std::vector<uint32_t> h_rcap;
+	std::vector<uint64_t> h_comp_off;
+	DevBuf<uint16_t> s_run_lid, s_seam_first, s_seam_last;
+	DevBuf<uint32_t> s_sc_w, s_sc_first, s_strip_nruns, s_strip_nsc;
+	DevBuf<uint64_t> d_label_slots;
+	uint32_t flat_nstrips = 0, flat_strip_rows = 0, flat_strip_cap = 0, flat_resolve_cap = 0;
+	int max_lds = 0;
+	bool flat_strips = false;
 	std::vector<uint32_t> count_special, count_corner;
 	DevBuf<uint32_t> d_plane_partial, t_blk_special, t_blk_corner;
 	DevBuf<unsigned long long> d_plane_partial_max, d_plane_out;
diff --git a/crackle_amd/csrc/ckl_strips.hpp b/crackle_amd/csrc/ckl_strips.hpp
--- a/crackle_amd/csrc/ckl_strips.hpp
+++ b/crackle_amd/csrc/ckl_strips.hpp
@@ -118,22 +118,25 @@
 	}
 }
 
-constexpr uint32_t kStripCclWords = (kStripCap + kStripEdgeCap + kStripWords / 2 + 2 * kStripBitmapWords + kWaves + 2 + 7) & ~7u;
-template <bool DIAG, bool RECORDS>
+constexpr uint32_t strip_ccl_words(uint32_t cap) { return (cap + (kStripWords + cap / 2) + kStripWords / 2 + 2 * (cap / 32) + kWaves + 2 + 7) & ~7u; }
+constexpr uint32_t kStripCclWords = strip_ccl_words(kStripCap);
+template <bool DIAG, bool RECORDS, bool ENC = false, uint32_t CAP = kStripCap>
 __device__ __forceinline__ void strip_ccl_body(
 	const RunGeom& g, const StripArrays& sa, const RecordLists& rl, const uint32_t* __restrict__ G, uint32_t n_pixels, unsigned long long* __restrict__ diag,
 	uint32_t zi, uint32_t k, uint32_t* lds
 ) {
+	constexpr uint32_t kRunsPerThread = CAP / kBlock, kBitmapWords = CAP / 32, kEdgeCap = kStripWords + CAP / 2;
+	static_assert(CAP % kBlock == 0 && CAP % 64 == 0 && CAP <= kStripCap, "whole runs per thread, whole bitmap words");
 	uint32_t* s_parent = lds;
-	uint32_t* s_mem = s_parent + kStripCap;
-	uint16_t* s_wb = reinterpret_cast<uint16_t*>(s_mem + kStripEdgeCap);
+	uint32_t* s_mem = s_parent + CAP;
+	uint16_t* s_wb = reinterpret_cast<uint16_t*>(s_mem + kEdgeCap);
 	uint32_t* s_b = s_mem;
 	uint16_t* s_pool = reinterpret_cast<uint16_t*>(s_mem + kStripWords);
-	uint32_t* s_bm = s_mem + kStripEdgeCap + kStripWords / 2;
-	uint32_t* s_bmbase = s_bm + kStripBitmapWords;
-	uint32_t* s_scan = s_bmbase + kStripBitmapWords;
+	uint32_t* s_bm = s_mem + kEdgeCap + kStripWords / 2;
+	uint32_t* s_bmbase = s_bm + kBitmapWords;
+	uint32_t* s_scan = s_bmbase + kBitmapWords;
 	uint32_t* s_misc = s_scan + kWaves;
-	static_assert((kStripCap * 4) % 16 == 0 && (kStripEdgeCap * 4) % 16 == 0, "tables stay 16-byte aligned");
+	static_assert((CAP * 4) % 16 == 0 && (kEdgeCap * 4) % 16 == 0, "tables stay 16-byte aligned");
 	unsigned long long d_t = DIAG ? __builtin_amdgcn_s_memtime() : 0ull;
 	auto stamp = [&](int slot) {
 		if (DIAG && threadIdx.x == 0) {
@@ -151,7 +154,7 @@
 	const uint64_t slot = static_cast<uint64_t>(si) * sa.cap;
 	uint32_t b[4], up[4], upl[4], cnt = 0;
 	if (RECORDS) {
-		static_assert(kStripCap >= kStripWords, "plane H piece is built in the union-find table");
+		static_assert(CAP >= kStripWords, "plane H piece is built in the union-find table");
 		uint32_t* sV = s_mem;
 		uint32_t* sH = s_parent;
 		const uint32_t n_rec = min(rl.count[si], rl.cap);
@@ -239,16 +242,19 @@
 		}
 	}
 	for (uint32_t j = t; j < nloc; j += kBlock) s_parent[j] = j;
-	if (t < kStripBitmapWords) s_bm[t] = 0u;
+	if (t < kBitmapWords) s_bm[t] = 0u;
 	__syncthreads();
 	stamp(1);
-	uint32_t gv[kStripRunsPerThread];
+	uint32_t gv[kRunsPerThread];
+	uint32_t first_px[ENC ? (kRunsPerThread + 1) / 2 : 1] = {};
 	{
 		const uint32_t p0 = y0 * g.sx;
 #pragma unroll
-		for (uint32_t i = 0; i < kStripRunsPerThread; i++) {
+		for (uint32_t i = 0; i < kRunsPerThread; i++) {
 			const uint32_t j = t + i * kBlock;
-			gv[i] = G[n_pixels - (p0 + s_pool[j < nloc ? j : 0u])];
+			const uint32_t px = s_pool[j < nloc ? j : 0u];
+			gv[i] = G[n_pixels - (p0 + px)];
+			if (ENC) first_px[i >> 1] |= px << (16u * (i & 1u));
 		}
 	}
 	{
@@ -259,7 +265,7 @@
 			if (j && w[j] == 0) yy++;
 			if (wl >= nw) break;
 			const uint16_t wbv = s_wb[wl];
-			if (w[j] == 0) sa.row_run[static_cast<uint64_t>(zi) * g.sy + y0 + yy] = wbv;
+			if (!ENC && w[j] == 0) sa.row_run[static_cast<uint64_t>(zi) * g.sy + y0 + yy] = wbv;
 			if (wl < rw) sa.seam_first[static_cast<uint64_t>(si) * rw + wl] = wbv;
 			if (wl + rw >= nw) sa.seam_last[static_cast<uint64_t>(si) * rw + (wl + rw - nw)] = wbv;
 		}
@@ -277,7 +283,7 @@
 		uint32_t ve[1] = { n_e }, te[1];
 		block_excl_add<1>(ve, te, s_scan);
 		const uint32_t n_edges = te[0];
-		if (n_edges <= kStripEdgeCap) {
+		if (n_edges <= kEdgeCap) {
 			uint32_t at = ve[0];
 #pragma unroll
 			for (uint32_t j = 0; j < 4; j++) {
@@ -301,23 +307,23 @@
 	}
 	__syncthreads();
 	stamp(2);
-	uint32_t root[kStripRunsPerThread];
-#pragma unroll
-	for (uint32_t i = 0; i < kStripRunsPerThread; i++) {
+	uint32_t root[kRunsPerThread];
+#pragma unroll
+	for (uint32_t i = 0; i < kRunsPerThread; i++) {
 		const uint32_t j = t + i * kBlock;
 		root[i] = j < nloc ? sm_find(s_parent, j) : 0u;
 		if (j < nloc && root[i] == j) atomicOr(s_bm + (j >> 5), 1u << (j & 31u));
 	}
 	__syncthreads();
 	if (t < kWave) {
-		static_assert(kStripBitmapWords <= 2 * kWave, "two bitmap words per lane");
-		const uint32_t c0 = t < kStripBitmapWords ? __popc(s_bm[t]) : 0u;
-		const uint32_t c1 = t + kWave < kStripBitmapWords ? __popc(s_bm[t + kWave]) : 0u;
+		static_assert(kBitmapWords <= 2 * kWave, "two bitmap words per lane");
+		const uint32_t c0 = t < kBitmapWords ? __popc(s_bm[t]) : 0u;
+		const uint32_t c1 = t + kWave < kBitmapWords ? __popc(s_bm[t + kWave]) : 0u;
 		const uint32_t i0 = wave_incl_add(c0);
 		const uint32_t tot0 = __shfl(i0, kWave - 1, kWave);
 		const uint32_t i1 = wave_incl_add(c1);
-		if (t < kStripBitmapWords) s_bmbase[t] = i0 - c0;
-		if (t + kWave < kStripBitmapWords) s_bmbase[t + kWave] = tot0 + i1 - c1;
+		if (t < kBitmapWords) s_bmbase[t] = i0 - c0;
+		if (t + kWave < kBitmapWords) s_bmbase[t + kWave] = tot0 + i1 - c1;
 		if (t == kWave - 1) s_misc[1] = tot0 + i1;
 	}
 	__syncthreads();
@@ -325,7 +331,7 @@
 	uint16_t* lid_out = sa.run_lid + slot;
 	const bool narrow = nsc <= 256u;
 #pragma unroll
-	for (uint32_t i = 0; i < kStripRunsPerThread; i++) {
+	for (uint32_t i = 0; i < kRunsPerThread; i++) {
 		const uint32_t j = t + i * kBlock;
 		if (j >= nloc) break;
 		const uint32_t r = root[i];
@@ -333,12 +339,13 @@
 		s_pool[j] = static_cast<uint16_t>(lid);
 		if (narrow) reinterpret_cast<uint8_t*>(lid_out)[j] = static_cast<uint8_t>(lid);
 		else lid_out[j] = static_cast<uint16_t>(lid);
+		if (ENC && r == j) sa.sc_cc[slot + lid] = y0 * g.sx + ((first_px[i >> 1] >> (16u * (i & 1u))) & 0xFFFFu);
 	}
 	for (uint32_t j = t; j < nsc; j += kBlock) s_parent[j] = 0u;
 	__syncthreads();
 	stamp(3);
 #pragma unroll
-	for (uint32_t i = 0; i < kStripRunsPerThread; i++) {
+	for (uint32_t i = 0; i < kRunsPerThread; i++) {
 		const uint32_t j = t + i * kBlock;
 		if (j >= nloc) break;
 		atomicXor(s_parent + s_pool[j], gv[i]);
@@ -375,6 +382,15 @@
 	uint32_t host_flags_n;
 };
 
+constexpr uint32_t kEncIdBits = 16;
+struct EncResolve {
+	const void* labels;
+	uint64_t sxy;
+	uint64_t* slots;
+	uint32_t* crc_acc;
+	uint32_t* idbits;
+};
+
 template <int W>
 __device__ __forceinline__ uint64_t ld_le(const uint8_t* p) {
 	if constexpr (W == 1) return *p;
@@ -392,10 +408,10 @@
 	}
 }
 
-template <typename OUT, bool LABELS, bool DIAG>
+template <typename OUT, bool LABELS, bool DIAG, bool ENC = false>
 __device__ __forceinline__ bool slice_resolve_body(
 	const RunGeom& g, const StripArrays& sa, const ResolveArgs& ra, uint32_t* __restrict__ ncomp_out, unsigned long long* __restrict__ diag,
-	uint32_t zi, uint32_t* s_tab, uint32_t* s_scbase, uint32_t* s_scan, uint32_t* s_flag_p
+	uint32_t zi, uint32_t* s_tab, uint32_t* s_scbase, uint32_t* s_scan, uint32_t* s_flag_p, const EncResolve* en = nullptr
 ) {
 	uint32_t& s_flag = *s_flag_p;
 	static_assert(kResolveCap <= 0xFFFFu, "index and rank share a table entry");
@@ -480,7 +496,11 @@
 	stamp(1);
 	const uint32_t per = (total + kResolveBlock - 1) / kResolveBlock;
 	const uint32_t i0 = min(total, t * per), i1 = min(total, i0 + per);
-	for (uint32_t i = i0; i < i1; i++) sm_store(s_tab, i, sm_find(s_tab, i));
+	for (uint32_t i = i0; i < i1; i++) {
+		uint32_t r = i;
+		for (uint32_t p = sm_load(s_tab, r); p != r; p = sm_load(s_tab, r)) r = p;
+		sm_store(s_tab, i, r);
+	}
 	__syncthreads();
 	uint32_t nroot = 0;
 	for (uint32_t i = i0; i < i1; i++) nroot += s_tab[i] == i ? 1u : 0u;
@@ -500,8 +520,9 @@
 	__syncthreads();
 	stamp(2);
 	const uint32_t ncomp = tot2[0];
-	const uint32_t nexp = ra.ncomp_expect[zi];
-	const uint64_t coff = ra.comp_off[zi];
+	const uint32_t nexp = ENC ? 0u : ra.ncomp_expect[zi];
+	const uint64_t coff = ENC ? 0ull : ra.comp_off[zi];
+	const uint32_t idbits = ENC ? kEncIdBits : ra.idbits;
 	uint32_t part = 0;
 	uint32_t sidx = strip0;
 	for (uint32_t r0 = i0; r0 < i1; r0 += kPer) {
@@ -517,10 +538,14 @@
 			gi[q] = static_cast<uint64_t>(si0 + sq) * sa.cap + (ii - s_scbase[sq]);
 			cc[q] = s_tab[s_tab[ii] & 0xFFFFu] >> 16;
 			wgt[q] = sa.sc_w[gi[q]];
-			key[q] = 0;
+			key[q] = ENC ? sa.sc_cc[gi[q]] : 0u;
 		}
 		uint64_t lab[kPer];
-		if (LABELS) {
+		if (ENC) {
+#pragma unroll
+			for (uint32_t q = 0; q < kPer; q++) lab[q] = static_cast<const OUT*>(en->labels)[zi * en->sxy + key[q]];
+		}
+		else if (LABELS) {
 			with_width(ra.key_width, [&](auto W) {
 #pragma unroll
 				for (uint32_t q = 0; q < kPer; q++) key[q] = ld_le<decltype(W)::value>(ra.keys + (coff + (cc[q] < nexp ? cc[q] : 0u)) * static_cast<uint64_t>(decltype(W)::value));
@@ -537,7 +562,10 @@
 #pragma unroll
 		for (uint32_t q = 0; q < kPer; q++) {
 			if (r0 + q >= i1) continue;
-			if (LABELS) {
+			if (ENC) {
+				if ((s_tab[r0 + q] & 0xFFFFu) == r0 + q) en->slots[static_cast<uint64_t>(zi) * ra.cap + cc[q]] = lab[q];
+			}
+			else if (LABELS) {
 				uint64_t val = 0;
 				if (cc[q] < nexp && key[q] < ra.num_unique) {
 					val = lab[q];
@@ -548,7 +576,7 @@
 			}
 			else sa.sc_cc[gi[q]] = cc[q];
 			uint32_t wg = wgt[q];
-			for (int j = static_cast<int>(ra.idbits) - 1; j >= 0; j--) {
+			for (int j = static_cast<int>(idbits) - 1; j >= 0; j--) {
 				part ^= ((cc[q] >> j) & 1u) ? wg : 0u;
 				wg = (wg >> 1) ^ ((wg & 1u) ? kCrcPoly : 0u);
 			}
@@ -560,12 +588,15 @@
 	if (t == 0) {
 		uint32_t x = 0;
 		for (int wv = 0; wv < NW; wv++) x ^= s_scan[wv];
-		uint32_t e = 0;
-		if (ncomp != nexp) e |= ERR_NCOMP;
-		else if (ra.check_crc && gf_mul(x, ra.crc_fix) != ra.crc_expect[zi]) e |= ERR_CRC;
-		if (e) atomicOr(sa.slice_err + zi, e);
-		ncomp_out[zi] = ncomp;
-		if (ra.host_flags) ra.host_flags[zi] = sa.slice_err[zi] | e;
+		if (ENC) { ncomp_out[zi] = ncomp; en->crc_acc[zi] = x; en->idbits[zi] = kEncIdBits; }
+		else {
+			uint32_t e = 0;
+			if (ncomp != nexp) e |= ERR_NCOMP;
+			else if (ra.check_crc && gf_mul(x, ra.crc_fix) != ra.crc_expect[zi]) e |= ERR_CRC;
+			if (e) atomicOr(sa.slice_err + zi, e);
+			ncomp_out[zi] = ncomp;
+			if (ra.host_flags) ra.host_flags[zi] = sa.slice_err[zi] | e;
+		}
 	}
 	stamp(3);
 	return true;
@@ -578,6 +609,15 @@
 	__shared__ uint32_t s_scan[kResolveBlock / kWave];
 	__shared__ uint32_t s_flag;
 	slice_resolve_body<OUT, LABELS, DIAG>(g, sa, ra, ncomp_out, diag, blockIdx.x + sa.zbase, s_tab, s_scbase, s_scan, &s_flag);
+}
+
+template <typename LABEL>
+static __global__ void __launch_bounds__(kResolveBlock, 8) k_slice_resolve_enc(RunGeom g, StripArrays sa, ResolveArgs ra, EncResolve en, uint32_t* __restrict__ ncomp_out) {
+	extern __shared__ __attribute__((aligned(16))) uint32_t s_tab[];
+	__shared__ uint32_t s_scbase[kMaxStrips + 1];
+	__shared__ uint32_t s_scan[kResolveBlock / kWave];
+	__shared__ uint32_t s_flag;
+	slice_resolve_body<LABEL, false, false, true>(g, sa, ra, ncomp_out, nullptr, blockIdx.x, s_tab, s_scbase, s_scan, &s_flag, &en);
 }
 
 template <typename OUT>
```
